# Rinoahu/SwiftOrtho

Measured on AMD Instinct MI355X. Metric: M query-aa/s scanned all-vs-all, higher is better.
Workload: dtype u8/int16/int32 (5-bit packed residues, packed 16-bit score-only DP, int32 traced DP); 1 GPU; BASELINE config 3: 100000 synthetic proteins x 300 aa self-search, seed 11111011111, aa9, -M 120000000, -c 50000 (2 chunks), -e 1e-5, -v 500; query_aa=30007201, rows=1618760

## Files before the change

include/sohit.h:

```cpp
#ifndef SOHIT_H
#define SOHIT_H

#include <stdint.h>

#ifdef __cplusplus
extern "C" {
#endif

#define SOHIT_ABI_VERSION 3

typedef struct so_ctx so_ctx;

typedef struct so_params {
    const char *seeds;
    const char *alphabet;
    int64_t nc;
    int64_t chunk;
    int64_t step;
    int64_t max_hits;
    int64_t thr;
    double expect;
    double max_miss;
    int32_t filter;
    int32_t profile;
// ... 49 lines not shown
    double bgroup_ms;
} so_counters;

so_ctx *so_create(int device, const so_params *params);
void so_destroy(so_ctx *ctx);
const char *so_last_error(const so_ctx *ctx);
int so_abi_version(void);
int so_set_option(so_ctx *ctx, const char *name, const char *value);

int so_load_ref(so_ctx *ctx, const char *fasta_path, int64_t r_lo, int64_t r_hi);
int so_load_ref_mem(so_ctx *ctx, const char *fasta_bytes, int64_t nbytes, int64_t r_lo, int64_t r_hi);
int so_build_index(so_ctx *ctx);
int so_drop_index(so_ctx *ctx);
int so_load_index(so_ctx *ctx, const char *prefix);

int so_load_queries(so_ctx *ctx, const char *fasta_path);
int so_load_queries_mem(so_ctx *ctx, const char *fasta_bytes, int64_t nbytes);
int64_t so_num_queries(const so_ctx *ctx);
int64_t so_num_refs(const so_ctx *ctx);
int64_t so_query_len(const so_ctx *ctx, int64_t qidx);
int64_t so_ref_len(const so_ctx *ctx, int64_t sidx);

int so_search_loaded(so_ctx *ctx, int64_t q_lo, int64_t q_hi, so_hit **hits, int64_t *n_hits);
int so_search(so_ctx *ctx, const char *qry_fasta_path, int64_t q_lo, int64_t q_hi, so_hit **hits, int64_t *n_hits);
void so_free_hits(so_hit *hits);

int so_search_loaded_aln(so_ctx *ctx, int64_t q_lo, int64_t q_hi, so_hit **hits, int64_t *n_hits, char **aln, int64_t *aln_bytes);
void so_free_aln(char *aln);

int so_search_loaded_cigar(so_ctx *ctx, int64_t q_lo, int64_t q_hi, so_hit **hits, int64_t *n_hits, uint32_t **ops, int64_t **op_off);
void so_free_cigar(uint32_t *ops, int64_t *op_off);
int64_t so_format_cigar(const uint32_t *ops, int64_t n_ops, char *buf, int64_t cap);

int so_search_device(so_ctx *ctx, int64_t q_lo, int64_t q_hi, const so_hit **d_hits, int64_t *n_hits);
int so_device_hits_copy(so_ctx *ctx, void *dst_device, int64_t n_hits);
int so_query_work(so_ctx *ctx, int64_t q_lo, int64_t q_hi, uint64_t *work);

int so_write_sc(so_ctx *ctx, const so_hit *hits, int64_t n_hits, const char *path, const char *mode);
int64_t so_format_hit(so_ctx *ctx, const so_hit *hit, char *buf, int64_t cap);
int so_write_sc_cigar(so_ctx *ctx, const so_hit *hits, int64_t n_hits, const uint32_t *ops, const int64_t *op_off, const char *path,
                      const char *mode);

int so_set_profile(so_ctx *ctx, int on);
int64_t so_bucket_count(const so_ctx *ctx);
int64_t so_fmt_rows(const double *v, int64_t n, char *out, int64_t cap);
int so_get_counters(const so_ctx *ctx, so_counters *out);
int so_reset_counters(so_ctx *ctx);
int64_t so_timing_report(const so_ctx *ctx, char *buf, int64_t cap);
int64_t so_chunk_threshold(const so_ctx *ctx, int64_t chunk);
int64_t so_chunk_entries(const so_ctx *ctx, int64_t chunk);
int so_chunk_download(so_ctx *ctx, int64_t chunk, uint32_t *start, uint64_t *entries);
int64_t so_masked_query(so_ctx *ctx, int64_t qidx, char *buf, int64_t cap);
int64_t so_query_candidates(so_ctx *ctx, int64_t qidx, uint32_t *out4, int64_t cap);
int so_align_pairs(so_ctx *ctx, int kernel, int64_t n, const int64_t *task6, const uint32_t *order, int32_t *out);
int so_align_pairs_aln(so_ctx *ctx, int kernel, int64_t n, const int64_t *task6, const uint32_t *order, int32_t *out, char **aln,
                       int64_t *aln_bytes);

int so_align_pairs_cigar(so_ctx *ctx, int kernel, int64_t n, const int64_t *task6, const uint32_t *order, int32_t *out, uint32_t **ops,
                         int64_t **op_off);

typedef struct so_mcl_result {
    int64_t n, nnz;
    int32_t rounds;
    int32_t converged;
    int64_t *indptr;
    int32_t *indices;
    float *data;
} so_mcl_result;
int so_mcl(int device, int64_t n, const int64_t *indptr, const int32_t *indices, const float *data, double inflation, int32_t max_rounds,
           int32_t check_every, double prune, double rtol, double atol, so_mcl_result *out);
void so_mcl_free(so_mcl_result *result);
const char *so_mcl_last_error(void);

typedef struct so_apc_result {
    int64_t n_genes, n_entries;
    int32_t rounds;
    int64_t *labels;
    float *r;
    float *a;
} so_apc_result;
int so_apc(int device, int64_t n_genes, int64_t n_entries, const int32_t *row, const int32_t *col, const float *score, double damp,
           int32_t rounds, so_apc_result *out);
void so_apc_free(so_apc_result *result);
const char *so_apc_last_error(void);

typedef struct so_orth_cand {
    int64_t n_ot, n_ip, n_co, n_rows, n_runs, n_groups;
    int64_t *ot_a, *ot_b; double *ot_s;
    int64_t *ip_a, *ip_b; double *ip_s;
    int64_t *co_key;      double *co_best;
} so_orth_cand;
int so_orth_candidates_cols(int device, int64_t n, const int32_t *q, const int32_t *s, const double *idy, const double *aln,
                            const double *qst, const double *qed, const double *score, const double *qlen, int64_t n_names,
                            const int32_t *tax, int64_t n_taxa, double coverage, double identity, int norm, so_orth_cand *out);
int so_orth_candidates_records(int device, const so_hit *d_hits, int64_t n, const int32_t *qmap, int64_t n_q, const int32_t *smap,
                               int64_t n_s, int64_t n_names, const int32_t *tax, int64_t n_taxa, double coverage, double identity,
                               int norm, so_orth_cand *out);
void so_orth_free(so_orth_cand *result);
const char *so_orth_last_error(void);
typedef struct so_orth_rel {
    int64_t n_ip, n_ot, n_co, n_rows, n_runs, n_groups;
    int64_t *ip_a, *ip_b; double *ip_v;
    int64_t *ot_a, *ot_b; double *ot_v;
    int64_t *co_a, *co_b; double *co_v;
} so_orth_rel;
int so_orth_relations_cols(int device, int64_t n, const int32_t *q, const int32_t *s, const double *idy, const double *aln,
// ... 21 lines not shown
```

swiftortho_amd/_lib.py:

```python
import ctypes as C
import os

HERE = os.path.dirname(os.path.abspath(__file__))
LIBPATH = os.path.join(HERE, "libsohit.so")


class SoParams(C.Structure):
    _fields_ = [("seeds", C.c_char_p), ("alphabet", C.c_char_p), ("nc", C.c_int64), ("chunk", C.c_int64), ("step", C.c_int64),
                ("max_hits", C.c_int64), ("thr", C.c_int64), ("expect", C.c_double), ("max_miss", C.c_double),
                ("filter", C.c_int32), ("profile", C.c_int32)]


class SoOrthRel(C.Structure):
    _fields_ = [(n, C.c_int64) for n in ("n_ip", "n_ot", "n_co", "n_rows", "n_runs", "n_groups")] + \
               [("ip_a", C.POINTER(C.c_int64)), ("ip_b", C.POINTER(C.c_int64)), ("ip_v", C.POINTER(C.c_double)),
                ("ot_a", C.POINTER(C.c_int64)), ("ot_b", C.POINTER(C.c_int64)), ("ot_v", C.POINTER(C.c_double)),
                ("co_a", C.POINTER(C.c_int64)), ("co_b", C.POINTER(C.c_int64)), ("co_v", C.POINTER(C.c_double))]


class SoHit(C.Structure):
    _fields_ = [("qidx", C.c_int64), ("sidx", C.c_int64), ("identity", C.c_double), ("evalue", C.c_double), ("aln", C.c_int32),
                ("mis", C.c_int32), ("gap", C.c_int32), ("qst", C.c_int32), ("qed", C.c_int32), ("sst", C.c_int32),
                ("sed", C.c_int32), ("bit", C.c_int32), ("qlen", C.c_int32), ("slen", C.c_int32), ("matches", C.c_int32),
                ("ungapped", C.c_int32)]


class SoCounters(C.Structure):
    _fields_ = [(n, C.c_int64) for n in ("n_queries", "query_aa", "ref_seqs", "ref_aa", "n_chunks", "seed_windows", "seed_hits",
                                         "groups", "candidates", "alignments", "cells", "rows", "index_entries")] + \
               [("lookup_launches", C.c_int64), ("lookup_ms", C.c_double), ("lookup_bytes", C.c_int64),
                ("bounds_launches", C.c_int64), ("bounds_ms", C.c_double), ("bounds_bytes", C.c_int64),
                ("align_launches", C.c_int64), ("align_ms", C.c_double),
                ("index_ms", C.c_double), ("seed_ms", C.c_double), ("group_ms", C.c_double), ("phase2_ms", C.c_double),
                ("total_ms", C.c_double), ("count_launches", C.c_int64), ("count_ms", C.c_double),
                ("hits_bucketed", C.c_int64), ("align_wide", C.c_int64), ("cells_wide", C.c_int64), ("seed_passes", C.c_int64),
                ("ungap_steps", C.c_int64), ("groups_single", C.c_int64), ("groups_chain", C.c_int64),
                ("bgroup_launches", C.c_int64), ("bgroup_ms", C.c_double)]

    def as_dict(self):
        return {n: getattr(self, n) for n, _ in self._fields_}


EXPORTS = ["so_abi_version", "so_set_option", "so_create", "so_destroy", "so_last_error", "so_load_ref", "so_load_ref_mem", "so_build_index", "so_drop_index", "so_load_index",
           "so_load_queries", "so_load_queries_mem", "so_num_queries", "so_num_refs", "so_query_len", "so_search_loaded",
           "so_search", "so_free_hits", "so_search_loaded_aln", "so_free_aln", "so_write_sc", "so_format_hit", "so_get_counters", "so_reset_counters", "so_timing_report",
           "so_chunk_threshold", "so_chunk_entries", "so_chunk_download", "so_masked_query", "so_query_candidates", "so_align_pairs", "so_align_pairs_aln", "so_set_profile",
           "so_bucket_count", "so_ref_len", "so_search_device", "so_device_hits_copy", "so_query_work", "so_mcl", "so_mcl_free",
           "so_mcl_last_error", "so_tsv_lines", "so_tsv_scan", "so_tsv_codes", "so_format_pairs", "so_py_repr", "so_fmt_rows",
           "so_search_loaded_cigar", "so_free_cigar", "so_format_cigar", "so_write_sc_cigar", "so_align_pairs_cigar",
           "so_apc", "so_apc_free", "so_apc_last_error",
           "so_orth_candidates_cols", "so_orth_candidates_records", "so_orth_free", "so_orth_last_error",
           "so_orth_relations_cols", "so_orth_relations_records", "so_orth_rel_free"]


class SoMclResult(C.Structure):
    _fields_ = [("n", C.c_int64), ("nnz", C.c_int64), ("rounds", C.c_int32), ("converged", C.c_int32), ("indptr", C.POINTER(C.c_int64)),
                ("indices", C.POINTER(C.c_int32)), ("data", C.POINTER(C.c_float))]


class SoApcResult(C.Structure):
    _fields_ = [("n_genes", C.c_int64), ("n_entries", C.c_int64), ("rounds", C.c_int32), ("labels", C.POINTER(C.c_int64)),
                ("r", C.POINTER(C.c_float)), ("a", C.POINTER(C.c_float))]


class SoOrthCand(C.Structure):
    _fields_ = [(n, C.c_int64) for n in ("n_ot", "n_ip", "n_co", "n_rows", "n_runs", "n_groups")] + \
               [("ot_a", C.POINTER(C.c_int64)), ("ot_b", C.POINTER(C.c_int64)), ("ot_s", C.POINTER(C.c_double)),
                ("ip_a", C.POINTER(C.c_int64)), ("ip_b", C.POINTER(C.c_int64)), ("ip_s", C.POINTER(C.c_double)),
                ("co_key", C.POINTER(C.c_int64)), ("co_best", C.POINTER(C.c_double))]


_lib = None


def _preload_torch_hip_runtime():
    import importlib.util
    import sys
    if "torch" in sys.modules or os.environ.get("SOHIT_TORCH_PRELOAD") == "0":
        return
    try:
        spec = importlib.util.find_spec("torch")
    except (ImportError, ValueError):
        spec = None
    if not spec or not spec.submodule_search_locations:
        return
    p = os.path.join(list(spec.submodule_search_locations)[0], "lib", "libamdhip64.so")
    if os.path.isfile(p):
        try:
            C.CDLL(p, mode=C.RTLD_GLOBAL)
        except OSError:
            pass


def load():
    global _lib
    if _lib is not None:
        return _lib
    _preload_torch_hip_runtime()
    if not os.path.isfile(LIBPATH):
# ... 14 lines not shown
    L.so_load_queries.argtypes = [vp, cp]
    L.so_load_queries_mem.argtypes = [vp, cp, i64]
    for f in ("so_num_queries", "so_num_refs"):
        getattr(L, f).restype = i64
        getattr(L, f).argtypes = [vp]
    L.so_query_len.restype = i64
    L.so_query_len.argtypes = [vp, i64]
    L.so_ref_len.restype = i64
    L.so_ref_len.argtypes = [vp, i64]
    L.so_search_loaded.argtypes = [vp, i64, i64, C.POINTER(C.POINTER(SoHit)), C.POINTER(i64)]
    L.so_search.argtypes = [vp, cp, i64, i64, C.POINTER(C.POINTER(SoHit)), C.POINTER(i64)]
    L.so_free_hits.argtypes = [C.POINTER(SoHit)]
    L.so_search_loaded_aln.argtypes = [vp, i64, i64, C.POINTER(C.POINTER(SoHit)), C.POINTER(i64), C.POINTER(C.c_void_p), C.POINTER(i64)]
    L.so_free_aln.argtypes = [vp]
    L.so_search_loaded_cigar.argtypes = [vp, i64, i64, C.POINTER(C.POINTER(SoHit)), C.POINTER(i64), C.POINTER(C.c_void_p), C.POINTER(C.c_void_p)]
    L.so_free_cigar.argtypes = [vp, vp]
    L.so_free_cigar.restype = None
    L.so_format_cigar.restype = i64
    L.so_format_cigar.argtypes = [vp, i64, vp, i64]
    L.so_write_sc_cigar.argtypes = [vp, C.POINTER(SoHit), i64, vp, vp, cp, cp]
    L.so_align_pairs_cigar.argtypes = [vp, C.c_int, i64, vp, vp, vp, C.POINTER(C.c_void_p), C.POINTER(C.c_void_p)]
    L.so_search_device.argtypes = [vp, i64, i64, C.POINTER(vp), C.POINTER(i64)]
    L.so_device_hits_copy.argtypes = [vp, vp, i64]
    L.so_query_work.argtypes = [vp, i64, i64, vp]
    L.so_write_sc.argtypes = [vp, C.POINTER(SoHit), i64, cp, cp]
    L.so_format_hit.restype = i64
    L.so_format_hit.argtypes = [vp, C.POINTER(SoHit), cp, i64]
    L.so_get_counters.argtypes = [vp, C.POINTER(SoCounters)]
    L.so_set_profile.argtypes = [vp, C.c_int]
    L.so_bucket_count.restype = i64
    L.so_bucket_count.argtypes = [vp]
    L.so_reset_counters.argtypes = [vp]
    L.so_timing_report.restype = i64
    L.so_timing_report.argtypes = [vp, cp, i64]
    L.so_tsv_lines.restype = i64
    L.so_tsv_lines.argtypes = [vp, i64, vp, i64]
    L.so_tsv_scan.argtypes = [vp, i64, vp, i64, C.c_int32, vp, vp, vp, vp, vp, vp, vp]
    L.so_tsv_codes.restype = i64
    L.so_tsv_codes.argtypes = [vp, i64, vp, vp, vp, vp, vp, vp, vp, vp, i64]
    L.so_format_pairs.restype = i64
    L.so_format_pairs.argtypes = [cp, C.c_int32, vp, vp, vp, vp, vp, i64, vp, i64]
    L.so_py_repr.restype = i64
    L.so_py_repr.argtypes = [vp, i64, vp, i64]
    L.so_fmt_rows.restype = i64
    L.so_fmt_rows.argtypes = [vp, i64, vp, i64]
    for f in ("so_chunk_threshold", "so_chunk_entries"):
        getattr(L, f).restype = i64
        getattr(L, f).argtypes = [vp, i64]
    L.so_chunk_download.argtypes = [vp, i64, vp, vp]
    L.so_masked_query.restype = i64
    L.so_masked_query.argtypes = [vp, i64, cp, i64]
    L.so_query_candidates.restype = i64
    L.so_query_candidates.argtypes = [vp, i64, vp, i64]
    L.so_align_pairs.argtypes = [vp, C.c_int, i64, vp, vp, vp]
    L.so_align_pairs_aln.argtypes = [vp, C.c_int, i64, vp, vp, vp, C.POINTER(C.c_void_p), C.POINTER(i64)]
    L.so_mcl.argtypes = [C.c_int, i64, vp, vp, vp, C.c_double, C.c_int32, C.c_int32, C.c_double, C.c_double, C.c_double, C.POINTER(SoMclResult)]
    L.so_mcl_free.argtypes = [C.POINTER(SoMclResult)]
    L.so_mcl_last_error.restype = cp
    L.so_apc.argtypes = [C.c_int, i64, i64, vp, vp, vp, C.c_double, C.c_int32, C.POINTER(SoApcResult)]
    L.so_apc_free.argtypes = [C.POINTER(SoApcResult)]
    L.so_apc_last_error.restype = cp
    L.so_orth_candidates_cols.argtypes = [C.c_int, i64, vp, vp, vp, vp, vp, vp, vp, vp, i64, vp, i64, C.c_double, C.c_double, C.c_int, C.POINTER(SoOrthCand)]
    L.so_orth_candidates_records.argtypes = [C.c_int, vp, i64, vp, i64, vp, i64, i64, vp, i64, C.c_double, C.c_double, C.c_int, C.POINTER(SoOrthCand)]
    L.so_orth_free.argtypes = [C.POINTER(SoOrthCand)]
    L.so_orth_last_error.restype = cp
    L.so_orth_relations_cols.argtypes = L.so_orth_candidates_cols.argtypes[:-1] + [C.POINTER(SoOrthRel)]
    L.so_orth_relations_records.argtypes = L.so_orth_candidates_records.argtypes[:-1] + [C.POINTER(SoOrthRel)]
    L.so_orth_rel_free.argtypes = [C.POINTER(SoOrthRel)]
    L.so_set_option.argtypes = [vp, cp, cp]
    if L.so_abi_version() != 3:
        raise ImportError("libsohit.so ABI version mismatch")
    _lib = L
    return L
```

swiftortho_amd/csrc/host.h:

```cpp
#pragma once
#include "common.h"
#include "kernels.h"
#include "seedhash.h"
#include "../../include/sohit.h"

#include <algorithm>
#include <array>
#include <atomic>
#include <chrono>
#include <cmath>
#include <cstring>
#include <functional>
#include <map>
#include <malloc.h>
#include <memory>
#include <mutex>
#include <thread>
#include <unordered_map>
#include <sys/stat.h>

inline double wall() { return std::chrono::duration<double>(std::chrono::steady_clock::now().time_since_epoch()).count(); }

extern double (*volatile p_pow)(double, double);
extern double (*volatile p_log)(double);
// ... 159 lines not shown
    struct BandPlan { i64 lo, hi; int bp; bool multi_ok; int k; u64 nband; };
    std::vector<BandPlan> band_plans;
    i64 r_lo = -1, r_hi = -1;
    std::vector<std::unique_ptr<ChunkIndex>> chunks;
    std::vector<std::unique_ptr<ChunkIndex>> spare_chunks;
    std::vector<std::string> masked;
    i64 masked_lo = 0;
    std::vector<std::vector<u32>> last_cands;
    u64 qry_gen = 0;
    i64 last_q_lo = 0;
    so_counters cnt;
    DevBuf<u32> d_scan_tmp, d_tmp32a, d_tmp32b;
    DevBuf<u64> d_stats;
    DevBuf<u32> d_small;
    DevBuf<u32> ix_bkt, ix_bkt2, ix_flags, ix_ridx, ix_plan, ix_tk;
    DevBuf<u64> ix_ent, ix_tv;
    DevBuf<u8> d_pcls;
    DevBuf<u8> d_sort_tmp;
    hipEvent_t ev0 = nullptr, ev1 = nullptr;
    hipStream_t st_rows = nullptr;
    hipEvent_t ev_rows = nullptr, ev_rows_done = nullptr;
    hipEvent_t ev_part[EMIT_PARTS_MAX] = {nullptr};
    hipStream_t st_side = nullptr;
    hipEvent_t ev_side_go = nullptr, ev_korder = nullptr;
    hipStream_t st_ug = nullptr;
    hipEvent_t ev_ug_go = nullptr, ev_ug_done = nullptr;
    hipEvent_t ev_bnd_go = nullptr, ev_bnd_done = nullptr;
    bool rows_in_flight = false;
    bool count_tab_now = false;
    size_t max_hits_per_pass = (size_t)1 << 30;
    u32 max_batch = 131072;
    DevBuf<u8> d_segtab, d_symmap, d_upmap, d_segmask;
    bool seg_on_device = false;
    bool q_present[256];
    void* pinned = nullptr;
    size_t pinned_cap = 0;
    bool want_aln = false;
    bool want_cigar = false;
    void* pinned_aln = nullptr;
    size_t pinned_aln_cap = 0;
    hipEvent_t ev_aln = nullptr;
    struct EmitJob {
        std::thread th;
        bool active = false;
        size_t base = 0, n = 0;
        bool aln = false;
        bool cig = false;
        std::atomic<i64> dropped{0};
        std::exception_ptr err;
    } emit;
    unsigned long long* h_qhits = nullptr;
    size_t h_qhits_cap = 0;
    unsigned long long* h_small = nullptr;
    std::map<std::string, double> tm;
    std::map<std::string, double> lt;
    std::shared_ptr<void> batch;
    std::thread warm;
    bool dev_out = false;
    DevBuf<u8> d_hits;
    size_t d_hits_n = 0;
    DevBuf<double> d_p2tab;
};

static inline u64 cand_limit() { return tune().cand_limit > 0 ? (u64)tune().cand_limit : 0xFFFFFFF0ull; }


struct SegTables {
    double lg12[64];
    double lgn[13][32];
    double log2v;
    SegTables() {
        log2v = p_log(2);
        for (int k = 1; k < 64; ++k) lg12[k] = p_log((double)k / 12.);
        lg12[0] = 0;
        for (int n = 1; n <= 12; ++n)
            for (int j = 1; j < 32; ++j) lgn[n][j] = p_log((double)j / ((double)n * 1.));
    }
};


template <class F>
void parallel_for(i64 n, F f) {
    unsigned nt = std::max(1u, std::min(16u, std::thread::hardware_concurrency()));
    if (n < 200000 || nt == 1) {
        for (i64 i = 0; i < n; ++i) f(i);
        return;
    }
    std::atomic<i64> next(0);
    std::vector<std::thread> th;
    for (unsigned t = 0; t < nt; ++t)
        th.emplace_back([&] {
            for (;;) {
                i64 b = next.fetch_add(4096);
                if (b >= n) break;
                for (i64 i = b; i < std::min(n, b + 4096); ++i) f(i);
            }
        });
    for (auto& t : th) t.join();
}


inline AlnSide aln_side(const SeqSet& s) { return AlnSide{s.d_res.p, s.d_scls.p, s.d_scls4.p, s.d_pcls.p, s.d_pcls4.p, s.d_off.p, s.d_bound.p}; }
struct AlnChain {
    DevBuf<u32> units, rofs, aofs, code, words, cofs, comp, runs, oofs, ops;
    size_t slot_words = 0;
};
// ... 262 lines not shown
        if (n + extra <= cap) return;
        if (!p) p = g_hit_cache.take(cap);
        if (n + extra <= cap) return;
        size_t nc = std::max<size_t>(n + extra, cap + cap / 2 + 1024);
        so_hit* np_ = (so_hit*)realloc(p, nc * sizeof(so_hit));
        if (!np_) throw SoError("out of host memory for the result rows");
        p = np_;
        cap = nc;
    }
    so_hit* release() {
        so_hit* r = p ? p : (so_hit*)malloc(sizeof(so_hit));
        p = nullptr;
        n = cap = 0;
        return r;
    }
    ~HitBuf() { g_hit_cache.give(p); }
};

struct HostRow {
    int v[12];
};

std::vector<std::string> split(const std::string& s, char sep);
void build_score_maps(u8 smap[256], signed char b62c[SCLS_N * SCLS_N]);
void nr_table(const std::string& gaa, int tbl[256]);
void byte_presence(const u8* bytes, size_t n, bool present[256]);
void build_hash_classes(const bool present[256], const std::vector<std::array<int, 256>>& codes, u8 hmap[256], HashLut& lut);
void set_tune(const Tune* t);
void set_params(so_ctx* c, const so_params* p);
void upload_constants(so_ctx* c);
void layout_set(so_ctx* c, SeqSet& s, const bool present[256], size_t nres, u32 nseq);
void upload_set(so_ctx* c, SeqSet& s, const u8* residues, const std::vector<u32>& off, u32 nseq, const bool* present_in = nullptr);
const SegTables& seg_tables();
void seg_mask(const u8* S, int n, u8* out);
void load_ref_common(so_ctx* c, i64 r_lo, i64 r_hi);
void load_queries_common(so_ctx* c, bool parsed = false);
void file_stamp(const char* path, long long& size, long long& mtime_ns);
bool read_file(const char* path, std::string& out);
i64 chunk_threshold(so_ctx* c, const u32* d_counts , u64 s1, u64 s2, u64 nn);
void warm_sort_modules(int device);
void build_index(so_ctx* c);
void load_index(so_ctx* c, const char* prefix);
void band_plan(so_ctx* c, ChunkIndex& ch, int bp, bool multi_ok, int* k_out, u64* nband_out);
ChunkIndex::BandEnc* band_encoding(so_ctx* c, ChunkIndex& ch, int ba, int bp, bool multi_ok);
void order_chunk(so_ctx* c, ChunkIndex& ch);
const ChunkIndex::RangeTab* range_table(so_ctx* c, ChunkIndex& ch, const ChunkIndex::BandEnc& e, int wb, u32 R);
void prepare_batch(so_ctx* c, Batch& b, i64 q_lo, i64 q_hi);
void order_queries(so_ctx* c, Batch& b);
void order_open_queries(so_ctx* c, Batch& b, const unsigned long long* qh);
void* small_host(so_ctx* c);
u32 d2h_u32(so_ctx* c, const u32* p);
void stash_u32(so_ctx* c, const u32* p, int slot);
void d2h_pair(so_ctx* c, const u32* second, u32& a, u32& b);
void ensure_sort_tmp(so_ctx* c, size_t bytes);
const unsigned long long* chunk_qhits(so_ctx* c, Batch& b, int ci);
void chunk_qhits_deferred(so_ctx* c, Batch& b, int ci);
bool class_takes_sorted_path(so_ctx* c, ChunkIndex& ch, u32 maxq, unsigned long long hits, unsigned long long nq);
void seed_stage(so_ctx* c, Batch& b, int ci);
void seed_pass(so_ctx* c, Batch& b, int ci, u32 qa, u32 qb, double t0, StageClock& sc);
void emit_join(so_ctx* c, HitBuf& out);
void phase2(so_ctx* c, Batch& b, HitBuf& out);
void align_pairs(so_ctx* c, int kernel, i64 n, const int64_t* task6, const uint32_t* order, int32_t* out, AlnBytes* aln = nullptr, CigarBuf* cig = nullptr);
void aln_decode(const u32* w, int AL, const u8* qp, const u8* sp, char* sq, char* ss);
void search_loaded(so_ctx* c, i64 q_lo, i64 q_hi, HitBuf& out);
void query_work(so_ctx* c, i64 q_lo, i64 q_hi, u64* out);
void format_hit_into(so_ctx* c, const so_hit& h, std::vector<char>& out);
std::string format_hit(so_ctx* c, const so_hit& h);
extern std::string g_create_err;


template <class F>
int guarded(so_ctx* c, F f) {
    try {
        if (!c) return 1;
        set_tune(&c->tune);
        g_poison = (int)c->tune.poison;
        HIP_CHECK(hipSetDevice(c->device));
        f();
        c->err.clear();
        return 0;
    } catch (const std::exception& e) {
        if (c) c->err = e.what();
        return 1;
    }
}
```

swiftortho_amd/csrc/host_abi.hip:

```cpp
#include "host.h"

std::string g_create_err;


int fmt_f6(double x, char* out) {
    if (!(std::fabs(x) < 1e15)) return snprintf(out, 400, "%f", x);
    char* o = out;
    if (std::signbit(x)) *o++ = '-', x = -x;
    unsigned __int128 q = 0;
    if (x != 0) {
        int ex;
        const double fr = frexp(x, &ex);
        const u64 m = (u64)ldexp(fr, 53);
        const int e = ex - 53;
        const unsigned __int128 P = (unsigned __int128)m * 1000000u;
        if (e >= 0) {
            q = P << e;
        } else if (-e < 100) {
            const int sh = -e;
            q = P >> sh;
            const unsigned __int128 rem = P & (((unsigned __int128)1 << sh) - 1), half = (unsigned __int128)1 << (sh - 1);
            if (rem > half || (rem == half && (q & 1))) ++q;
        }
    }
// ... 101 lines not shown
        if (!params) throw SoError("so_create: params is NULL");
        int n = 0;
        hipError_t e = hipGetDeviceCount(&n);
        if (e != hipSuccess || n <= 0) throw SoError("so_create: no HIP device available (libsohit has no CPU fallback)");
        if (device < 0 || device >= n) throw SoError("so_create: device index out of range");
        HIP_CHECK(hipSetDevice(device));
        c = new so_ctx();
        c->device = device;
        c->tune.read();
        set_tune(&c->tune);
        g_poison = (int)c->tune.poison;
        {
            int ncu = 0;
            HIP_CHECK(hipDeviceGetAttribute(&ncu, hipDeviceAttributeMultiprocessorCount, device));
            c->ncu = (u32)std::max(1, ncu);
        }
        memset(&c->cnt, 0, sizeof c->cnt);
        set_params(c, params);
        HIP_CHECK(hipStreamCreate(&c->st));
        HIP_CHECK(hipEventCreate(&c->ev0));
        HIP_CHECK(hipEventCreate(&c->ev1));
        HIP_CHECK(hipStreamCreateWithFlags(&c->st_rows, hipStreamNonBlocking));
        HIP_CHECK(hipEventCreateWithFlags(&c->ev_rows, hipEventDisableTiming));
        HIP_CHECK(hipEventCreateWithFlags(&c->ev_rows_done, hipEventDisableTiming));
        HIP_CHECK(hipEventCreateWithFlags(&c->ev_aln, hipEventDisableTiming));
        for (auto& e : c->ev_part) HIP_CHECK(hipEventCreateWithFlags(&e, hipEventDisableTiming));
        HIP_CHECK(hipStreamCreateWithFlags(&c->st_side, hipStreamNonBlocking));
        HIP_CHECK(hipEventCreateWithFlags(&c->ev_side_go, hipEventDisableTiming));
        HIP_CHECK(hipEventCreateWithFlags(&c->ev_korder, hipEventDisableTiming));
        HIP_CHECK(hipStreamCreateWithFlags(&c->st_ug, hipStreamNonBlocking));
        HIP_CHECK(hipEventCreateWithFlags(&c->ev_ug_go, hipEventDisableTiming));
        HIP_CHECK(hipEventCreateWithFlags(&c->ev_ug_done, hipEventDisableTiming));
        HIP_CHECK(hipEventCreateWithFlags(&c->ev_bnd_go, hipEventDisableTiming));
        HIP_CHECK(hipEventCreateWithFlags(&c->ev_bnd_done, hipEventDisableTiming));
        upload_constants(c);
        c->warm = std::thread(warm_sort_modules, device);
        g_create_err.clear();
        return c;
    } catch (const std::exception& e) {
        g_create_err = e.what();
        delete c;
        return nullptr;
    }
}

void so_destroy(so_ctx* c) {
    if (!c) return;
    if (c->warm.joinable()) c->warm.join();
    (void)hipSetDevice(c->device);
    if (c->st) (void)hipStreamSynchronize(c->st);
    if (c->pinned) (void)hipHostFree(c->pinned);
    if (c->pinned_aln) (void)hipHostFree(c->pinned_aln);
    if (c->h_small) (void)hipHostFree(c->h_small);
    if (c->h_qhits) (void)hipHostFree(c->h_qhits);
    if (c->ev0) (void)hipEventDestroy(c->ev0);
    if (c->ev1) (void)hipEventDestroy(c->ev1);
    if (c->ev_rows) (void)hipEventDestroy(c->ev_rows);
    if (c->ev_rows_done) (void)hipEventDestroy(c->ev_rows_done);
    if (c->ev_aln) (void)hipEventDestroy(c->ev_aln);
    for (auto& e : c->ev_part)
        if (e) (void)hipEventDestroy(e);
    if (c->st_rows) (void)hipStreamDestroy(c->st_rows);
    if (c->ev_side_go) (void)hipEventDestroy(c->ev_side_go);
    if (c->ev_korder) (void)hipEventDestroy(c->ev_korder);
    if (c->st_side) (void)hipStreamDestroy(c->st_side);
    if (c->ev_ug_go) (void)hipEventDestroy(c->ev_ug_go);
    if (c->ev_ug_done) (void)hipEventDestroy(c->ev_ug_done);
    if (c->ev_bnd_go) (void)hipEventDestroy(c->ev_bnd_go);
    if (c->ev_bnd_done) (void)hipEventDestroy(c->ev_bnd_done);
    if (c->st_ug) (void)hipStreamDestroy(c->st_ug);
    if (c->st) (void)hipStreamDestroy(c->st);
    if (&c->tune == &tune()) set_tune(nullptr);
    delete c;
    g_hit_cache.clear();
    g_cig_ops_cache.clear(), g_cig_off_cache.clear();
}

const char* so_last_error(const so_ctx* c) { return c ? c->err.c_str() : g_create_err.c_str(); }

int so_load_ref(so_ctx* c, const char* path, int64_t r_lo, int64_t r_hi) {
    return guarded(c, [&] {
        if (!read_file(path, c->ref.data)) throw SoError(std::string("cannot read reference FASTA ") + path);
        load_ref_common(c, r_lo, r_hi);
        c->ref_path = path;
        file_stamp(path, c->ref_fsize, c->ref_mtime_ns);
    });
}

int so_load_ref_mem(so_ctx* c, const char* bytes, int64_t n, int64_t r_lo, int64_t r_hi) {
    return guarded(c, [&] {
        c->ref.data.assign(bytes, (size_t)n);
        load_ref_common(c, r_lo, r_hi);
        c->ref_path.clear();
    });
}

int so_build_index(so_ctx* c) {
    return guarded(c, [&] { build_index(c); });
}

int so_load_index(so_ctx* c, const char* prefix) {
    return guarded(c, [&] { load_index(c, prefix); });
}

int so_drop_index(so_ctx* c) {
    return guarded(c, [&] {
// ... 326 lines not shown
    memset(&c->cnt, 0, sizeof c->cnt);
    c->cnt.ref_seqs = keep.ref_seqs, c->cnt.ref_aa = keep.ref_aa, c->cnt.n_chunks = keep.n_chunks;
    c->cnt.index_entries = keep.index_entries;
    return 0;
}

int64_t so_chunk_threshold(const so_ctx* c, int64_t k) { return (c && k >= 0 && k < (int64_t)c->chunks.size()) ? c->chunks[k]->threshold : -1; }
int64_t so_chunk_entries(const so_ctx* c, int64_t k) { return (c && k >= 0 && k < (int64_t)c->chunks.size()) ? (int64_t)c->chunks[k]->E : -1; }

int so_chunk_download(so_ctx* c, int64_t k, uint32_t* start, uint64_t* entries) {
    return guarded(c, [&] {
        if (k < 0 || k >= (int64_t)c->chunks.size()) throw SoError("so_chunk_download: no such chunk");
        ChunkIndex& ch = *c->chunks[k];
        order_chunk(c, ch);
        if (start) {
            std::vector<u32> ub(ch.U), ubeg((size_t)ch.U + 1);
            if (ch.U) {
                HIP_CHECK(hipMemcpy(ub.data(), ch.ub.p, (size_t)ch.U * sizeof(u32), hipMemcpyDeviceToHost));
                HIP_CHECK(hipMemcpy(ubeg.data(), ch.ubeg.p, ((size_t)ch.U + 1) * sizeof(u32), hipMemcpyDeviceToHost));
            }
            size_t k = 0;
            for (size_t bk = 0; bk <= (size_t)c->nc; ++bk) {
                while (k < ch.U && ub[k] < bk) ++k;
                start[bk] = k < ch.U ? ubeg[k] : ch.E;
            }
        }
        if (entries && ch.E) {
            HIP_CHECK(hipStreamSynchronize(c->st));
            HIP_CHECK(hipMemcpy(entries, ch.entries.p, (size_t)ch.E * sizeof(u64), hipMemcpyDeviceToHost));
        }
    });
}

int64_t so_masked_query(so_ctx* c, int64_t q, char* buf, int64_t cap) {
    if (!c) return -1;
    i64 k = q - c->masked_lo;
    if (k < 0 || k >= (i64)c->masked.size()) return -1;
    const std::string& s = c->masked[(size_t)k];
    if (buf && cap > 0) memcpy(buf, s.data(), std::min<size_t>(s.size(), (size_t)cap));
    return (int64_t)s.size();
}

int64_t so_query_candidates(so_ctx* c, int64_t q, uint32_t* out4, int64_t cap) {
    if (!c) return -1;
    i64 k = q - c->last_q_lo;
    if (k < 0 || k >= (i64)c->last_cands.size()) return -1;
    const auto& v = c->last_cands[(size_t)k];
    const int64_t n = (int64_t)v.size() / 4;
    if (out4)
        for (int64_t i = 0; i < std::min(n, cap) * 4; ++i) out4[i] = v[(size_t)i];
    return n;
}

int so_align_pairs(so_ctx* c, int kernel, int64_t n, const int64_t* task6, const uint32_t* order, int32_t* out) {
    return guarded(c, [&] { align_pairs(c, kernel, n, task6, order, out); });
}

int so_align_pairs_aln(so_ctx* c, int kernel, int64_t n, const int64_t* task6, const uint32_t* order, int32_t* out, char** aln, int64_t* aln_bytes) {
    return guarded(c, [&] {
        if (!aln || !aln_bytes) throw SoError("so_align_pairs_aln: output pointers are NULL");
        *aln = nullptr, *aln_bytes = 0;
        if (kernel != 3 && kernel != 4) throw SoError("so_align_pairs_aln: only the traced kernels (3, 4) give alignments");
        AlnBytes a;
        align_pairs(c, kernel, n, task6, order, out, &a);
        *aln_bytes = (int64_t)a.n;
        *aln = a.release();
    });
}

int so_align_pairs_cigar(so_ctx* c, int kernel, int64_t n, const int64_t* task6, const uint32_t* order, int32_t* out, uint32_t** ops, int64_t** op_off) {
    return guarded(c, [&] {
        if (!ops || !op_off) throw SoError("so_align_pairs_cigar: output pointers are NULL");
        *ops = nullptr, *op_off = nullptr;
        if (kernel != 3 && kernel != 4) throw SoError("so_align_pairs_cigar: only the traced kernels (3, 4) give alignments");
        CigarBuf g;
        align_pairs(c, kernel, n, task6, order, out, nullptr, &g);
        g.release(ops, op_off);
    });
}

}
```

swiftortho_amd/csrc/host_index.hip:

```cpp
#include "host.h"


i64 chunk_threshold(so_ctx* c, const u32* d_counts , u64 s1, u64 s2, u64 nn) {
    const double N = (double)(nn + 1);
    const double mu = (double)s1 / N;
    long double lm = (long double)mu;
    long double ss = (long double)s2 - 2.0L * lm * (long double)s1 + (long double)nn * lm * lm;
    if (ss < 0) ss = 0;
    long double T = lm + 2.0L * sqrtl(ss / (long double)N);
    long double fl = floorl(T);
    long double margin = ((long double)nn * 8e-16L + 1e-11L) * (T + 1.0L);
    const bool forced = tune().exact_threshold;
    if (!forced && T - fl > margin && (fl + 1.0L) - T > margin) return (i64)fl;
    std::vector<u32> counts((size_t)nn);
    if (nn) HIP_CHECK(hipMemcpyAsync(counts.data(), d_counts, (size_t)nn * sizeof(u32), hipMemcpyDeviceToHost, c->st));
    HIP_CHECK(hipStreamSynchronize(c->st));
    i64 Nn = 1;
    double m = 0.;
    for (u32 v : counts)
        if (v > 0) m += (double)v, Nn += 1;
    m /= (double)Nn;
    double sd = 0.;
    for (u32 v : counts)
        if (v > 0) sd += p_pow((double)v - m, 2);
// ... 48 lines not shown
    };
    for (i64 s = Start; s < End; s += c->chunk) {
        std::unique_ptr<ChunkIndex> ch;
        if (!c->spare_chunks.empty()) {
            ch = std::move(c->spare_chunks.front());
            c->spare_chunks.erase(c->spare_chunks.begin());
            ch->d_sh_subj = ch->d_sh_diag = -1;
            for (auto& e : ch->encs) e->stale = true;
            ch->ordered = false;
            for (auto& t : ch->rtabs) t->k = -1;
        } else {
            ch = std::make_unique<ChunkIndex>();
        }
        i64 e = std::min(s + c->chunk, End);
        ch->seq_lo = std::min<i64>(std::max<i64>(0, s), N);
        ch->seq_hi = std::min<i64>(e, N);
        if (ch->seq_hi < ch->seq_lo) ch->seq_hi = ch->seq_lo;
        ch->p_lo = c->ref.off[ch->seq_lo] + (u32)ch->seq_lo;
        ch->p_hi = c->ref.off[ch->seq_hi] + (u32)ch->seq_hi;
        ch->maxslen = 0;
        for (i64 j = ch->seq_lo; j < ch->seq_hi; ++j) ch->maxslen = std::max(ch->maxslen, c->ref.len(j));
        {
            ch->use_dir = (u64)NC <= (tune().dir_max >= 0 ? (u64)tune().dir_max : (1ull << 28));
        }
        const u32 npos = ch->p_hi - ch->p_lo;
        const int AS = c->cfg.A * c->cfg.S;
        const u64 nslots64 = (u64)npos * (u64)AS;
        if (nslots64 >= (1ull << 31)) throw SoError("chunk holds 2^31 seed-window slots or more; lower -c");
        const u32 nslots = (u32)nslots64;
        u32 E = 0;
        ch->U = 0;
        u64 s2 = 0;
        if (nslots) {
            c->ix_bkt.ensure((size_t)nslots + 4), c->ix_ent.ensure((size_t)nslots + 4);
            c->ix_plan.ensure(ixsort_plan_elems((u32)NC) + 8);
            c->d_scan_tmp.ensure(scan_u32_temp_elems(std::max<size_t>(ixsort_plan_elems((u32)NC), (size_t)nslots + 1)) + 8);
            dlap("alloc pairs / plan");
            launch_index_windows_sparse(c->ref.d_words.p, c->ref.d_pseq.p, c->ref.d_off.p, ch->p_lo, ch->p_hi, c->ref.Ppad, (u32)ch->seq_lo, c->cfg, c->ref.lut,
                                        (u32)c->step, c->ix_bkt.p, c->ix_ent.p, c->st);
            E = d2h_u32(c, ixsort_count(c->ix_bkt.p, nslots, (u32)NC, c->ix_plan.p, c->d_scan_tmp.p, c->st));
            dlap("windows + level-1 count");
        }
        if ((u64)E >= (1ull << 29)) throw SoError("chunk index exceeds 2^29 entries (the lookup kernel addresses 8-byte slots with 32-bit byte offsets); lower -c");
        ch->E = E;
        ch->entries.ensure((size_t)E + 4);
        if (E) {
            c->ix_bkt2.ensure((size_t)E + 4), c->ix_tk.ensure((size_t)E + 4), c->ix_tv.ensure((size_t)E + 4);
            dlap("alloc entries / grouping scratch");
            ixsort_finish(c->ix_bkt.p, c->ix_ent.p, nslots, (u32)NC, c->ix_plan.p, c->ix_tk.p, c->ix_tv.p, c->ix_bkt2.p, ch->entries.p, c->st);
            dlap("pair grouping");
            c->ix_flags.ensure((size_t)E + 4), c->ix_ridx.ensure((size_t)E + 4);
            c->d_scan_tmp.ensure(scan_u32_temp_elems((size_t)E + 1) + 8);
            launch_run_heads(c->ix_bkt2.p, E, c->ix_flags.p, c->st);
            const u32 U = d2h_u32(c, scan_u32(c->ix_flags.p, c->ix_ridx.p, E, false, c->d_scan_tmp.p, c->st));
            ch->U = U;
            ch->ub.ensure((size_t)U + 4), ch->ubeg.ensure((size_t)U + 4), ch->ucnt.ensure((size_t)U + 4);
            launch_run_list(c->ix_bkt2.p, c->ix_flags.p, c->ix_ridx.p, E, U, ch->ub.p, ch->ubeg.p, ch->ucnt.p, c->st);
            dlap("run heads / list");
            launch_index_stats(ch->ucnt.p, U, c->d_stats.p, c->st);
            u64* stats = (u64*)small_host(c);
            u32* last_lo_h = (u32*)(stats + 4);
            HIP_CHECK(hipMemcpyAsync(stats, c->d_stats.p, 4 * sizeof(u64), hipMemcpyDeviceToHost, c->st));
            HIP_CHECK(hipMemcpyAsync(last_lo_h, ch->ubeg.p + (U - 1), sizeof(u32), hipMemcpyDeviceToHost, c->st));
            HIP_CHECK(hipStreamSynchronize(c->st));
            s2 = stats[1];
            const u32 last_lo = *last_lo_h;
            dlap("stats");
            if (ch->use_dir) {
                const size_t nd = (size_t)NC / 32 + 2;
                ch->dir.ensure(nd);
                HIP_CHECK(hipMemsetAsync(ch->dir.p, 0, nd * sizeof(u64), c->st));
                launch_dir_build(ch->ub.p, U, ch->dir.p, c->st);
            } else {
                u32 cap = 1024;
                int lg = 10;
                while (cap < 2 * U) cap <<= 1, ++lg;
                ch->hkey.ensure(cap), ch->hval.ensure(cap);
                ch->hshift = 32 - lg, ch->hmask = cap - 1;
                HIP_CHECK(hipMemsetAsync(ch->hkey.p, 0xFF, (size_t)cap * sizeof(u32), c->st));
                launch_htab_insert(ch->ub.p, ch->ubeg.p, U, ch->hkey.p, ch->hval.p, ch->hshift, ch->hmask, c->st);
            }
            launch_index_fixlast(ch->entries.p, last_lo, E, c->st);
        } else if (ch->use_dir) {
            const size_t nd = (size_t)NC / 32 + 2;
            ch->dir.ensure(nd);
            ch->ubeg.ensure(4);
            HIP_CHECK(hipMemsetAsync(ch->dir.p, 0, nd * sizeof(u64), c->st));
        } else {
            ch->hkey.ensure(1024), ch->hval.ensure(1024);
            ch->hshift = 22, ch->hmask = 1023;
            HIP_CHECK(hipMemsetAsync(ch->hkey.p, 0xFF, 1024 * sizeof(u32), c->st));
        }
        dlap("directory + fixlast");
        ch->threshold = chunk_threshold(c, ch->ucnt.p, (u64)E, s2, (u64)ch->U);
        ch->s2 = s2;
        HIP_CHECK(hipStreamSynchronize(c->st));
        c->cnt.index_entries += ch->E;
        c->chunks.push_back(std::move(ch));
    }
    c->spare_chunks.clear();
    c->cnt.n_chunks = (i64)c->chunks.size();
    c->index_built = true;
    c->cnt.index_ms += (wall() - t0) * 1e3;
}


bool host_window_bucket(const so_ctx* c, const u8* seq, u32 len, u32 pos, int a, int s, u32* bucket) {
// ... 314 lines not shown
```

swiftortho_amd/csrc/host_phase2.hip:

```cpp
#include "host.h"


void aln_decode(const u32* w, int AL, const u8* qp, const u8* sp, char* sq, char* ss) {
    for (int f = 0; f < AL; ++f) {
        const int cc = AL - 1 - f;
        const u32 code = (w[cc >> 4] >> ((cc & 15) << 1)) & 3u;
        sq[f] = code != 2 ? (char)*qp++ : '-';
        ss[f] = code != 3 ? (char)*sp++ : '-';
    }
}

void emit_join(so_ctx* c, HitBuf& out) {
    if (!c->emit.active) return;
    c->emit.th.join();
    c->emit.active = false;
    if (c->emit.err) {
        std::exception_ptr e = c->emit.err;
        c->emit.err = nullptr;
        std::rethrow_exception(e);
    }
    if (c->emit.dropped.load()) {
        const double expect = c->expect;
        if (c->emit.cig) {
            CigarBuf& g = out.cig;
            size_t w = c->emit.base;
            int64_t rp = g.off[c->emit.base], ap = rp;
            for (size_t k = c->emit.base; k < c->emit.base + c->emit.n; ++k) {
                const int64_t re = g.off[k + 1], nr = re - rp;
                if (out.p[k].evalue <= expect) {
                    if (nr && ap != rp) memmove(g.ops + ap, g.ops + rp, (size_t)nr * sizeof(uint32_t));
                    ap += nr;
                    g.off[++w] = ap;
                }
                rp = re;
            }
            g.n = (size_t)ap;
        }
        size_t wpos = c->emit.base;
        size_t bytes = 0;
        if (c->emit.aln)
            for (size_t k = c->emit.base; k < c->emit.base + c->emit.n; ++k) bytes += 2 * (size_t)std::max(0, out.p[k].aln);
        size_t rpos = out.aln.n - std::min(bytes, out.aln.n), apos = rpos;
        for (size_t k = c->emit.base; k < c->emit.base + c->emit.n; ++k) {
            const size_t nb = c->emit.aln ? 2 * (size_t)std::max(0, out.p[k].aln) : 0;
            if (out.p[k].evalue <= expect) {
                if (nb && apos != rpos) memmove(out.aln.p + apos, out.aln.p + rpos, nb);
                apos += nb;
                out.p[wpos++] = out.p[k];
            }
            rpos += nb;
        }
        out.n = wpos;
        if (c->emit.aln) out.aln.n = apos;
    }
}

enum { P2TAB_N = 1200 };
static const double* pow2_table() {
    static const std::vector<double> t = [] {
        std::vector<double> v(P2TAB_N);
        for (int k = 0; k < P2TAB_N; ++k) v[k] = p_pow(2, (double)(-k));
        return v;
    }();
    return t.data();
}

static void aln_slots(so_ctx* c, AlnChain& a, const AlnTask* tasks, const u32* list, u32 n, u32 ntasks, const AlnSeqs& s) {
    a.units.ensure((size_t)n + 4), a.rofs.ensure((size_t)n + 4), a.aofs.ensure((size_t)ntasks + 4);
    c->d_scan_tmp.ensure(scan_u32_temp_elems((size_t)n + 1) + 8);
    if ((u64)n * 129u >= (1ull << 30)) throw SoError("alignments: more than 8 M reported rows in one batch; search a smaller query range per call");
    launch_aln_units(tasks, list, n, s, a.units.p, c->st);
    const size_t units = d2h_u32(c, scan_u32(a.units.p, a.rofs.p, (size_t)n + 1, false, c->d_scan_tmp.p, c->st));
    a.slot_words = units * aln_unit_words();
    a.code.ensure(a.slot_words + 64);
    launch_aln_scatter(list, n, a.rofs.p, a.aofs.p, c->st);
}
static size_t aln_compact(so_ctx* c, AlnChain& a, const u32* list, u32 n, const AlnRes* res) {
    a.words.ensure((size_t)n + 4), a.cofs.ensure((size_t)n + 4);
    launch_aln_words(list, n, res, a.words.p, c->st);
    const size_t words = d2h_u32(c, scan_u32(a.words.p, a.cofs.p, (size_t)n + 1, false, c->d_scan_tmp.p, c->st));
    a.comp.ensure(words + 64);
    launch_aln_compact(list, n, a.aofs.p, a.code.p, a.cofs.p, a.comp.p, c->st);
    return words;
}
static size_t cigar_code(so_ctx* c, AlnChain& a, const u32* list, u32 n, const AlnRes* res) {
    if (a.slot_words * 16ull >= (1ull << 32)) throw SoError("CIGARs: the reported rows of one batch hold 2^32 columns or more; search a smaller query range per call");
    a.runs.ensure((size_t)n + 4), a.oofs.ensure((size_t)n + 4);
    launch_cigar_count(list, n, a.aofs.p, a.code.p, res, a.runs.p, c->st);
    const size_t n_ops = d2h_u32(c, scan_u32(a.runs.p, a.oofs.p, (size_t)n + 1, false, c->d_scan_tmp.p, c->st));
    a.ops.ensure(n_ops + 64);
    launch_cigar_emit(list, n, a.aofs.p, a.code.p, res, a.oofs.p, a.ops.p, c->st);
    return n_ops;
}
template <class F>
static std::vector<size_t> aln_word_offsets(size_t n, F aln_at, size_t words, const char* who) {
    std::vector<size_t> w(n + 1, 0);
    for (size_t i = 0; i < n; ++i) w[i + 1] = w[i] + (size_t)(std::max(0, (int)aln_at(i)) + 15) / 16;
    if (w[n] != words) throw SoError(std::string(who) + ": column words do not add up");
    return w;
}

struct P2 {
    P2(so_ctx* c, const Batch& b) : sc(c), nq(b.nq) {}
    const double t0 = wall();
    StageClock sc;
    u32 nq, Ntot = 0, NT = 0, nspec = 0, NO = 0;
    AlnSeqs seqs{};
    bool align_sort = false, pk_on = false, pk_mixed = false, lane_on = false, traced_pk = false, aln_on = false, cig_on = false;
    u32 stride = 0, slab = 0, TU = 0;
    size_t var_budget_words = 0, aln_words = 0, cig_ops = 0;
    int parts = 1; u32 qstep = 0;
    std::array<u32, EMIT_PARTS_MAX + 1> part_row{};
    std::vector<u32> h_ooff;
};

static bool gather_candidates(so_ctx* c, Batch& b, P2& p) {
    const int nchunks = (int)c->chunks.size();
    const u32 nq = p.nq;
    const u32 Ntot = p.Ntot = b.chunk_base.empty() ? 0u : b.chunk_base.back();
    b.qtot.ensure((size_t)nq + 4), b.qcoff.ensure((size_t)nq + 4), b.prior.ensure((size_t)nq + 4), b.cqoff.ensure((size_t)nq + 4);
    HIP_CHECK(hipMemsetAsync(b.qtot.p, 0, ((size_t)nq + 4) * sizeof(u32), c->st));
    for (int ci = 0; ci < nchunks; ++ci) launch_add_u32(b.qtot.p, b.ccnt.p + (size_t)ci * nq, nq, c->st);
    c->d_scan_tmp.ensure(scan_u32_temp_elems((size_t)nq + 1) + 8);
    scan_u32(b.qtot.p, b.qcoff.p, (size_t)nq + 1, false, c->d_scan_tmp.p, c->st);
    b.fin_rec.ensure(4 * (size_t)Ntot + 16);
    HIP_CHECK(hipMemsetAsync(b.prior.p, 0, ((size_t)nq + 4) * sizeof(u32), c->st));
    for (int ci = 0; ci < nchunks; ++ci) {
        const u32 lo = ci == 0 ? 0u : b.chunk_base[ci - 1], hi = b.chunk_base[ci];
        const u32* cc = b.ccnt.p + (size_t)ci * nq;
        if (hi > lo) {
            scan_u32(cc, b.cqoff.p, nq, false, c->d_scan_tmp.p, c->st);
            launch_gather_cands(b.cand_q.p + lo, b.cand_rec.p + 4 * (size_t)lo, hi - lo, b.cqoff.p, b.prior.p, b.qcoff.p, b.fin_rec.p,
                                c->st);
        }
        launch_add_u32(b.prior.p, cc, nq, c->st);
    }
    p.sc.lap("phase2.gather");
    if (tune().keep_cands) {
        std::vector<u32> qcoff((size_t)nq + 1), rec(4 * (size_t)Ntot + 4);
        HIP_CHECK(hipMemcpyAsync(qcoff.data(), b.qcoff.p, ((size_t)nq + 1) * sizeof(u32), hipMemcpyDeviceToHost, c->st));
        if (Ntot) HIP_CHECK(hipMemcpyAsync(rec.data(), b.fin_rec.p, 4 * (size_t)Ntot * sizeof(u32), hipMemcpyDeviceToHost, c->st));
        HIP_CHECK(hipStreamSynchronize(c->st));
        for (u32 q = 0; q < nq; ++q) {
            auto& dst = c->last_cands[(size_t)(b.q_lo - c->last_q_lo) + b.qid[q]];
            dst.assign(rec.begin() + 4 * (size_t)qcoff[q], rec.begin() + 4 * (size_t)qcoff[q + 1]);
        }
    }
    return Ntot != 0;
}

static void make_tasks(so_ctx* c, Batch& b, P2& p) {
    const u32 nq = p.nq, Ntot = p.Ntot;
    const u32 vmax = (u32)std::max<i64>(100, std::max<i64>(c->v + 100, (i64)((double)c->v * 1.1)));
    b.perm.ensure((size_t)Ntot + 4), b.ntask.ensure((size_t)nq + 4), b.ntile.ensure((size_t)nq + 4);
    b.toff.ensure((size_t)nq + 4), b.roffc.ensure((size_t)nq + 4);
    HIP_CHECK(hipMemsetAsync(b.ntask.p, 0, ((size_t)nq + 4) * sizeof(u32), c->st));
    HIP_CHECK(hipMemsetAsync(b.ntile.p, 0, ((size_t)nq + 4) * sizeof(u32), c->st));
    if (c->h_qhits_cap < nq) {
        if (c->h_qhits) (void)hipHostFree(c->h_qhits);
        c->h_qhits_cap = (size_t)nq + 1024;
        HIP_CHECK(hipHostMalloc((void**)&c->h_qhits, c->h_qhits_cap * sizeof(unsigned long long), hipHostMallocDefault));
    }
    const u32* qt = reinterpret_cast<const u32*>(c->h_qhits);
    HIP_CHECK(hipMemcpyAsync(c->h_qhits, b.qtot.p, (size_t)nq * sizeof(u32), hipMemcpyDeviceToHost, c->st));
    HIP_CHECK(hipStreamSynchronize(c->st));
    u32 mx = 0;
    for (u32 i = 0; i < nq; ++i) mx = std::max(mx, qt[i]);
    u64* gx = nullptr;
    u32 *gL = nullptr, *gR = nullptr;
    if ((int)mx > csort_lds_max()) {
        b.gx.ensure((size_t)Ntot + 4), b.gL.ensure((size_t)Ntot + 4), b.gR.ensure((size_t)Ntot + 4);
        gx = b.gx.p, gL = b.gL.p, gR = b.gR.p;
    }
    const bool cs_aside = gx != nullptr;
    if (cs_aside) {
        HIP_CHECK(hipEventRecord(c->ev_ug_go, c->st));
        HIP_CHECK(hipStreamWaitEvent(c->st_side, c->ev_ug_go, 0));
    }
    launch_csort(b.fin_rec.p, b.qcoff.p, nq, vmax, b.dev.d_off.p, c->ref.d_off.p, b.perm.p, b.ntask.p, b.ntile.p, gx, gL, gR, c->st,
                 cs_aside ? c->st_side : c->st);
    if (cs_aside) {
        HIP_CHECK(hipEventRecord(c->ev_ug_done, c->st_side));
        HIP_CHECK(hipStreamWaitEvent(c->st, c->ev_ug_done, 0));
    }
    const u32* dNRk = scan_u32(b.ntask.p, b.roffc.p, (size_t)nq + 1, false, c->d_scan_tmp.p, c->st);
    stash_u32(c, dNRk, SM_STASH0);
    const u32* dNT = scan_u32(b.ntile.p, b.toff.p, (size_t)nq + 1, false, c->d_scan_tmp.p, c->st);
    u32 NRK;
    d2h_pair(c, dNT, NRK, p.NT);
    const u32 NT = p.NT;
    p.sc.lap("phase2.csort");
    b.tasks.ensure((size_t)NT + 4), b.ares.ensure((size_t)NT + 4), b.bits.ensure((size_t)NT + 4), b.sel.ensure((size_t)NT + 4);
    b.rk_slot.ensure((size_t)NRK + 4);
    b.qcells.ensure((size_t)nq + 2);
    HIP_CHECK(hipMemsetAsync(b.qcells.p, 0, ((size_t)nq + 2) * sizeof(unsigned long long), c->st));
    launch_mktasks(b.fin_rec.p, b.qcoff.p, b.perm.p, b.ntask.p, b.roffc.p, b.toff.p, nq, b.dev.d_off.p, c->ref.d_off.p, b.tasks.p,
                   b.rk_slot.p, c->st);
    p.align_sort = tune().align_sort;
    const u32 maxwin_q = std::min<u32>(b.maxqlen, LONG_SEQ), maxwin_s = std::min<u32>(c->ref.maxlen, LONG_SEQ);
    p.pk_on = tune().align_pk && align_pk_supported(c->st);
    p.pk_mixed = p.pk_on && (int)std::min(maxwin_q, maxwin_s) > align_pk_max_len();
    p.seqs = AlnSeqs{aln_side(b.dev), aln_side(c->ref), c->d_b62c.p};
    p.lane_on = p.pk_on && tune().align_lane && b.maxqlen < LONG_SEQ && c->ref.maxlen < LONG_SEQ;
    p.traced_pk = p.pk_on;
    p.stride = align_trace_stride((int)std::min<u32>(std::max(maxwin_q, maxwin_s), std::min(maxwin_q, maxwin_s) + 16) + 1);
    const long long trace_var_max = tune().trace_var_max;
    const size_t budget_words = trace_var_max >= 0 ? (size_t)trace_var_max : (size_t)1 << 30;
    p.slab = (u32)std::max<size_t>(16, std::min<size_t>(std::max<u32>(NT, 1), budget_words / std::max<u32>(p.stride, 1)));
    p.var_budget_words = trace_var_max >= 0 ? (size_t)trace_var_max : (size_t)1 << 31;
    p.TU = align_trace_unit();
    b.st_state.ensure(5 * (size_t)nq + 8), b.rcnt.ensure((size_t)nq + 4), b.tcnt.ensure((size_t)nq + 4), b.roff.ensure((size_t)nq + 4);
    b.order_tmp.ensure((size_t)nq + 4);
    b.ridx.ensure((size_t)NT + 4);
    HIP_CHECK(hipMemsetAsync(b.st_state.p, 0, (5 * (size_t)nq + 8) * sizeof(u32), c->st));
    p.sc.lap("phase2.mktasks");
}

static void order_by_rows(so_ctx* c, Batch& b, const AlnSeqs& s, const u32* in, u32 n, u32* out, u32* n_wide, unsigned long long* cells) {
    if (!n) return;
    b.tmp64.ensure((size_t)n + 2), b.c_ft2.ensure((size_t)n + 2);
    ensure_sort_tmp(c, sort_pairs_u64_u32_temp_bytes(n, 64));
    launch_task_rows(b.tasks.p, in, n, s, n_wide, cells, b.tmp64.p, c->st);
    sort_pairs_u64_u32(c->d_sort_tmp.p, c->d_sort_tmp.cap, b.tmp64.p, b.c_ft2.p, in, out, n, n_wide ? 14 : 13, c->st);
}

static const u32* round_list(so_ctx* c, Batch& b, const P2& p, const u32* list, u32 n, u32* n_wide) {
    const bool split = n_wide && p.pk_mixed;
    if (n_wide) *n_wide = p.pk_on ? 0u : n;
    if (!split && (!p.align_sort || n < 4096)) return list;
    b.ridx2.ensure((size_t)n + 2);
    c->d_small.ensure(SM_WORDS);
    if (split) HIP_CHECK(hipMemsetAsync(c->d_small.p + SM_WIDE_ROUND, 0, sizeof(u32), c->st));
    order_by_rows(c, b, p.seqs, list, n, b.ridx2.p, split ? c->d_small.p + SM_WIDE_ROUND : nullptr, b.ucount.p + 2);
    if (split) *n_wide = d2h_u32(c, c->d_small.p + SM_WIDE_ROUND);
    return b.ridx2.p;
}

static size_t trace_offsets(so_ctx* c, Batch& b, const P2& p, const u32* list, u32 n) {
    if ((u64)n * ((u64)(p.stride + p.TU - 1) / p.TU + 1) >= (1ull << 32)) return ~(size_t)0;
    b.tr_units.ensure((size_t)n + 4), b.tr_ofs.ensure((size_t)n + 4);
    c->d_scan_tmp.ensure(scan_u32_temp_elems((size_t)n + 1) + 8);
    launch_trace_units(b.tasks.p, list, n, p.seqs, b.tr_units.p, c->st);
    return (size_t)d2h_u32(c, scan_u32(b.tr_units.p, b.tr_ofs.p, (size_t)n + 1, false, c->d_scan_tmp.p, c->st)) * p.TU;
}

static void align_rounds(so_ctx* c, Batch& b, P2& p) {
    const u32 nq = p.nq, NT = p.NT;
    const AlnSeqs& s = p.seqs;
    u32 aligned_total = 0;
    const bool spec_on = tune().spec >= 0 ? tune().spec != 0 : NT >= (1u << 21);
    const double spec_slack = tune().spec_slack;
    u32 spec_cap = NT;
    if (tune().spec_cap >= 0) spec_cap = (u32)tune().spec_cap;
    if (spec_on) {
        b.tpos.ensure((size_t)NT + 4);
        HIP_CHECK(hipMemsetAsync(b.tpos.p, 0xFF, ((size_t)NT + 4) * sizeof(u32), c->st));
    }
    bool first_round = true;
    for (u32 minr = 8;; minr = minr < 256 ? minr * 2 : minr) {
        u32 NR = 0, RR = 0, NS = 0;
        bool spec_round = spec_on && first_round;
        first_round = false;
        if (spec_round) {
            b.spcnt.ensure((size_t)nq + 4), b.spoff.ensure((size_t)nq + 4), b.sidx.ensure((size_t)NT + 4);
            c->d_small.ensure(SM_WORDS);
            HIP_CHECK(hipMemsetAsync(c->d_small.p + SM_ANY_RANK, 0, sizeof(u32), c->st));
            launch_round_counts_spec(b.ntask.p, b.ntile.p, b.roffc.p, b.rk_slot.p, b.qcoff.p, b.st_state.p, nq, c->max_miss, minr, b.tasks.p, b.toff.p,
                                     b.dev.d_off.p, c->ref.d_off.p, c->d_bittab.p, so_ctx::BITTAB_N, c->ref.N, c->expect * spec_slack, b.rcnt.p, b.tcnt.p, b.spcnt.p,
                                     c->d_small.p + SM_ANY_RANK, c->st);
            stash_u32(c, scan_u32(b.tcnt.p, b.roff.p, (size_t)nq + 1, false, c->d_scan_tmp.p, c->st), SM_STASH0);
            stash_u32(c, scan_u32(b.spcnt.p, b.spoff.p, (size_t)nq + 1, false, c->d_scan_tmp.p, c->st), SM_STASH1);
            u32* v = (u32*)small_host(c);
            HIP_CHECK(hipMemcpyAsync(v, c->d_small.p, (SM_ANY_RANK + 1) * sizeof(u32), hipMemcpyDeviceToHost, c->st));
            HIP_CHECK(hipStreamSynchronize(c->st));
            NR = v[SM_STASH0], NS = v[SM_STASH1], RR = v[SM_ANY_RANK];
            if (NS > spec_cap) spec_round = false;
        }
        if (!spec_round) {
            NS = 0;
            launch_round_counts(b.ntask.p, b.ntile.p, b.roffc.p, b.rk_slot.p, b.qcoff.p, b.st_state.p, nq, c->max_miss, minr, b.rcnt.p,
                                b.tcnt.p, c->st);
            const u32* dNR = scan_u32(b.tcnt.p, b.roff.p, (size_t)nq + 1, false, c->d_scan_tmp.p, c->st);
            stash_u32(c, dNR, SM_STASH0);
            const u32* dRR = scan_u32(b.rcnt.p, b.order_tmp.p, (size_t)nq + 1, false, c->d_scan_tmp.p, c->st);
            d2h_pair(c, dRR, NR, RR);
        }
        if (RR == 0) break;
        if (spec_round) {
            launch_round_idx_spec(b.tcnt.p, b.spcnt.p, b.roff.p, b.spoff.p, b.toff.p, b.ntask.p, b.ntile.p, b.roffc.p, b.rk_slot.p, b.st_state.p, nq,
                                  b.ridx.p, b.sidx.p, c->st);
            if (NS) {
                u32 nw_s = 0;
                const u32* slist = round_list(c, b, p, b.sidx.p, NS, p.traced_pk ? &nw_s : nullptr);
                if (!p.traced_pk) nw_s = NS;
                const size_t tw = trace_offsets(c, b, p, slist, NS);
                ProfTimer pt(c, &c->cnt.align_ms, &c->cnt.align_launches);
                if (tw <= p.var_budget_words) {
                    b.spec_trace.ensure(tw + 64);
                    launch_align_traced(b.tasks.p, slist, NS, s, b.spec_trace.p, p.TU, b.tr_ofs.p, b.ares.p, b.tpos.p, 0u, c->st, nw_s);
                    p.nspec = NS;
                } else {
                    if (tune().debug) fprintf(stderr, "[sohit] kept traces do not fit: %u tasks scored only\n", NS);
                    launch_align(b.tasks.p, slist, NS, s, b.ares.p, c->st);
                }
                pt.stop();
            }
        } else if (NR) {
            launch_round_idx(b.tcnt.p, b.roff.p, b.toff.p, b.ntask.p, b.ntile.p, b.roffc.p, b.rk_slot.p, b.st_state.p, nq, b.ridx.p, c->st);
        }
        if (NR) {
            u32 n_wide = 0;
            const u32* rlist = round_list(c, b, p, b.ridx.p, NR, &n_wide);
            ProfTimer pt(c, &c->cnt.align_ms, &c->cnt.align_launches);
            const bool wide_aside = n_wide && NR > n_wide;
            hipStream_t wst = wide_aside ? c->st_side : c->st;
            if (wide_aside) {
                HIP_CHECK(hipEventRecord(c->ev_ug_go, c->st));
                HIP_CHECK(hipStreamWaitEvent(c->st_side, c->ev_ug_go, 0));
            }
            if (n_wide) launch_align(b.tasks.p, rlist, n_wide, s, b.ares.p, wst);
            if (wide_aside) HIP_CHECK(hipEventRecord(c->ev_ug_done, c->st_side));
            if (NR > n_wide) {
                if (p.lane_on && (long long)(NR - n_wide) >= tune().align_lane_min) {
                    c->d_small.ensure(SM_WORDS);
                    launch_align_lane(b.tasks.p, rlist + n_wide, NR - n_wide, s, b.ares.p, c->d_small.p + SM_LANE_CTR, c->ncu, c->st);
                } else {
                    launch_align_pk(b.tasks.p, rlist + n_wide, NR - n_wide, s, b.ares.p, c->st);
                }
            }
            if (wide_aside) HIP_CHECK(hipStreamWaitEvent(c->st, c->ev_ug_done, 0));
            pt.stop();
            c->cnt.align_wide += n_wide;
        }
        launch_stop_round_w(b.tasks.p, b.ares.p, b.qcoff.p, b.ntask.p, b.ntile.p, b.roffc.p, b.rk_slot.p, b.toff.p, b.rcnt.p, nq,
                            b.dev.d_off.p, c->ref.d_off.p, c->d_bittab.p, so_ctx::BITTAB_N, c->ref.N, c->expect, c->max_miss, c->v, b.sel.p,
                            b.st_state.p, b.bits.p, b.qcells.p, c->st);
        aligned_total += NR + NS;
    }
    launch_sum_u64(b.qcells.p, nq, b.ucount.p + 1, c->st);
    p.sc.lap("phase2.align_rounds");
    c->cnt.alignments += aligned_total;
}

static void select_rows(so_ctx* c, Batch& b, P2& p) {
    const u32 nq = p.nq;
    b.nout.ensure((size_t)nq + 4), b.ooff.ensure((size_t)nq + 4);
    HIP_CHECK(hipMemsetAsync(b.nout.p, 0xFF, (size_t)nq * sizeof(u32), c->st));
    HIP_CHECK(hipMemsetAsync(b.nout.p + nq, 0, 4 * sizeof(u32), c->st));
    launch_final_select(b.toff.p, nq, c->v, b.sel.p, b.st_state.p, b.bits.p, b.nout.p, c->st);
    const u32* dNO = scan_u32(b.nout.p, b.ooff.p, (size_t)nq + 1, false, c->d_scan_tmp.p, c->st);
    const int emit_parts = std::min<int>(EMIT_PARTS_MAX, std::max(1, (p.nspec && (b.permuted || p.pk_mixed)) ? 2 : (int)tune().emit_parts));
    const u32 emit_min_rows = (u32)std::max(1ll, tune().emit_min_rows);
    const u32 qstep = p.qstep = (nq + emit_parts - 1) / emit_parts;
    c->d_small.ensure(SM_WORDS);
    launch_stride_gather(b.ooff.p, qstep, (nq + qstep - 1) / qstep, c->d_small.p + SM_PART_ROW, c->st);
    stash_u32(c, dNO, SM_STASH0);
    u32* v = (u32*)small_host(c);
    HIP_CHECK(hipMemcpyAsync(v, c->d_small.p, (SM_PART_ROW + EMIT_PARTS_MAX) * sizeof(u32), hipMemcpyDeviceToHost, c->st));
    if (b.permuted && !c->dev_out) {
        p.h_ooff.resize((size_t)nq + 1);
        HIP_CHECK(hipMemcpyAsync(p.h_ooff.data(), b.ooff.p, ((size_t)nq + 1) * sizeof(u32), hipMemcpyDeviceToHost, c->st));
    }
    HIP_CHECK(hipStreamSynchronize(c->st));
    const u32 NO = p.NO = v[SM_STASH0];
    for (int q = 0; q <= emit_parts; ++q) p.part_row[q] = (u64)q * qstep < nq ? v[SM_PART_ROW + q] : NO;
    p.parts = (c->dev_out || NO < emit_min_rows) ? 1 : emit_parts;
    if (p.parts == 1) p.part_row[1] = NO;
    p.aln_on = c->want_aln && !c->dev_out;
    p.cig_on = c->want_cigar && !c->dev_out;
    p.sc.lap("phase2.stop");
}

static void split_kept_traces(so_ctx* c, Batch& b, const P2& p, u32* pb ) {
    const u32 NO = p.NO;
    const int parts = p.parts;
    const u32* slist = b.sel_idx.p;
    b.flags.ensure((size_t)NO + 4), b.gidx.ensure((size_t)NO + 4), b.sel_b.ensure((size_t)NO + 4), b.sel_a.ensure((size_t)NO + 4);
    c->d_scan_tmp.ensure(scan_u32_temp_elems((size_t)NO + 1) + 8);
    launch_trace_flags(slist, NO, b.tpos.p, b.flags.p, c->st);
    const u32* dNB = scan_u32(b.flags.p, b.gidx.p, NO, false, c->d_scan_tmp.p, c->st);
    launch_trace_split(slist, NO, b.flags.p, b.gidx.p, b.sel_b.p, b.sel_a.p, c->st);
    u32* v = (u32*)small_host(c);
    HIP_CHECK(hipMemcpyAsync(v + parts, dNB, sizeof(u32), hipMemcpyDeviceToHost, c->st));
    for (int q = 1; q < parts; ++q)
        if (p.part_row[q] < NO) HIP_CHECK(hipMemcpyAsync(v + q, b.gidx.p + p.part_row[q], sizeof(u32), hipMemcpyDeviceToHost, c->st));
    HIP_CHECK(hipStreamSynchronize(c->st));
    pb[parts] = v[parts];
    for (int q = 1; q < parts; ++q) pb[q] = p.part_row[q] < NO ? v[q] : pb[parts];
    if (tune().debug) fprintf(stderr, "[sohit] kept traces %u, reported rows %u, of them without a trace %u\n", p.nspec, NO, pb[parts]);
}

static void order_trace_lists(so_ctx* c, Batch& b, const P2& p, const u32* tlist, u32 tn, const u32* alist, const u32* pb, u32* nwide) {
    c->d_small.ensure(SM_WORDS);
    const bool split = p.traced_pk && p.pk_mixed;
    if (split) HIP_CHECK(hipMemsetAsync(c->d_small.p + SM_WIDE_PART, 0, EMIT_PARTS_MAX * sizeof(u32), c->st));
    b.tl_sorted.ensure((size_t)tn + 4);
    if (p.nspec) b.al_sorted.ensure((size_t)(p.NO - tn) + 4);
    for (int q = 0; q < p.parts; ++q) {
        const u32 a0 = p.part_row[q] - pb[q], a1 = p.part_row[q + 1] - pb[q + 1];
        order_by_rows(c, b, p.seqs, tlist + pb[q], pb[q + 1] - pb[q], b.tl_sorted.p + pb[q], split ? c->d_small.p + SM_WIDE_PART + q : nullptr, nullptr);
        if (p.nspec) order_by_rows(c, b, p.seqs, alist + a0, a1 - a0, b.al_sorted.p + a0, nullptr, nullptr);
    }
    if (split) {
        u32* v = (u32*)small_host(c);
        HIP_CHECK(hipMemcpyAsync(v, c->d_small.p + SM_WIDE_PART, EMIT_PARTS_MAX * sizeof(u32), hipMemcpyDeviceToHost, c->st));
        HIP_CHECK(hipStreamSynchronize(c->st));
        for (int q = 0; q < p.parts; ++q) nwide[q] = v[q];
    }
}

static void trace_pass(so_ctx* c, Batch& b, P2& p, HitBuf& out) {
    const u32 nq = p.nq, NO = p.NO, nspec = p.nspec;
    const int parts = p.parts;
    b.sel_idx.ensure((size_t)NO + 4);
    launch_selected_idx(b.toff.p, b.sel.p, b.nout.p, b.ooff.p, nq, b.sel_idx.p, c->st);
    u32 maxpart = 0;
    for (int q = 0; q < parts; ++q) maxpart = std::max(maxpart, p.part_row[q + 1] - p.part_row[q]);
    b.outrec.ensure(12 * (size_t)NO + 16);
    if (c->rows_in_flight) {
        HIP_CHECK(hipStreamWaitEvent(c->st, c->ev_rows_done, 0));
        c->rows_in_flight = false;
    }
    if (!c->dev_out) {
        emit_join(c, out);
        if (c->pinned_cap < (size_t)NO * sizeof(HostRow)) {
            if (c->pinned) (void)hipHostFree(c->pinned);
            c->pinned_cap = (size_t)NO * sizeof(HostRow) * 5 / 4 + 4096;
            HIP_CHECK(hipHostMalloc(&c->pinned, c->pinned_cap, hipHostMallocDefault));
        }
    }
    const u32* slist = b.sel_idx.p;
    const bool emit_cols = p.aln_on || p.cig_on;
    if (emit_cols) aln_slots(c, b.aln, b.tasks.p, slist, NO, p.NT, p.seqs);
// ... 46 lines not shown
            HIP_CHECK(hipMemcpyAsync((char*)c->pinned + (size_t)r0 * sizeof(HostRow), b.outrec.p + 12 * (size_t)r0, (size_t)(r1 - r0) * sizeof(HostRow),
                                     hipMemcpyDeviceToHost, c->st_rows));
            HIP_CHECK(hipEventRecord(c->ev_part[q], c->st_rows));
        }
    }
    if (p.aln_on) {
        const size_t aln_words = p.aln_words = aln_compact(c, b.aln, slist, NO, b.ares.p);
        const size_t qbytes = b.h_off[nq], need = aln_words * 4 + qbytes + 64;
        if (c->pinned_aln_cap < need) {
            if (c->pinned_aln) (void)hipHostFree(c->pinned_aln);
            c->pinned_aln = nullptr, c->pinned_aln_cap = 0;
            HIP_CHECK(hipHostMalloc(&c->pinned_aln, need * 5 / 4 + 4096, hipHostMallocDefault));
            c->pinned_aln_cap = need * 5 / 4 + 4096;
        }
        if (aln_words) HIP_CHECK(hipMemcpyAsync(c->pinned_aln, b.aln.comp.p, aln_words * 4, hipMemcpyDeviceToHost, c->st));
        if (qbytes) HIP_CHECK(hipMemcpyAsync((char*)c->pinned_aln + aln_words * 4, b.dev.d_res.p, qbytes, hipMemcpyDeviceToHost, c->st));
        HIP_CHECK(hipEventRecord(c->ev_aln, c->st));
    }
    if (p.cig_on) {
        const size_t n_ops = p.cig_ops = cigar_code(c, b.aln, slist, NO, b.ares.p);
        const size_t need = ((size_t)NO + 1 + n_ops) * sizeof(u32) + 64;
        if (c->pinned_aln_cap < need) {
            if (c->pinned_aln) (void)hipHostFree(c->pinned_aln);
            c->pinned_aln = nullptr, c->pinned_aln_cap = 0;
            HIP_CHECK(hipHostMalloc(&c->pinned_aln, need * 5 / 4 + 4096, hipHostMallocDefault));
            c->pinned_aln_cap = need * 5 / 4 + 4096;
        }
        HIP_CHECK(hipMemcpyAsync(c->pinned_aln, b.aln.oofs.p, ((size_t)NO + 1) * sizeof(u32), hipMemcpyDeviceToHost, c->st));
        if (n_ops) HIP_CHECK(hipMemcpyAsync((u32*)c->pinned_aln + NO + 1, b.aln.ops.p, n_ops * sizeof(u32), hipMemcpyDeviceToHost, c->st));
        HIP_CHECK(hipEventRecord(c->ev_aln, c->st));
    }
    p.sc.lap("phase2.trace_pass");
    {
        static bool fired = false;
        if (!fired && nq > 1 && tune().test_oom_phase2) {
            fired = true;
            throw DevOom(0);
        }
    }
}

static void emit_device(so_ctx* c, Batch& b, P2& p) {
    const u32 nq = p.nq, NO = p.NO;
    if (!c->d_p2tab.p) {
        c->d_p2tab.ensure(P2TAB_N);
        HIP_CHECK(hipMemcpy(c->d_p2tab.p, pow2_table(), P2TAB_N * sizeof(double), hipMemcpyHostToDevice));
    }
    c->d_hits.ensure((c->d_hits_n + NO) * sizeof(so_hit) + 256, true, c->st);
    const u32 *d_qid = nullptr, *d_ostart = nullptr;
    if (b.permuted) {
        b.d_ocnt.ensure((size_t)nq + 4), b.d_ostart.ensure((size_t)nq + 4);
        launch_scatter_u32(b.nout.p, b.d_qid.p, nq, b.d_ocnt.p, c->st);
        HIP_CHECK(hipMemsetAsync(b.d_ocnt.p + nq, 0, sizeof(u32), c->st));
        scan_u32(b.d_ocnt.p, b.d_ostart.p, (size_t)nq + 1, false, c->d_scan_tmp.p, c->st);
        d_qid = b.d_qid.p, d_ostart = b.d_ostart.p;
    }
    launch_make_hits(b.outrec.p, NO, b.q_lo, d_qid, b.ooff.p, d_ostart, c->qry.d_off.p, c->ref.d_off.p, c->ref.N, c->d_p2tab.p, P2TAB_N,
                     c->d_hits.p + c->d_hits_n * sizeof(so_hit), c->st);
    c->d_hits_n += NO;
    p.sc.lap("phase2.emit_device");
}

static void emit_host(so_ctx* c, Batch& b, P2& p, HitBuf& out) {
    const u32 nq = p.nq, NO = p.NO;
    const HostRow* rows = (const HostRow*)c->pinned;
    HIP_CHECK(hipEventRecord(c->ev_rows_done, c->st_rows));
    c->rows_in_flight = true;
    if (c->profile) HIP_CHECK(hipEventSynchronize(c->ev_rows_done));
    p.sc.lap("phase2.emit_d2h");
    const size_t base = out.n;
    out.grow(NO);
    so_hit* dst = out.p + base;
    out.n = base + NO;
    std::shared_ptr<std::vector<std::pair<u32, i64>>> place;
    if (b.permuted) {
        const std::vector<u32>& ooff = p.h_ooff;
        std::vector<u32> ocnt((size_t)nq + 1, 0);
        for (u32 s = 0; s < nq; ++s) ocnt[b.qid[s]] = ooff[s + 1] - ooff[s];
        u32 run = 0;
        for (u32 o = 0; o < nq; ++o) {
            const u32 n = ocnt[o];
            ocnt[o] = run;
            run += n;
        }
        place = std::make_shared<std::vector<std::pair<u32, i64>>>(nq);
        for (u32 s = 0; s < nq; ++s) (*place)[s] = {b.qid[s], (i64)ocnt[b.qid[s]] - (i64)ooff[s]};
    }
    c->emit.base = base, c->emit.n = NO, c->emit.aln = p.aln_on, c->emit.cig = p.cig_on;
    if (p.cig_on) out.cig.rows(base + NO);
    c->emit.dropped.store(0);
    c->emit.active = true;
    std::shared_ptr<std::vector<u32>> aln_qoff;
    if (p.aln_on) aln_qoff = std::make_shared<std::vector<u32>>(b.h_off.begin(), b.h_off.begin() + nq + 1);
    c->emit.th = std::thread([c, rows, dst, NO, D = c->ref.N, expect = c->expect, q_lo = b.q_lo, p2p = pow2_table(), place, part_row = p.part_row, parts = p.parts, aln_qoff,
                              abuf = &out.aln, aln_words = p.aln_words, cbuf = p.cig_on ? &out.cig : nullptr, cig_ops = p.cig_ops, base] {
        try {
            HIP_CHECK(hipSetDevice(c->device));
            auto convert = [&](i64 i) {
                const int* v = rows[i].v;
                so_hit h;
                i64 di = i;
                if (place) {
                    const auto& pl = (*place)[(size_t)v[0]];
                    h.qidx = q_lo + pl.first;
                    di = i + pl.second;
                } else {
                    h.qidx = q_lo + v[0];
// ... 131 lines not shown
        if (kernel == 2 && (qe != lq || se != ls)) refuse("k_align_lane takes no tile: both windows must end where their sequences end");
        if (kernel == 2 && (lq >= LONG_SEQ || ls >= LONG_SEQ)) refuse("k_align_lane takes no sequence of 4096 residues or more");
        tk[(size_t)t] = AlnTask{(u32)v[0], (u32)v[1], (u32)v[2], (u32)v[3], 0u, 0u, (u32)qe, (u32)se};
    }
    std::vector<u32> list((size_t)n);
    std::vector<char> listed((size_t)n, 0);
    for (i64 p = 0; p < n; ++p) {
        const u32 s = order ? order[p] : (u32)p;
        if ((i64)s >= n) throw SoError("so_align_pairs: order[" + std::to_string(p) + "] out of range");
        if (traced && listed[s]) throw SoError("so_align_pairs: a traced launch list holds every task once");
        listed[s] = 1, list[(size_t)p] = s;
    }
    if (packed && !(tune().align_pk && align_pk_supported(c->st))) throw SoError("so_align_pairs: the packed aligners are switched off or not supported here");
    SeqSet qs;
    upload_set(c, qs, Q.res.data(), Q.off, (u32)Q.N);
    const AlnSeqs seqs{aln_side(qs), aln_side(R), c->d_b62c.p};
    DevBuf<AlnTask> d_tasks;
    DevBuf<u32> d_list, d_cnt;
    DevBuf<u64> d_keys;
    DevBuf<AlnRes> d_res;
    d_tasks.ensure((size_t)n + 4), d_list.ensure((size_t)n + 4), d_cnt.ensure(4), d_keys.ensure((size_t)n + 4), d_res.ensure((size_t)n + 4);
    HIP_CHECK(hipMemcpyAsync(d_tasks.p, tk.data(), (size_t)n * sizeof(AlnTask), hipMemcpyHostToDevice, c->st));
    HIP_CHECK(hipMemcpyAsync(d_list.p, list.data(), (size_t)n * sizeof(u32), hipMemcpyHostToDevice, c->st));
    HIP_CHECK(hipMemsetAsync(d_cnt.p, 0, 4 * sizeof(u32), c->st));
    launch_task_rows(d_tasks.p, d_list.p, (u32)n, seqs, d_cnt.p, nullptr, d_keys.p, c->st);
    std::vector<u64> keys((size_t)n);
    HIP_CHECK(hipMemcpyAsync(keys.data(), d_keys.p, (size_t)n * sizeof(u64), hipMemcpyDeviceToHost, c->st));
    HIP_CHECK(hipStreamSynchronize(c->st));
    std::vector<char> wide((size_t)n, 0);
    for (i64 p = 0; p < n; ++p) wide[list[(size_t)p]] = (keys[(size_t)p] & 8192u) ? 0 : 1;
    if (packed)
        for (i64 t = 0; t < n; ++t)
            if (listed[(size_t)t] && wide[(size_t)t])
                throw SoError("so_align_pairs: task " + std::to_string(t) + ": its scores need 32-bit cells, the packed aligners do not take it");
    DevBuf<u32> d_units, d_tofs, d_trace;
    AlnChain chain;
    std::vector<u32> h_acomp, h_oofs, h_ops;
    size_t aln_words = 0;
    switch (kernel) {
    case 0:
        launch_align(d_tasks.p, d_list.p, (u32)n, seqs, d_res.p, c->st);
        break;
    case 1:
        launch_align_pk(d_tasks.p, d_list.p, (u32)n, seqs, d_res.p, c->st);
        break;
    case 2:
        launch_align_lane(d_tasks.p, d_list.p, (u32)n, seqs, d_res.p, d_cnt.p + 1, c->ncu, c->st);
        break;
    default: {
        const u32 TU = align_trace_unit();
        d_units.ensure((size_t)n + 4), d_tofs.ensure((size_t)n + 4);
        c->d_scan_tmp.ensure(scan_u32_temp_elems((size_t)n + 1) + 8);
        launch_trace_units(d_tasks.p, d_list.p, (u32)n, seqs, d_units.p, c->st);
        const size_t tw = (size_t)d2h_u32(c, scan_u32(d_units.p, d_tofs.p, (size_t)n + 1, false, c->d_scan_tmp.p, c->st)) * TU;
        d_trace.ensure(tw + 64);
        if (aln || cig) aln_slots(c, chain, d_tasks.p, d_list.p, (u32)n, (u32)n, seqs);
        launch_align_walk(d_tasks.p, d_list.p, (u32)n, seqs, d_trace.p, TU, d_tofs.p, d_res.p, c->st, kernel == 3 ? (u32)n : 0u, aln || cig ? chain.code.p : nullptr,
                          aln || cig ? chain.aofs.p : nullptr);
        if (cig) {
            const size_t n_ops = cigar_code(c, chain, d_list.p, (u32)n, d_res.p);
            h_oofs.resize((size_t)n + 1), h_ops.resize(n_ops + 1);
            HIP_CHECK(hipMemcpyAsync(h_oofs.data(), chain.oofs.p, ((size_t)n + 1) * sizeof(u32), hipMemcpyDeviceToHost, c->st));
            if (n_ops) HIP_CHECK(hipMemcpyAsync(h_ops.data(), chain.ops.p, n_ops * sizeof(u32), hipMemcpyDeviceToHost, c->st));
        }
        if (aln) {
            aln_words = aln_compact(c, chain, d_list.p, (u32)n, d_res.p);
            h_acomp.resize(aln_words + 1);
            if (aln_words) HIP_CHECK(hipMemcpyAsync(h_acomp.data(), chain.comp.p, aln_words * sizeof(u32), hipMemcpyDeviceToHost, c->st));
        }
        break;
    }
    }
    std::vector<AlnRes> res((size_t)n);
    HIP_CHECK(hipMemcpyAsync(res.data(), d_res.p, (size_t)n * sizeof(AlnRes), hipMemcpyDeviceToHost, c->st));
    HIP_CHECK(hipStreamSynchronize(c->st));
    if (aln) {
        const std::vector<size_t> woff = aln_word_offsets((size_t)n, [&](size_t p) { return res[list[p]].aln; }, aln_words, "so_align_pairs_aln");
        std::vector<size_t> boff((size_t)n + 1, 0);
        for (i64 t = 0; t < n; ++t) boff[(size_t)t + 1] = boff[(size_t)t] + 2 * (size_t)std::max(0, res[(size_t)t].aln);
        const size_t a0 = aln->n;
        aln->grow(boff[(size_t)n]);
        for (i64 p = 0; p < n; ++p) {
            const u32 t = list[(size_t)p];
            const AlnRes& r = res[t];
            if (r.aln <= 0) continue;
            const u32* w = h_acomp.data() + woff[(size_t)p];
            int nq_adv = 0, ns_adv = 0;
            for (int cc = 0; cc < r.aln; ++cc) {
                const u32 code = (w[cc >> 4] >> ((cc & 15) << 1)) & 3u;
                nq_adv += code != 2, ns_adv += code != 3;
            }
            if (r.qst < 0 || r.sst < 0 || nq_adv != r.qed - r.qst || ns_adv != r.sed - r.sst || r.qed > (int)Q.len(tk[t].q) || r.sed > (int)R.len(tk[t].subj))
                throw SoError("so_align_pairs_aln: task " + std::to_string(t) + ": the columns do not cover its coordinates");
            char* sq = aln->p + a0 + boff[t];
            aln_decode(w, r.aln, Q.res.data() + Q.off[tk[t].q] + r.qst, R.res.data() + R.off[tk[t].subj] + r.sst, sq, sq + r.aln);
        }
        aln->n = a0 + boff[(size_t)n];
    }
    if (cig) {
        for (i64 p = 0; p < n; ++p) cig->off[list[(size_t)p] + 1] = (int64_t)h_oofs[(size_t)p + 1] - (int64_t)h_oofs[(size_t)p];
        for (i64 t = 0; t < n; ++t) cig->off[t + 1] += cig->off[t];
        cig->grow((size_t)cig->off[n]);
        for (i64 p = 0; p < n; ++p) {
            const u32 t = list[(size_t)p];
            const AlnRes& r = res[t];
            const u32* w = h_ops.data() + h_oofs[(size_t)p];
            const i64 nr = cig->off[t + 1] - cig->off[t];
// ... 20 lines not shown
```

swiftortho_amd/csrc/host_seed.hip:

```cpp
#include "host.h"

static void defer_long_class(so_ctx* c, Batch& b, u32 q_long) {
    b.korder_async = q_long < b.nq && b.cls_sorted && b.qcls[q_long] != b.qcls[0];
    if (!b.korder_async) return;
    b.q_defer = q_long;
    while (b.q_defer > 0 && b.qcls[b.q_defer - 1] == b.qcls[q_long]) --b.q_defer;
    HIP_CHECK(hipEventRecord(c->ev_side_go, c->st));
    HIP_CHECK(hipStreamWaitEvent(c->st_side, c->ev_side_go, 0));
}

void order_queries(so_ctx* c, Batch& b) {
    const u32 q_long = b.ksc_long;
    const size_t nres = b.h_off[b.nq];
    if (q_long < b.nq) b.gx.ensure(nres + 4), b.gL.ensure(nres + 4), b.gR.ensure(nres + 4);
    defer_long_class(c, b, q_long);
    launch_ksc_order(b.dev.d_scls.p, b.dev.d_off.p, b.nq, q_long, c->cfg.mink, c->d_b62c.p, b.gx.p, b.gL.p, b.gR.p, b.korder.p, c->st,
                     b.korder_async ? c->st_side : c->st);
    if (b.korder_async) HIP_CHECK(hipEventRecord(c->ev_korder, c->st_side));
    b.korder_ready = true;
}

void order_open_queries(so_ctx* c, Batch& b, const unsigned long long* qh) {
    u32 q_long = b.nq;
    for (u32 q = b.ksc_long; q < b.nq && q_long == b.nq; ++q)
// ... 82 lines not shown
                HIP_CHECK(hipStreamWaitEvent(c->st_side, c->ev_side_go, 0));
            }
            launch_seg(c->qry.d_res.p, c->qry.d_off.p, (u32)q_lo, d_qid, b.nq, b.dev.d_off.p, c->d_symmap.p, c->d_upmap.p, c->d_segtab.p,
                       c->d_segmask.p, b.dev.d_res.p, b.maxqlen, q_mid, q_long, c->st, seg_aside ? c->st_side : c->st);
            if (seg_aside) {
                HIP_CHECK(hipEventRecord(c->ev_ug_done, c->st_side));
                HIP_CHECK(hipStreamWaitEvent(c->st, c->ev_ug_done, 0));
            }
        } else if (b.permuted) {
            launch_gather_seqs(c->qry.d_res.p, c->qry.d_off.p, (u32)q_lo, d_qid, b.nq, b.dev.d_off.p, b.dev.d_res.p, c->st);
        } else {
            launch_copy_range(c->qry.d_res.p + Q.off[q_lo], b.dev.d_res.p, nres_b, c->st);
        }
        layout_set(c, b.dev, c->q_present, nres_b, b.nq);
        b.h_res.clear();
    } else {
        b.h_res.resize(nres_b + 16);
        const u8* src = Q.res.data();
        parallel_for((i64)b.nq, [&](i64 i) { seg_mask(src + Q.off[q_lo + b.qid[i]], (int)Q.len(q_lo + b.qid[i]), b.h_res.data() + b.h_off[i]); });
        upload_set(c, b.dev, b.h_res.data(), b.h_off, b.nq);
    }
    const int AS = c->cfg.A * c->cfg.S;
    const u32 Ppad = b.dev.Ppad;
    const size_t T = (size_t)AS * Ppad;
    b.qbucket.ensure(T);
    launch_qhash(b.dev.d_words.p, Ppad, c->cfg, b.dev.lut, b.qbucket.p, c->st);
    const size_t nres = b.h_off[b.nq];
    b.korder.ensure(nres + 1);
    {
        u32 q_long = b.nq;
        for (u32 blk = 0; blk < (u32)b.blkmax.size() && q_long == b.nq; ++blk) {
            if ((i64)b.blkmax[blk] - c->cfg.mink + 1 <= (i64)ksc_lds_max()) continue;
            for (u32 i = blk << 8; i < std::min<u32>(b.nq, (blk + 1) << 8); ++i)
                if ((i64)(b.h_off[i + 1] - b.h_off[i]) - c->cfg.mink + 1 > (i64)ksc_lds_max()) {
                    q_long = i;
                    break;
                }
        }
        b.ksc_long = q_long;
        b.korder_ready = false, b.kord_have_clear = false, b.n_open = 0;
        if (!tune().ksc_lazy) order_queries(c, b);
    }
    b.sbeg.ensure(T), b.scnt.ensure(T), b.hoff.ensure(T + 4), b.cidx.ensure(T + 4);
    b.pcnt.ensure(Ppad), b.mark.ensure(Ppad);
    b.counters.ensure(8);
    b.ucount.ensure(4);
    HIP_CHECK(hipMemsetAsync(b.ucount.p, 0, 4 * sizeof(unsigned long long), c->st));
    c->d_scan_tmp.ensure(std::max(scan_u32_temp_elems(std::max<size_t>(T, (size_t)c->nc + 1)), effscan_temp_elems(T)) + 8);
    c->cnt.seed_windows += (i64)AS * (i64)nres;
}


void* small_host(so_ctx* c) {
    if (!c->h_small) HIP_CHECK(hipHostMalloc((void**)&c->h_small, 1024, hipHostMallocDefault));
    return c->h_small;
}

u32 d2h_u32(so_ctx* c, const u32* p) {
    u32* v = (u32*)small_host(c);
    HIP_CHECK(hipMemcpyAsync(v, p, sizeof(u32), hipMemcpyDeviceToHost, c->st));
    HIP_CHECK(hipStreamSynchronize(c->st));
    return *v;
}

void stash_u32(so_ctx* c, const u32* p, int slot) {
    c->d_small.ensure(SM_WORDS);
    HIP_CHECK(hipMemcpyAsync(c->d_small.p + slot, p, sizeof(u32), hipMemcpyDeviceToDevice, c->st));
}
void d2h_pair(so_ctx* c, const u32* second, u32& a, u32& b) {
    stash_u32(c, second, SM_STASH1);
    u32* v = (u32*)small_host(c);
    HIP_CHECK(hipMemcpyAsync(v, c->d_small.p + SM_STASH0, 2 * sizeof(u32), hipMemcpyDeviceToHost, c->st));
    HIP_CHECK(hipStreamSynchronize(c->st));
    a = v[0], b = v[1];
}

void ensure_sort_tmp(so_ctx* c, size_t bytes) { c->d_sort_tmp.ensure(bytes + 256); }

const unsigned long long* chunk_qhits(so_ctx* c, Batch& b, int ci) {
    ChunkIndex& ch = *c->chunks[ci];
    const int AS = c->cfg.A * c->cfg.S;
    const u32 Ppad = b.dev.Ppad, NC = (u32)c->nc;
    if (b.bnd_ci == ci) {
        HIP_CHECK(hipStreamWaitEvent(c->st, c->ev_bnd_done, 0));
        std::swap(b.sbeg.p, b.sbeg2.p), std::swap(b.sbeg.cap, b.sbeg2.cap);
        std::swap(b.scnt.p, b.scnt2.p), std::swap(b.scnt.cap, b.scnt2.cap);
        std::swap(b.pcnt.p, b.pcnt2.p), std::swap(b.pcnt.cap, b.pcnt2.cap);
    } else {
        if (b.bnd_ci >= 0) HIP_CHECK(hipStreamWaitEvent(c->st, c->ev_bnd_done, 0));
        ProfTimer pt(c, &c->cnt.bounds_ms, &c->cnt.bounds_launches);
        launch_bounds(b.qbucket.p, Ppad, AS, ch.hkey.p, ch.hval.p, ch.hshift, ch.hmask, ch.use_dir ? ch.dir.p : nullptr, ch.ubeg.p, NC, ch.E, b.sbeg.p,
                      b.scnt.p, b.pcnt.p, c->st);
        pt.stop();
        if (c->profile) c->cnt.bounds_bytes += (i64)8 * AS * (i64)b.h_off[b.nq];
    }
    b.bnd_ci = -1;
    if (tune().bounds_ahead && !c->profile) {
        int nx = ci + 1;
        while (nx < (int)c->chunks.size() && (c->chunks[nx]->seq_hi == c->chunks[nx]->seq_lo || c->chunks[nx]->E == 0)) ++nx;
        if (nx < (int)c->chunks.size()) {
            ChunkIndex& cn = *c->chunks[nx];
            const size_t T = (size_t)AS * Ppad;
            b.sbeg2.ensure(T), b.scnt2.ensure(T), b.pcnt2.ensure(Ppad);
            HIP_CHECK(hipEventRecord(c->ev_bnd_go, c->st));
            HIP_CHECK(hipStreamWaitEvent(c->st_side, c->ev_bnd_go, 0));
            launch_bounds(b.qbucket.p, Ppad, AS, cn.hkey.p, cn.hval.p, cn.hshift, cn.hmask, cn.use_dir ? cn.dir.p : nullptr, cn.ubeg.p, NC, cn.E, b.sbeg2.p, b.scnt2.p,
                          b.pcnt2.p, c->st_side);
            HIP_CHECK(hipEventRecord(c->ev_bnd_done, c->st_side));
// ... 93 lines not shown
                unsigned long long h = 0;
                for (u32 q = b.cls_start[k]; q < b.cls_start[k + 1]; ++q) h += qh[q];
                hits[k] = h;
            }
        } else {
            for (u32 q = 0; q < known; ++q) {
                const int k = b.qcls[q];
                hits[k] += qh[q], cnt[k]++, maxq[k] = std::max(maxq[k], b.h_off[q + 1] - b.h_off[q]);
            }
        }
        whole_classes = b.cls_sorted && known == b.nq;
        for (int k = 0; k < QCLASSES; ++k) cls_hits[k] = hits[k];
        {
            unsigned long long tot = 0;
            for (int k = 0; k < QCLASSES; ++k) tot += hits[k];
            c->count_tab_now = tune().count_tab >= 2 || (tune().count_tab == 1 && (ch.ordered || tot >= 2 * budget));
            if (tune().debug) fprintf(stderr, "[sohit] chunk %d: %llu seed hits in this batch, budget %llu per pass, count_tab %lld -> %d\n", ci, tot, budget, (long long)tune().count_tab, (int)c->count_tab_now);
        }
        const int held = b.korder_async ? (int)b.qcls[b.q_defer] : -1;
        bool sp[QCLASSES];
        for (int k = 0; k < QCLASSES; ++k) sp[k] = merge_on && k != held && cnt[k] && class_takes_sorted_path(c, ch, maxq[k], hits[k], cnt[k]);
        grp[0] = 0;
        for (int k = 1; k < QCLASSES; ++k) {
            int j = k - 1;
            while (j > 0 && !cnt[j] && j != held) --j;
            grp[k] = grp[k - 1] + ((sp[k] && sp[j] && grp[j] == grp[k - 1]) || (!cnt[k] && k != held) ? 0 : 1);
        }
    }
    u32 qa = 0;
    while (qa < b.nq) {
        if (b.korder_async && qa >= b.q_defer) chunk_qhits_deferred(c, b, ci);
        unsigned long long acc = 0;
        u32 qb = qa;
        while (whole_classes && qb < b.nq && qb == b.cls_start[b.qcls[qb]] && acc + cls_hits[b.qcls[qb]] <= budget && grp[b.qcls[qb]] == grp[b.qcls[qa]])
            acc += cls_hits[b.qcls[qb]], qb = b.cls_start[b.qcls[qb] + 1];
        while (qb < b.nq && (qb == qa || (acc + qh[qb] <= budget && grp[b.qcls[qb]] == grp[b.qcls[qa]]))) acc += qh[qb++];
        if (acc >= 0xFFFFFFF0ull) throw SoError("a single query visits >= 2^32 index entries in one chunk: lower -c");
        if (acc) seed_pass(c, b, ci, qa, qb, wall(), sc), ++c->cnt.seed_passes;
        if (tune().debug) fprintf(stderr, "[sohit] chunk %d pass queries [%u, %u) classes %d..%d hits %llu\n", ci, qa, qb, (int)b.qcls[qa], (int)b.qcls[qb - 1], acc);
        qa = qb;
    }
}

void seed_pass(so_ctx* c, Batch& b, int ci, u32 qa, u32 qb, double t0, StageClock& sc) {
    ChunkIndex& ch = *c->chunks[ci];
    const u32 p_lo = b.h_off[qa] + qa, p_hi = b.h_off[qb] + qb;
    const int AS = c->cfg.A * c->cfg.S;
    const u32 nseq_chunk = (u32)(ch.seq_hi - ch.seq_lo);
    u32* qcnt = b.ccnt.p + (size_t)ci * b.nq;
    const size_t t_lo = (size_t)AS * p_lo, Tp = (size_t)AS * (p_hi - p_lo);
    u32 H, K;
    if (AS == 1) {
        c->d_scan_tmp.ensure(effscan_temp_elems(Tp) + 8);
        const u32* dHK = effscan(b.mark.p + p_lo, b.scnt.p + t_lo, Tp, b.hoff.p + t_lo, b.cidx.p + t_lo, c->d_scan_tmp.p, c->st);
        u32* v = (u32*)small_host(c);
        HIP_CHECK(hipMemcpyAsync(v, dHK, 2 * sizeof(u32), hipMemcpyDeviceToHost, c->st));
        HIP_CHECK(hipStreamSynchronize(c->st));
        H = v[0], K = v[1];
    } else {
        b.eff.ensure((size_t)AS * b.dev.Ppad + 4), b.nz.ensure((size_t)AS * b.dev.Ppad + 4);
        launch_effcnt(b.mark.p, b.scnt.p, AS, p_lo, p_hi, b.eff.p, b.nz.p, c->st);
        const u32* dH = scan_u32(b.eff.p + t_lo, b.hoff.p + t_lo, Tp, false, c->d_scan_tmp.p, c->st);
        stash_u32(c, dH, SM_STASH0);
        const u32* dK = scan_u32(b.nz.p + t_lo, b.cidx.p + t_lo, Tp, false, c->d_scan_tmp.p, c->st);
        d2h_pair(c, dK, H, K);
    }
    sc.lap("seed.bounds_cap_scan");
    c->cnt.seed_hits += H;
    if (H == 0 || K == 0) {
        c->cnt.seed_ms += (wall() - t0) * 1e3;
        return;
    }
    u32 pmaxq = 0;
    for (u32 q = qa; q < qb;) {
        if ((q & 255u) == 0 && q + 256u <= qb) pmaxq = std::max(pmaxq, b.blkmax[q >> 8]), q += 256u;
        else pmaxq = std::max(pmaxq, b.h_off[q + 1] - b.h_off[q]), ++q;
    }
    KeyLayout kl;
    kl.bq = ceil_log2((u64)b.nq + 1);
    kl.bp = ceil_log2(std::max<u32>(pmaxq, 2));
    kl.ba = AS > 1 ? ceil_log2((u64)AS) : 0;
    const bool force_wide = tune().lk_wide;
    const bool bands_ok = tune().bands;
    if (tune().bucket && c->count_tab_now && AS == 1 && !force_wide && !ch.ordered &&
        (u64)H * 1024ull >= (u64)std::max(1ll, tune().bucket_min) * (u64)(qb - qa) * (u64)std::max<u32>(nseq_chunk, 1))
        order_chunk(c, ch);
    ChunkIndex::BandEnc* enc = force_wide ? nullptr : band_encoding(c, ch, kl.ba, kl.bp, AS == 1 && bands_ok);
    const bool compact = enc != nullptr;
    const u32 nunit = compact ? enc->nband : nseq_chunk;
    if (compact) {
        kl.bs = ceil_log2(std::max<u32>(enc->nband, 2));
        kl.bd = enc->k;
        kl.diag_off = enc->C;
    } else {
        kl.bs = ceil_log2(nseq_chunk);
        kl.bd = ceil_log2((u64)pmaxq + ch.maxslen + 1);
        kl.diag_off = ch.maxslen;
    }
    kl.finish();
    KeyLayout klr = kl;
    const void* btab = nullptr;
    if (compact && enc->multi) {
        klr.bs = ceil_log2(nseq_chunk);
        klr.bd = ceil_log2((u64)pmaxq + ch.maxslen + 1);
        klr.diag_off = ch.maxslen;
        klr.finish();
        btab = enc->btab.p;
    }
    const u32 gallop_min = 1024;
    const int bsp = ceil_log2((u64)ch.maxslen + 1);
    const int ft_bits_entry = (klr.bs + 1) + klr.ba + bsp;
    const bool ft_walk = AS > 1;
    if (kl.total > 64) throw SoError("sort key needs " + std::to_string(kl.total) + " bits (> 64): lower SOHIT_BATCH or -c");
    if (klr.sh_subj + klr.bs > 64) throw SoError("pass-record key exceeds 64 bits: sequences too long for this build");
    if (kl.ba + kl.bp + ft_bits_entry > 64) throw SoError("first-touch key exceeds 64 bits: sequences too long for this build");
    b.cs_hoff.ensure((size_t)K + 2), b.cs_beg.ensure((size_t)K + 2), b.cs_kbase.ensure((size_t)K + 2);
    launch_compact_seeds(b.mark.p, b.scnt.p, b.hoff.p, b.cidx.p, b.sbeg.p, b.dev.d_pseq.p, b.dev.d_off.p, p_lo, p_hi, AS, kl, b.cs_hoff.p, b.cs_beg.p,
                         b.cs_kbase.p, c->st);
    const u32* dk32 = compact ? enc->dk32.p : nullptr;
    if (!compact && (ch.d_sh_subj != kl.sh_subj || ch.d_sh_diag != kl.sh_diag)) {
        ch.dkeys.ensure((size_t)ch.E + 2);
        launch_encode_delta(ch.entries.p, ch.E, kl.sh_subj, kl.sh_diag, ch.maxslen, ch.dkeys.p, c->st);
        ch.d_sh_subj = kl.sh_subj, ch.d_sh_diag = kl.sh_diag;
    }
    const u32 shard_cap = ungap_shard_cap(H);
    const size_t pcap = (size_t)shard_cap * UG_SHARDS + 2 + ungap1_list_slack(c->ncu);
    b.p_qs.ensure(pcap), b.p_sd.ensure(pcap), b.p_ft.ensure(pcap);
    b.shard.ensure(2 * UG_SHARDS + 8);
    b.stepshard.ensure(UG_SHARDS + 4);
    b.bflag.ensure(8);
    double t1 = wall();
    bool bbest = false;
    BktLayout bL;
    u32 bnb = 0;
    memset(&bL, 0, sizeof bL);
    unsigned long long* const ugstat = c->tune.count_steps ? b.stepshard.p + UG_SHARDS : nullptr;
    auto reset_pass_lists = [&] {
        HIP_CHECK(hipMemsetAsync(b.shard.p, 0, (2 * UG_SHARDS + 8) * sizeof(u32), c->st));
        HIP_CHECK(hipMemsetAsync(b.stepshard.p, 0, (UG_SHARDS + 4) * sizeof(unsigned long long), c->st));
        HIP_CHECK(hipMemsetAsync(b.bflag.p, 0, 8 * sizeof(u32), c->st));
    };

    auto group_bucketed = [&]() -> bool {
        const bool enabled = tune().bucket;
        if (!enabled || AS != 1 || !compact || UG_SHARDS != 1) return false;
        const u32 nqp = qb - qa;
        const int wb_hi = std::min(std::min(31 - kl.bd - kl.bp, kl.bs), bkt_max_wb());
        int wb_lo = 0;
        while (((u64)nunit + (1ull << wb_lo) - 1) >> wb_lo > BKT_RMAX) ++wb_lo;
        if (wb_hi < wb_lo || kl.bp > 16) return false;
        const u32 target = (u32)std::max(1ll, tune().bucket_avg);
        int wb = wb_hi;
        const u32 sparse = (u32)std::max(0ll, tune().bucket_min);
        if ((u64)H / ((u64)nqp * (((u64)nunit + (1ull << wb) - 1) >> wb)) < sparse) return false;
        while (wb > wb_lo && (u64)H / ((u64)nqp * (((u64)nunit + (1ull << wb) - 1) >> wb)) > target) --wb;
        BktLayout L;
        L.wb = wb, L.bd = kl.bd, L.bp = kl.bp, L.sh_q = kl.sh_q, L.sh_qpos = kl.sh_qpos, L.nqp = nqp, L.qa = qa;
        L.R = (u32)(((u64)nunit + (1ull << wb) - 1) >> wb);
        L.maxslen = ch.maxslen;
        if ((u64)L.R * nqp >= 0xFFFFFFF0ull) return false;
        const u32 nb = L.R * nqp;
        b.qseg.ensure((size_t)b.nq + 4);
        launch_query_segments(b.hoff.p, b.dev.d_off.p, qa, qb, AS, H, b.qseg.p, c->st);
        const u32* qseg = b.qseg.p + qa;
        b.bt0.ensure((size_t)nqp + 4);
        launch_bkt_ntiles(qseg, nqp, b.bt0.p, c->st);
        c->d_scan_tmp.ensure(scan_u32_temp_elems((size_t)nqp + 1) + 8);
        const u32 NT = d2h_u32(c, scan_u32(b.bt0.p, b.bt0.p, (size_t)nqp + 1, false, c->d_scan_tmp.p, c->st));
        if ((u64)L.R * NT >= 0xFFFFFFF0ull) return false;
        b.btd.ensure(4 * (size_t)NT + 8);
        launch_bkt_tiledesc(qseg, b.bt0.p, nqp, NT, b.cs_hoff.p, K, b.btd.p, c->st);
        const size_t nm = (size_t)L.R * NT;
        b.bmat.ensure(nm + 4);
        {
            const ChunkIndex::RangeTab* rt = (c->count_tab_now && ch.ordered) ? range_table(c, ch, *enc, wb, L.R) : nullptr;
            const bool tab = rt && rt->ok;
            ProfTimer pt(c, &c->cnt.count_ms, &c->cnt.count_launches);
            if (tab) launch_bkt_count_tab(b.btd.p, qseg, b.bt0.p, nqp, NT, b.cs_hoff.p, b.cs_beg.p, ch.row_of_slot.p, rt->tab.p, L.R, b.bmat.p, c->st);
            else launch_bkt_pass(false, b.btd.p, qseg, NT, b.cs_hoff.p, b.cs_beg.p, b.cs_kbase.p, dk32, c->ref.d_off.p + ch.seq_lo, L, b.bmat.p, nullptr, c->st);
            pt.stop();
            if (tab && c->profile) c->tm["seed.bucket_count_tab_launches"] += 1;
            if (tab && tune().count_tab == 2) {
                b.bpart.ensure(nm + 4);
                launch_bkt_pass(false, b.btd.p, qseg, NT, b.cs_hoff.p, b.cs_beg.p, b.cs_kbase.p, dk32, c->ref.d_off.p + ch.seq_lo, L, b.bpart.p, nullptr, c->st);
                c->d_small.ensure(SM_WORDS);
                HIP_CHECK(hipMemsetAsync(c->d_small.p + SM_FLAG, 0, sizeof(u32), c->st));
                launch_u32_differ(b.bmat.p, b.bpart.p, nm, c->d_small.p + SM_FLAG, c->st);
                const u32 nd = d2h_u32(c, c->d_small.p + SM_FLAG);
                if (nd) throw SoError("range-table counts differ from the counting pass in " + std::to_string(nd) + " cells");
            }
        }
        const size_t npart = (size_t)L.R * bkt_scan_blocks(NT);
        b.bpart.ensure(npart + 4);
        c->d_scan_tmp.ensure(scan_u32_temp_elems(npart + 1) + 8);
        launch_bkt_colsum(b.bmat.p, NT, L.R, b.bpart.p, c->st);
        const u32* dHv = scan_u32(b.bpart.p, b.bpart.p, npart, false, c->d_scan_tmp.p, c->st);
        stash_u32(c, dHv, SM_SEED_TOTAL);
        launch_bkt_colscan(b.bmat.p, NT, L.R, b.bpart.p, c->st);
        const u32 Hv = d2h_u32(c, c->d_small.p + SM_SEED_TOTAL);
        sc.lap("seed.bucket_count");
        b.hits32.ensure((size_t)H + 2);
        {
            ProfTimer pt(c, &c->cnt.lookup_ms, &c->cnt.lookup_launches);
            launch_bkt_pass(true, b.btd.p, qseg, NT, b.cs_hoff.p, b.cs_beg.p, b.cs_kbase.p, dk32, c->ref.d_off.p + ch.seq_lo, L, b.bmat.p,
                            b.hits32.p, c->st);
            pt.stop();
            if (c->profile) c->cnt.lookup_bytes += (i64)8 * (i64)H;
        }
        t1 = wall();
        sc.lap("seed.bucket_scatter");
        const bool w32 = tune().ug_w32;
        if (w32) b.hits32s.ensure((size_t)H + 8);
        else b.keys2.ensure((size_t)H + 2);
        b.bext.ensure((size_t)nb + 4);
        launch_bkt_extents(b.bmat.p, b.bt0.p, NT, L.R, nqp, nb, c->d_small.p + SM_SEED_TOTAL, b.bext.p, c->st);
        {
            ProfTimer pt(c, &c->cnt.bgroup_ms, &c->cnt.bgroup_launches);
            launch_bkt_group(b.hits32.p, b.bext.p, nb, L, kl, w32 ? nullptr : b.keys2.p, w32 ? b.hits32s.p : nullptr, b.bflag.p, c->st);
            pt.stop();
        }
        const u32 refused = d2h_u32(c, b.bflag.p);
        sc.lap("group.bucket_group");
        if (refused) {
            if (tune().debug) fprintf(stderr, "[sohit] bucketed pass refused (flag %u): sorted path\n", refused);
            return false;
        }
        if (tune().debug) fprintf(stderr, "[sohit] bucketed pass: wb %d ranges %u buckets %u tiles %u hits %u of %u\n", wb, L.R, nb, NT, Hv, H);
        bbest = tune().bucket_best && !ft_walk && (kl.ba + kl.bp + ft_bits_entry <= 44) &&
                (u64)std::min<u32>(pmaxq, ch.maxslen) * 11ull < (1ull << 20);
        const bool ug1 = w32 && c->tune.ug1 && pmaxq <= ungap1_qcap() && bbest;
        const bool ug2 = ug1 && c->tune.ug1_chain;
        if (ug1 && !c->ref.ug_valid) {
            const size_t nres = c->ref.res.size();
            c->ref.d_ug_store.ensure(nres + 2 * (size_t)U1_UG_PAD);
            launch_make_ug(c->ref.d_scls.p, c->ref.d_off.p, (u32)c->ref.N, nres, 8u, c->ref.d_ug_store.p + U1_UG_PAD, c->st);
            c->ref.ug_valid = true;
        }
        if (ug2) {
            if (!b.dev.ug_valid) {
                const size_t nres = b.h_off[b.nq];
                b.dev.d_ug_store.ensure(nres + 2 * (size_t)U1_UG_PAD);
                launch_make_ug(b.dev.d_scls.p, b.dev.d_off.p, b.nq, nres, 1u, b.dev.d_ug_store.p + U1_UG_PAD, c->st);
                b.dev.ug_valid = true;
            }
            b.mlist.ensure(ungap1_mlist_cap(Hv, c->ncu));
        }
        if (ug1)
            launch_ungap1(c->ncu, pmaxq, b.hits32s.p, b.bext.p, nb, L, kl, klr, btab, U1_WAIT, b.dev.d_scls.p, b.dev.d_off.p,
                          c->ref.d_ug_store.p + U1_UG_PAD, c->ref.d_off.p + ch.seq_lo, c->d_b62c.p, b.bflag.p + 1, b.shard.p, b.p_qs.p, b.p_sd.p, b.p_ft.p, b.stepshard.p,
                          ug2 ? b.mlist.p : nullptr, b.bflag.p + 3, ugstat, c->st);
        if (ug2)
            launch_ungap2(c->ncu, b.mlist.p, b.bflag.p + 3, b.hits32s.p, b.bext.p, L, kl, klr, btab, U1_WAIT, b.dev.d_ug_store.p + U1_UG_PAD, b.dev.d_off.p,
// ... 47 lines not shown
    sc.lap("seed.compact_lookup");
    const int seg_mode = (int)tune().segsort;
    if (seg_mode && nseg >= 256) {
        ensure_sort_tmp(c, sort_keys_u64_seg_temp_bytes(H, nseg, kl.sh_diag, kl.sh_q));
        if (uq) sort_keys_u64_seg2(c->d_sort_tmp.p, c->d_sort_tmp.cap, b.keys.p, b.keys2.p, H, nseg, b.qseg.p + qa, b.flags.p, kl.sh_diag, kl.sh_q, c->st);
        else sort_keys_u64_seg(c->d_sort_tmp.p, c->d_sort_tmp.cap, b.keys.p, b.keys2.p, H, nseg, b.qseg.p + qa, kl.sh_diag, kl.sh_q, c->st);
    } else {
    ensure_sort_tmp(c, sort_keys_u64_temp_bytes(H, kl.total));
    sort_keys_u64(c->d_sort_tmp.p, c->d_sort_tmp.cap, b.keys.p, b.keys2.p, H, kl.sh_diag, kl.total, c->st);
    }
    sc.lap("group.sort_keys");
    launch_ungap(b.keys2.p, H, kl, klr, btab, pmaxq >= gallop_min, ft_walk, b.dev.d_scls.p, b.dev.d_off.p, c->ref.d_scls4.p, c->ref.d_off.p + ch.seq_lo,
                 c->d_b62c.p, b.shard.p, shard_cap, b.p_qs.p, b.p_sd.p, b.p_ft.p, b.stepshard.p, c->st, nullptr, nullptr, 0, nullptr, false, ugstat);
    };

    reset_pass_lists();
    if (!group_bucketed()) {
        bbest = false;
        group_sorted();
    }
    u64* c_ftp = nullptr;
    u32 *c_qp = nullptr, *c_recp = nullptr;
    u32 NS = 0, maxseg = 0xFFFFFFFFu;
    int cand_idx_bits = 0, cand_ftw = 0;
    for (;;) {
        u32* shard_off = b.shard.p + UG_SHARDS;
        launch_shard_scan(b.shard.p, shard_off, c->st);
        u32 NP;
        {
            static_assert((UG_SHARDS + 4) * sizeof(unsigned long long) + sizeof(u32) <= 1024, "h_small too small");
            unsigned long long* gc = (unsigned long long*)small_host(c);
            u32* np = (u32*)(gc + UG_SHARDS + 4);
            HIP_CHECK(hipMemcpyAsync(gc, b.stepshard.p, (UG_SHARDS + 4) * sizeof(unsigned long long), hipMemcpyDeviceToHost, c->st));
            HIP_CHECK(hipMemcpyAsync(np, shard_off + UG_SHARDS, sizeof(u32), hipMemcpyDeviceToHost, c->st));
            HIP_CHECK(hipStreamSynchronize(c->st));
            for (int k = 0; k < UG_SHARDS; ++k) c->cnt.groups += (i64)gc[k];
            c->cnt.ungap_steps += (i64)gc[UG_SHARDS], c->cnt.groups_single += (i64)gc[UG_SHARDS + 1], c->cnt.groups_chain += (i64)gc[UG_SHARDS + 2];
            NP = *np;
        }
        sc.lap("group.ungap");
        const u64 *q_qs = b.p_qs.p, *q_sd = b.p_sd.p, *q_ft = b.p_ft.p;
        if (NP && UG_SHARDS > 1) {
            b.q_qs.ensure((size_t)NP + 2), b.q_sd.ensure((size_t)NP + 2), b.q_ft.ensure((size_t)NP + 2);
            launch_compact_shards(b.shard.p, shard_off, shard_cap, b.p_qs.p, b.p_sd.p, b.p_ft.p, b.q_qs.p, b.q_sd.p, b.q_ft.p, c->st);
            q_qs = b.q_qs.p, q_sd = b.q_sd.p, q_ft = b.q_ft.p;
        }
        if (bbest && NP) {
            static_assert(UG_SHARDS == 1, "the bucketed best-diagonal path reads one contiguous pass list");
            b.bcnt.ensure((size_t)bnb + 2), b.bccnt.ensure((size_t)bnb + 2), b.pidx.ensure((size_t)NP + 2);
            b.q_qs.ensure((size_t)NP + 2), b.q_sd.ensure((size_t)NP + 2), b.q_ft.ensure((size_t)NP + 2);
            c->d_scan_tmp.ensure(scan_u32_temp_elems((size_t)bnb + 2) + 8);
            HIP_CHECK(hipMemsetAsync(b.bcnt.p, 0, ((size_t)bnb + 2) * sizeof(u32), c->st));
            launch_rec_count(b.p_qs.p, NP, klr.bs, bL, b.bcnt.p, b.pidx.p, c->st);
            scan_u32(b.bcnt.p, b.bcnt.p, (size_t)bnb + 1, false, c->d_scan_tmp.p, c->st);
            launch_rec_scatter(b.p_qs.p, b.p_sd.p, b.p_ft.p, b.pidx.p, NP, klr, bL, ft_bits_entry, bsp, c->ref.d_off.p + ch.seq_lo, b.bcnt.p, b.q_qs.p,
                               b.q_sd.p, b.q_ft.p, c->st);
            HIP_CHECK(hipMemsetAsync(b.bccnt.p + bnb, 0, 2 * sizeof(u32), c->st));
            launch_bkt_best(false, b.q_qs.p, b.q_sd.p, b.q_ft.p, b.bcnt.p, bnb, bL, klr.bs, (u32)ch.seq_lo, b.bccnt.p, nullptr, nullptr, nullptr, bsp, 0,
                            c->st);
            NS = d2h_u32(c, scan_u32(b.bccnt.p, b.bccnt.p, (size_t)bnb + 1, false, c->d_scan_tmp.p, c->st));
            if (tune().debug)
                fprintf(stderr, "[sohit] seed pass: queries %u..%u hits %u seeds %u pass records %u candidates %u (bucketed best)\n", qa, qb, H, K, NP, NS);
            b.c_ft.ensure((size_t)NS + 2), b.c_q.ensure((size_t)NS + 2), b.c_rec.ensure(4 * (size_t)NS + 8);
            c_ftp = b.c_ft.p, c_qp = b.c_q.p, c_recp = b.c_rec.p;
            {
                const int ftw = kl.ba + kl.bp + ft_bits_entry - bsp + 1;
                if (bL.nqp >= 256 && ftw < 63 && 63 - ftw >= klr.bs + 1) cand_idx_bits = 63 - ftw, cand_ftw = ftw;
            }
            launch_bkt_best(true, b.q_qs.p, b.q_sd.p, b.q_ft.p, b.bcnt.p, bnb, bL, klr.bs, (u32)ch.seq_lo, b.bccnt.p, c_ftp, c_qp, c_recp, bsp,
                            cand_idx_bits, c->st);
            break;
        }
        if (NP) launch_first_touch(ft_walk, b.keys2.p, H, klr, ft_bits_entry, bsp, c->ref.d_off.p + ch.seq_lo, const_cast<u64*>(q_ft), NP, c->st);
        if (NP == 0) break;
        if (pmaxq < 4096 && (kl.ba + kl.bp + ft_bits_entry) - bsp + 1 <= cand_order_lds_key_bits() && qb > qa) {
            const u32 nqp = qb - qa;
            BktLayout Lq{};
            Lq.wb = 31, Lq.nqp = nqp, Lq.qa = qa, Lq.R = 1;
            b.bcnt.ensure((size_t)nqp + 2), b.bccnt.ensure((size_t)nqp + 2), b.pidx.ensure((size_t)NP + 2), b.pidx2.ensure((size_t)NP + 2);
            b.order.ensure((size_t)NP + 2), b.order2.ensure((size_t)NP + 2), b.p_qs2.ensure((size_t)NP + 2), b.tmp64.ensure((size_t)NP + 2);
            b.c_rec.ensure(4 * (size_t)NP + 8), b.bflag.ensure(4);
            c->d_scan_tmp.ensure(scan_u32_temp_elems((size_t)nqp + 2) + 8);
            HIP_CHECK(hipMemsetAsync(b.bcnt.p, 0, ((size_t)nqp + 2) * sizeof(u32), c->st));
            launch_rec_count(q_qs, NP, klr.bs, Lq, b.bcnt.p, b.pidx.p, c->st);
            scan_u32(b.bcnt.p, b.bcnt.p, (size_t)nqp + 1, false, c->d_scan_tmp.p, c->st);
            launch_qrec_scatter(q_qs, q_sd, q_ft, b.pidx.p, NP, klr.bs, qa, b.bcnt.p, b.pidx2.p , b.order.p , b.p_qs2.p ,
                                b.tmp64.p , c->st);
            HIP_CHECK(hipMemsetAsync(b.bflag.p, 0, sizeof(u32), c->st));
            launch_q_best(b.bcnt.p, qa, nqp, b.order.p, b.p_qs2.p, b.tmp64.p, (u32)ch.seq_lo, bsp, b.c_rec.p, b.order2.p, qcnt, b.bflag.p, c->st);
            HIP_CHECK(hipMemcpyAsync(b.bccnt.p, qcnt + qa, (size_t)nqp * sizeof(u32), hipMemcpyDeviceToDevice, c->st));
            HIP_CHECK(hipMemsetAsync(b.bccnt.p + nqp, 0, 2 * sizeof(u32), c->st));
            const u32* dT = scan_u32(b.bccnt.p, b.bccnt.p, (size_t)nqp + 1, false, c->d_scan_tmp.p, c->st);
            stash_u32(c, dT, SM_STASH0);
            u32 flag = 0;
            d2h_pair(c, b.bflag.p, NS, flag);
            if (!flag) {
                if (tune().debug) fprintf(stderr, "[sohit] seed pass: queries %u..%u hits %u seeds %u pass records %u candidates %u (per query)\n", qa, qb, H, K, NP, NS);
                if (NS) {
                    const u32 base = b.chunk_base.back();
                    if ((u64)base + NS >= cand_limit()) throw CandOverflow();
                    b.cand_q.ensure((size_t)base + NS + 4, true, c->st);
                    b.cand_rec.ensure(4 * ((size_t)base + NS) + 16, true, c->st);
                    launch_q_emit(b.bcnt.p, qa, nqp, NP, b.pidx2.p, qcnt, b.bccnt.p, b.order2.p, b.c_rec.p, b.cand_q.p + base, b.cand_rec.p + 4 * (size_t)base, c->st);
                    b.chunk_base.back() = base + NS;
                    c->cnt.candidates += NS;
                }
                sc.lap("group.best_order");
                c->cnt.seed_ms += (t1 - t0) * 1e3;
                c->cnt.group_ms += (wall() - t1) * 1e3;
                return;
            }
            NS = 0;
        }
        b.pidx.ensure((size_t)NP + 2), b.pidx2.ensure((size_t)NP + 2), b.p_qs2.ensure((size_t)NP + 2);
        launch_iota(b.pidx.p, NP, c->st);
        ensure_sort_tmp(c, sort_pairs_u64_u32_temp_bytes(NP, 64));
        sort_pairs_u64_u32(c->d_sort_tmp.p, c->d_sort_tmp.cap, q_qs, b.p_qs2.p, b.pidx.p, b.pidx2.p, NP, klr.bs + kl.bq, c->st);
        b.flags.ensure((size_t)NP + 4), b.gidx.ensure((size_t)NP + 4);
        c->d_small.ensure(SM_WORDS);
        launch_seg_flags(b.p_qs2.p, NP, b.flags.p, c->d_small.p + SM_STASH0, c->st);
        const u32* dS = scan_u32(b.flags.p, b.gidx.p, NP, false, c->d_scan_tmp.p, c->st);
        b.qseg.ensure((size_t)b.nq + 4);
        launch_qseg(b.p_qs2.p, NP, b.gidx.p, dS, klr.bs, qa, qb, b.qseg.p, c->d_small.p + SM_STASH0, c->st);
        d2h_pair(c, dS, maxseg, NS);
        b.shead.ensure((size_t)NS + 2);
        if (tune().debug) fprintf(stderr, "[sohit] seed pass: queries %u..%u hits %u seeds %u pass records %u candidates %u\n", qa, qb, H, K, NP, NS);
        launch_group_list(b.flags.p, b.gidx.p, NP, b.shead.p, c->st);
        b.c_ft.ensure((size_t)NS + 2), b.c_q.ensure((size_t)NS + 2), b.c_rec.ensure(4 * (size_t)NS + 8);
        c_ftp = b.c_ft.p, c_qp = b.c_q.p, c_recp = b.c_rec.p;
        launch_best(b.p_qs2.p, b.pidx2.p, b.shead.p, NS, NP, q_sd, q_ft, (u32)ch.seq_lo, klr.bs, c_ftp, c_qp, c_recp, c->st);
        break;
    }
    if (NS == 0) {
        c->cnt.seed_ms += (t1 - t0) * 1e3;
        c->cnt.group_ms += (wall() - t1) * 1e3;
        return;
    }
    const int ftbits = kl.ba + kl.bp + ft_bits_entry;
    if (!bbest && maxseg <= (u32)cand_order_lds_max() && ftbits - bsp + 1 <= cand_order_lds_key_bits()) {
        const u32 base = b.chunk_base.back();
        if ((u64)base + NS >= cand_limit()) throw CandOverflow();
        b.cand_q.ensure((size_t)base + NS + 4, true, c->st);
        b.cand_rec.ensure(4 * ((size_t)base + NS) + 16, true, c->st);
        launch_cand_order_lds(c_ftp, c_recp, b.qseg.p, qa, qb, maxseg, bsp, b.cand_q.p + base, b.cand_rec.p + 4 * (size_t)base, qcnt, c->st);
        b.chunk_base.back() = base + NS;
        c->cnt.candidates += NS;
        sc.lap("group.best_order");
        c->cnt.seed_ms += (t1 - t0) * 1e3;
        c->cnt.group_ms += (wall() - t1) * 1e3;
        return;
    }
    if (cand_idx_bits) {
        const u32 base = b.chunk_base.back();
        if ((u64)base + NS >= cand_limit()) throw CandOverflow();
        b.qseg.ensure((size_t)b.nq + 4), b.tmp64.ensure((size_t)NS + 2);
        launch_stride_gather(b.bccnt.p, bL.R, bL.nqp + 1, b.qseg.p, c->st);
        b.cand_q.ensure((size_t)base + NS + 4, true, c->st);
        b.cand_rec.ensure(4 * ((size_t)base + NS) + 16, true, c->st);
        HIP_CHECK(hipMemsetAsync(b.bflag.p, 0, sizeof(u32), c->st));
        launch_cand_order_seg(c_ftp, b.qseg.p, bL.nqp, bL.qa, cand_idx_bits, cand_idx_bits + cand_ftw, c_recp, b.cand_q.p + base, b.cand_rec.p + 4 * (size_t)base,
                              qcnt, b.bflag.p, c->st);
        if (d2h_u32(c, b.bflag.p) != 0) {
            ensure_sort_tmp(c, sort_cand_keys_seg_temp_bytes(NS, bL.nqp, cand_idx_bits, cand_idx_bits + cand_ftw));
            sort_cand_keys_seg(c->d_sort_tmp.p, c->d_sort_tmp.cap, c_ftp, b.tmp64.p, NS, bL.nqp, b.qseg.p, cand_idx_bits, cand_idx_bits + cand_ftw, c->st);
            launch_emit_cands_seg(b.tmp64.p, b.qseg.p, bL.nqp, bL.qa, cand_idx_bits, c_recp, b.cand_q.p + base, b.cand_rec.p + 4 * (size_t)base, qcnt, c->st);
        }
        b.chunk_base.back() = base + NS;
        c->cnt.candidates += NS;
        sc.lap("group.best_order");
        c->cnt.seed_ms += (t1 - t0) * 1e3;
        c->cnt.group_ms += (wall() - t1) * 1e3;
        return;
    }
    b.order.ensure((size_t)NS + 2), b.order2.ensure((size_t)NS + 2), b.tmp64.ensure((size_t)NS + 2), b.c_ft2.ensure((size_t)NS + 2);
    launch_iota(b.order.p, NS, c->st);
    int qshift = 0;
    if (ftbits + kl.bq <= 64) {
// ... 25 lines not shown
```

swiftortho_amd/csrc/k_util.hip:

```cpp
#include "common.h"
#include "kernels.h"

#define SCAN_THREADS 256
#define SCAN_ITERS 8
#define SCAN_TILE (SCAN_THREADS * 4 * SCAN_ITERS)

__device__ __forceinline__ uint4 ld4(const u32* p) {
    uint4 v;
    __builtin_memcpy(&v, p, 16);
    return v;
}
__device__ __forceinline__ void st4(u32* p, const uint4& v) { __builtin_memcpy(p, &v, 16); }

__device__ __forceinline__ u32 wave_incl_scan_u32(u32 v, int lane) {
#pragma unroll
    for (int o = 1; o < 64; o <<= 1) {
        u32 t = __shfl_up(v, o);
        if (lane >= o) v += t;
    }
    return v;
}

__device__ __forceinline__ u32 block_excl_scan_u32(u32 v, u32* lds4, u32* total) {
    const int lane = threadIdx.x & 63, w = threadIdx.x >> 6;
    u32 inc = wave_incl_scan_u32(v, lane);
    if (lane == 63) lds4[w] = inc;
    __syncthreads();
    u32 base = 0, tot = 0;
#pragma unroll
    for (int k = 0; k < SCAN_THREADS / 64; ++k) {
        u32 s = lds4[k];
        if (k < w) base += s;
        tot += s;
    }
    __syncthreads();
    *total = tot;
    return base + inc - v;
}

__global__ __launch_bounds__(SCAN_THREADS) void k_scan_reduce(const u32* __restrict__ in, size_t n, u32* __restrict__ blocksums) {
    __shared__ u32 lds4[4];
    size_t base = (size_t)blockIdx.x * SCAN_TILE;
    u32 s = 0;
#pragma unroll
    for (int it = 0; it < SCAN_ITERS; ++it) {
        size_t i = base + (size_t)it * SCAN_THREADS * 4 + (size_t)threadIdx.x * 4;
        if (i + 3 < n) {
            uint4 v = ld4(in + i);
            s += v.x + v.y + v.z + v.w;
        } else {
            for (int k = 0; k < 4; ++k)
                if (i + k < n) s += in[i + k];
        }
    }
    u32 tot;
    block_excl_scan_u32(s, lds4, &tot);
    if (threadIdx.x == 0) blocksums[blockIdx.x] = tot;
}

__global__ __launch_bounds__(SCAN_THREADS) void k_scan_blocksums(u32* __restrict__ blocksums, size_t nb) {
    __shared__ u32 lds4[4];
    u32 carry = 0;
    for (size_t b0 = 0; b0 < nb; b0 += SCAN_THREADS) {
        size_t i = b0 + threadIdx.x;
        u32 v = i < nb ? blocksums[i] : 0;
        u32 tot;
        u32 ex = block_excl_scan_u32(v, lds4, &tot);
        if (i < nb) blocksums[i] = carry + ex;
        carry += tot;
    }
    if (threadIdx.x == 0) blocksums[nb] = carry;
}

__global__ __launch_bounds__(SCAN_THREADS) void k_scan_apply(const u32* __restrict__ in, u32* __restrict__ out, size_t n,
                                                             const u32* __restrict__ blocksums, int inclusive) {
    __shared__ u32 lds4[4];
    size_t base = (size_t)blockIdx.x * SCAN_TILE;
    u32 carry = blocksums[blockIdx.x];
#pragma unroll 1
    for (int it = 0; it < SCAN_ITERS; ++it) {
        size_t i = base + (size_t)it * SCAN_THREADS * 4 + (size_t)threadIdx.x * 4;
        u32 a = 0, b = 0, c = 0, d = 0;
        if (i + 3 < n) {
            uint4 v = ld4(in + i);
            a = v.x, b = v.y, c = v.z, d = v.w;
        } else {
            if (i < n) a = in[i];
            if (i + 1 < n) b = in[i + 1];
            if (i + 2 < n) c = in[i + 2];
            if (i + 3 < n) d = in[i + 3];
        }
        u32 s = a + b + c + d, tot;
        u32 ex = carry + block_excl_scan_u32(s, lds4, &tot);
        u32 o0, o1, o2, o3;
        if (inclusive) o0 = ex + a, o1 = o0 + b, o2 = o1 + c, o3 = o2 + d;
        else o0 = ex, o1 = ex + a, o2 = o1 + b, o3 = o2 + c;
        if (i + 3 < n) {
            st4(out + i, make_uint4(o0, o1, o2, o3));
        } else {
            if (i < n) out[i] = o0;
            if (i + 1 < n) out[i + 1] = o1;
            if (i + 2 < n) out[i + 2] = o2;
            if (i + 3 < n) out[i + 3] = o3;
        }
        carry += tot;
    }
}

__device__ __forceinline__ u64 wave_incl_scan_u64(u64 v, int lane) {
#pragma unroll
    for (int o = 1; o < 64; o <<= 1) {
        const u64 t = __shfl_up((unsigned long long)v, o);
        if (lane >= o) v += t;
    }
    return v;
}
__device__ __forceinline__ u64 block_excl_scan_u64(u64 v, u64* lds4, u64* total) {
    const int lane = threadIdx.x & 63, w = threadIdx.x >> 6;
    const u64 inc = wave_incl_scan_u64(v, lane);
    if (lane == 63) lds4[w] = inc;
    __syncthreads();
    u64 base = 0, tot = 0;
#pragma unroll
    for (int k = 0; k < SCAN_THREADS / 64; ++k) {
        const u64 s = lds4[k];
        if (k < w) base += s;
        tot += s;
    }
    __syncthreads();
    *total = tot;
    return base + inc - v;
}
__device__ __forceinline__ uint4 eff4(const u8* __restrict__ mark, const u32* __restrict__ scnt, size_t i, size_t n) {
    uint4 c = make_uint4(0, 0, 0, 0);
    if (i + 3 < n) {
        u32 m;
        __builtin_memcpy(&m, mark + i, 4);
        const uint4 v = ld4(scnt + i);
        c.x = (m & 0xFFu) ? v.x : 0u, c.y = (m & 0xFF00u) ? v.y : 0u, c.z = (m & 0xFF0000u) ? v.z : 0u, c.w = (m & 0xFF000000u) ? v.w : 0u;
    } else {
        if (i < n) c.x = mark[i] ? scnt[i] : 0u;
        if (i + 1 < n) c.y = mark[i + 1] ? scnt[i + 1] : 0u;
        if (i + 2 < n) c.z = mark[i + 2] ? scnt[i + 2] : 0u;
    }
    return c;
}
__device__ __forceinline__ u64 pair4(const uint4& c) {
    return ((u64)((c.x != 0) + (c.y != 0) + (c.z != 0) + (c.w != 0)) << 32) + (u64)c.x + c.y + c.z + c.w;
}

__global__ __launch_bounds__(SCAN_THREADS) void k_effscan_reduce(const u8* __restrict__ mark, const u32* __restrict__ scnt, size_t n,
                                                                 u64* __restrict__ blocksums) {
    __shared__ u64 lds4[4];
    const size_t base = (size_t)blockIdx.x * SCAN_TILE;
    u64 s = 0;
#pragma unroll
    for (int it = 0; it < SCAN_ITERS; ++it) s += pair4(eff4(mark, scnt, base + (size_t)it * SCAN_THREADS * 4 + (size_t)threadIdx.x * 4, n));
    u64 tot;
    block_excl_scan_u64(s, lds4, &tot);
    if (threadIdx.x == 0) blocksums[blockIdx.x] = tot;
}

__global__ __launch_bounds__(SCAN_THREADS) void k_scan_blocksums64(u64* __restrict__ blocksums, size_t nb) {
    __shared__ u64 lds4[4];
    u64 carry = 0;
    for (size_t b0 = 0; b0 < nb; b0 += SCAN_THREADS) {
        const size_t i = b0 + threadIdx.x;
        const u64 v = i < nb ? blocksums[i] : 0;
        u64 tot;
        const u64 ex = block_excl_scan_u64(v, lds4, &tot);
        if (i < nb) blocksums[i] = carry + ex;
        carry += tot;
    }
    if (threadIdx.x == 0) blocksums[nb] = carry;
}

__global__ __launch_bounds__(SCAN_THREADS) void k_effscan_apply(const u8* __restrict__ mark, const u32* __restrict__ scnt, size_t n,
                                                                const u64* __restrict__ blocksums, u32* __restrict__ hoff, u32* __restrict__ cidx) {
    __shared__ u64 lds4[4];
    const size_t base = (size_t)blockIdx.x * SCAN_TILE;
    u64 carry = blocksums[blockIdx.x];
#pragma unroll 1
    for (int it = 0; it < SCAN_ITERS; ++it) {
        const size_t i = base + (size_t)it * SCAN_THREADS * 4 + (size_t)threadIdx.x * 4;
        const uint4 c = eff4(mark, scnt, i, n);
        u64 tot;
        const u64 ex = carry + block_excl_scan_u64(pair4(c), lds4, &tot);
        const u32 h0 = (u32)ex, h1 = h0 + c.x, h2 = h1 + c.y, h3 = h2 + c.z;
        const u32 k0 = (u32)(ex >> 32), k1 = k0 + (c.x != 0), k2 = k1 + (c.y != 0), k3 = k2 + (c.z != 0);
        if (i + 3 < n) {
            st4(hoff + i, make_uint4(h0, h1, h2, h3));
            st4(cidx + i, make_uint4(k0, k1, k2, k3));
        } else {
            if (i < n) hoff[i] = h0, cidx[i] = k0;
            if (i + 1 < n) hoff[i + 1] = h1, cidx[i + 1] = k1;
            if (i + 2 < n) hoff[i + 2] = h2, cidx[i + 2] = k2;
        }
        carry += tot;
    }
}

size_t effscan_temp_elems(size_t n) { return 2 * ((n + SCAN_TILE - 1) / SCAN_TILE + 2) + 2; }

const u32* effscan(const u8* mark, const u32* scnt, size_t n, u32* hoff, u32* cidx, u32* temp, hipStream_t st) {
    const size_t nb = (n + SCAN_TILE - 1) / SCAN_TILE;
    u64* t64 = reinterpret_cast<u64*>(temp);
    if (nb == 0) {
        HIP_CHECK(hipMemsetAsync(t64, 0, sizeof(u64), st));
        return temp;
    }
    hipLaunchKernelGGL(k_effscan_reduce, dim3((unsigned)nb), dim3(SCAN_THREADS), 0, st, mark, scnt, n, t64);
    hipLaunchKernelGGL(k_scan_blocksums64, dim3(1), dim3(SCAN_THREADS), 0, st, t64, nb);
    hipLaunchKernelGGL(k_effscan_apply, dim3((unsigned)nb), dim3(SCAN_THREADS), 0, st, mark, scnt, n, t64, hoff, cidx);
    return reinterpret_cast<const u32*>(t64 + nb);
}

#define SS_THREADS 1024
#define SS_ITEMS 16
__global__ __launch_bounds__(SS_THREADS) void k_scan_small(const u32* __restrict__ in, u32* __restrict__ out, size_t n, u32* __restrict__ total,
                                                           int inclusive) {
    __shared__ u32 s_w[SS_THREADS / 64];
    const int lane = threadIdx.x & 63, w = threadIdx.x >> 6;
    u32 carry = 0;
    for (size_t i0 = 0; i0 < n; i0 += (size_t)SS_THREADS * SS_ITEMS) {
        const size_t i = i0 + (size_t)threadIdx.x * SS_ITEMS;
        u32 v[SS_ITEMS];
        if (i + SS_ITEMS <= n) {
#pragma unroll
            for (int k = 0; k < SS_ITEMS; k += 4) {
                const uint4 x = ld4(in + i + k);
                v[k] = x.x, v[k + 1] = x.y, v[k + 2] = x.z, v[k + 3] = x.w;
            }
        } else {
#pragma unroll
            for (int k = 0; k < SS_ITEMS; ++k) v[k] = i + k < n ? in[i + k] : 0u;
        }
        u32 s = 0;
#pragma unroll
        for (int k = 0; k < SS_ITEMS; ++k) s += v[k];
        const u32 inc = wave_incl_scan_u32(s, lane);
        if (lane == 63) s_w[w] = inc;
        __syncthreads();
        u32 base = 0, tot = 0;
#pragma unroll
        for (int k = 0; k < SS_THREADS / 64; ++k) {
            const u32 x = s_w[k];
            base += k < w ? x : 0u;
            tot += x;
        }
        __syncthreads();
        u32 run = carry + base + inc - s;
#pragma unroll
        for (int k = 0; k < SS_ITEMS; ++k) {
            const u32 x = v[k];
            v[k] = inclusive ? run + x : run;
            run += x;
        }
        if (i + SS_ITEMS <= n) {
#pragma unroll
            for (int k = 0; k < SS_ITEMS; k += 4) st4(out + i + k, make_uint4(v[k], v[k + 1], v[k + 2], v[k + 3]));
        } else {
#pragma unroll
            for (int k = 0; k < SS_ITEMS; ++k)
                if (i + k < n) out[i + k] = v[k];
        }
        carry += tot;
    }
    if (threadIdx.x == 0) *total = carry;
}
#define SCAN_SMALL_TILES 4

size_t scan_u32_temp_elems(size_t n) { return (n + SCAN_TILE - 1) / SCAN_TILE + 2; }

const u32* scan_u32(const u32* in, u32* out, size_t n, bool inclusive, u32* temp, hipStream_t st) {
    size_t nb = (n + SCAN_TILE - 1) / SCAN_TILE;
    if (nb == 0) {
        HIP_CHECK(hipMemsetAsync(temp, 0, sizeof(u32), st));
        return temp;
    }
    if (nb <= SCAN_SMALL_TILES) {
        hipLaunchKernelGGL(k_scan_small, dim3(1), dim3(SS_THREADS), 0, st, in, out, n, temp + nb, inclusive ? 1 : 0);
        return temp + nb;
    }
    hipLaunchKernelGGL(k_scan_reduce, dim3((unsigned)nb), dim3(SCAN_THREADS), 0, st, in, n, temp);
    hipLaunchKernelGGL(k_scan_blocksums, dim3(1), dim3(SCAN_THREADS), 0, st, temp, nb);
    hipLaunchKernelGGL(k_scan_apply, dim3((unsigned)nb), dim3(SCAN_THREADS), 0, st, in, out, n, temp, inclusive ? 1 : 0);
    return temp + nb;
}

__global__ void k_fill_u32(u32* p, size_t n, u32 v) {
    size_t i = (size_t)blockIdx.x * blockDim.x + threadIdx.x;
    if (i < n) p[i] = v;
}

void fill_u32(u32* p, size_t n, u32 v, hipStream_t st) {
    if (!n) return;
    hipLaunchKernelGGL(k_fill_u32, dim3((unsigned)((n + 255) / 256)), dim3(256), 0, st, p, n, v);
}

__global__ __launch_bounds__(256) void k_query_segments(const u32* __restrict__ hoff, const u32* __restrict__ qoff, u32 qa, u32 qb, int AS,
                                                        u32 H, u32* __restrict__ seg ) {
    const u32 q = qa + blockIdx.x * 256u + threadIdx.x;
    if (q > qb) return;
    const size_t t = ((size_t)qoff[q] + q) * (size_t)AS;
    seg[q] = q < qb ? hoff[t] : H;
}

void launch_query_segments(const u32* hoff, const u32* qoff, u32 qa, u32 qb, int AS, u32 H, u32* seg, hipStream_t st) {
    hipLaunchKernelGGL(k_query_segments, dim3((qb - qa + 1 + 255) / 256), dim3(256), 0, st, hoff, qoff, qa, qb, AS, H, seg);
}
```

swiftortho_amd/csrc/kernels.h:

```cpp
#pragma once
#include "common.h"

struct HashLut;

size_t scan_u32_temp_elems(size_t n);
size_t effscan_temp_elems(size_t n);
const u32* effscan(const u8* mark, const u32* scnt, size_t n, u32* hoff, u32* cidx, u32* temp, hipStream_t st);
const u32* scan_u32(const u32* in, u32* out, size_t n, bool inclusive, u32* temp, hipStream_t st);
void fill_u32(u32* p, size_t n, u32 v, hipStream_t st);

size_t sort_keys_u64_temp_bytes(size_t n, int bits);
void sort_keys_u64(void* temp, size_t temp_bytes, const u64* in, u64* out, size_t n, int begin_bit, int end_bit, hipStream_t st);
void launch_query_segments(const u32* hoff, const u32* qoff, u32 qa, u32 qb, int AS, u32 H, u32* seg, hipStream_t st);
size_t sort_keys_u64_seg_temp_bytes(size_t n, u32 nseg, int begin_bit, int end_bit);
void sort_keys_u64_seg(void* temp, size_t temp_bytes, const u64* in, u64* out, size_t n, u32 nseg, const u32* seg, int begin_bit,
                       int end_bit, hipStream_t st);
void sort_keys_u64_seg2(void* temp, size_t temp_bytes, const u64* in, u64* out, size_t n, u32 nseg, const u32* seg_begin, const u32* seg_end, int begin_bit,
                        int end_bit, hipStream_t st);
void launch_stride_gather(const u32* src, u32 stride, u32 n, u32* dst, hipStream_t st);
size_t sort_pairs_u64_u32_temp_bytes(size_t n, int bits);
void sort_pairs_u64_u32(void* temp, size_t temp_bytes, const u64* kin, u64* kout, const u32* vin, u32* vout, size_t n, int bits,
                        hipStream_t st);
size_t sort_pairs_u64_u64_temp_bytes(size_t n, int bits);
void sort_pairs_u64_u64(void* temp, size_t temp_bytes, const u64* kin, u64* kout, const u64* vin, u64* vout, size_t n, int bits,
                        hipStream_t st);

size_t ixsort_plan_elems(u32 NC);
void ixsort_pairs(u32* kin, u64* vin, u32 E, u32 NC, u32* plan, u32* scan_tmp, u32* tk, u64* tv, u32* kout, u64* vout, hipStream_t st);
const u32* ixsort_count(const u32* kin, u32 n, u32 NC, u32* plan, u32* scan_tmp, hipStream_t st);
void ixsort_finish(u32* kin, u64* vin, u32 n, u32 NC, const u32* plan, u32* tk, u64* tv, u32* kout, u64* vout, hipStream_t st);
void launch_index_windows_sparse(const u32* words, const u32* pseq, const u32* off, u32 p_lo, u32 p_hi, u32 Ppad, u32 seq_lo, const SeedCfg& cfg, const HashLut& lut, u32 step,
                                 u32* bkt, u64* ent, hipStream_t st);

void launch_layout(const u8* res, const u32* off, u32 nseq, u32 P, u32 Ppad, const u8* hmap, u32* pseq, u8* pcls, u32* words,
                   hipStream_t st);
#define PCLS_PAD 48
struct AlnSide { const u8 *res, *scls, *scls4, *pcls, *pcls4; const u32 *off, *bound; };
struct AlnSeqs { AlnSide q, r; const signed char* b62 ; };
void launch_pad_cls(const u8* scls, const u32* off, u32 nseq, u8* out , u8* out4,
                    hipStream_t st);
#define SCLS_PAD_FRONT 16
#define SCLS_PAD_BACK 64
void launch_scls(const u8* res, size_t n, const u8* smap, u8* scls, u8* scls4 , hipStream_t st);
void launch_seq_bound(const u8* scls, const u32* off, u32 nseq, const signed char* b62c_host, u32* bound, hipStream_t st);
void launch_seg(const u8* raw, const u32* src_off, u32 q_lo, const u32* qid, u32 nq, const u32* dst_off, const u8* symmap, const u8* upmap,
                const void* tab, u8* mk, u8* out, u32 max_len, u32 q_mid, u32 q_long, hipStream_t st, hipStream_t st_long);
void launch_gather_seqs(const u8* raw, const u32* src_off, u32 q_lo, const u32* qid, u32 nq, const u32* dst_off, u8* out, hipStream_t st);
void launch_copy_range(const u8* src, u8* dst, size_t n, hipStream_t st);

#define HTAB_EMPTY 0xFFFFFFFFu
void launch_run_heads(const u32* bkt, u32 E, u32* flags, hipStream_t st);
void launch_run_list(const u32* bkt, const u32* flags, const u32* ridx, u32 E, u32 U, u32* ub, u32* ubeg, u32* cnt, hipStream_t st);
void launch_dir_build(const u32* ub, u32 U, u64* dir , hipStream_t st);
void launch_htab_insert(const u32* ub, const u32* ubeg, u32 U, u32* hkey, u64* hval, int hshift, u32 hmask, hipStream_t st);
#define INDEX_STATS_BLOCKS 2048
void launch_index_stats(const u32* counts, u32 NC, u64* stats_buf , hipStream_t st);
void launch_encode_band32(const u64* entries, u32 E, int ba, const u32* gbase , const u32* roff , u32* dk32, hipStream_t st);
void launch_encode_delta(const u64* entries, u32 E, int sh_subj, int sh_diag, u32 maxslen, u64* dkeys, hipStream_t st);
void launch_index_fixlast(u64* entries, u32 lo, u32 E, hipStream_t st);

void launch_qhash(const u32* words, u32 Ppad, const SeedCfg& cfg, const HashLut& lut, u32* qbucket, hipStream_t st);
// ... 172 lines not shown
```

swiftortho_amd/csrc/tune.h:

```cpp
#pragma once
#include <cstdlib>

#define SOHIT_TUNE_TABLE(X)                                                                                                                                     \
                                                                                                                              \
    X(B, ug1, "SOHIT_UG1", 1, "bucketed passes: singleton groups to k_ungap1 (0: everything to k_ungap)")                                                     \
    X(B, ug1_chain, "SOHIT_UG1_CHAIN", 1, "... and the groups of two and more hits to k_ungap2 (0: to k_ungap, which then skips the singletons)")              \
    X(B, count_steps, "SOHIT_UG_COUNT", 0, "counting instances of the extension kernels: so_counters.ungap_steps, groups_single, groups_chain")                \
    X(B, ungapq, "SOHIT_UNGAPQ", 1, "sparse passes of queries up to 512 residues: hits alone on their diagonal by k_ungapq, a wave per query (0: every hit through the sorted keys)")     \
    X(B, ug_w32, "SOHIT_UG_W32", 1, "bucketed passes hand k_ungap the buckets' 32-bit words (0: 64-bit keys; no k_ungap1 then)")                               \
                                                                                                             \
    X(B, bucket, "SOHIT_BUCKET", 1, "bucketed diagonal binning (0: every pass on the sorted path)")                                                            \
    X(I, bucket_min, "SOHIT_BUCKET_MIN", 192, "hits per bucket below which a pass takes the sorted path (0: bucketed whenever possible)")                      \
    X(I, bucket_avg, "SOHIT_BUCKET_AVG", 2560, "average bucket size the band-range width is chosen for")                                                       \
    X(I, count_tab, "SOHIT_COUNT_TAB", 1, "bucketed passes: hits per (tile, range) from the range boundaries of the ordered index buckets when a batch brings a chunk two passes and more (0: always the counting pass over the entries; 2: always both, compared -- tests; 3: always)") \
    X(B, bucket_best, "SOHIT_BUCKET_BEST", 1, "best diagonal per subject by the per-bucket reduction (0: sort of the pass records)")                           \
    X(B, bands, "SOHIT_BANDS", 1, "diagonal bands follow the subjects' lengths (0: one band per subject)")                                                     \
    X(B, lk_wide, "SOHIT_LK_WIDE", 0, "8-byte index addends whatever the field widths")                                                                        \
    X(B, qclass, "SOHIT_QCLASS", 1, "queries of a batch in length-class order (0: file order)")                                                                \
    X(B, pass_merge, "SOHIT_PASS_MERGE", 1, "neighbouring length classes that take the sorted path anyway share one pass")                                     \
    X(B, ksc_lazy, "SOHIT_KSC_LAZY", 1, "k-mer orders computed for the queries that reach their frequency cap, when they do (a query below it keeps every window whatever the order; 0: for every query, with the batch)") \
    X(B, bounds_ahead, "SOHIT_BOUNDS_AHEAD", 1, "the next chunk's bucket bounds (k_bounds) on the side stream beside this chunk's seed stage (0: in front of its own)")     \
    X(I, segsort, "SOHIT_SEGSORT", 1, "sorted path: segmented sort of the keys inside each query (0: device-wide sort)")                                        \
    X(I, write_threads, "SOHIT_WRITE_THREADS", 48, "so_write_sc: formatter threads (at most the host's cores)")                                                                          \
                                                                                                                                 \
    X(I, cand_limit, "SOHIT_CAND_LIMIT", 0, "tests: candidate-store size at which a batch is split (0: 2^32 - 16)")                                            \
                                                                                                                                         \
    X(B, align_pk, "SOHIT_ALIGN_PK", 1, "packed 16-bit score-only aligner where the scores fit")                                                               \
    X(B, align_lane, "SOHIT_ALIGN_LANE", 1, "score-only rounds: one lane per alignment pair (k_align_lane) when no sequence reaches 4096 residues (0: k_align_pk)")            \
    X(I, align_lane_min, "SOHIT_ALIGN_LANE_MIN", 1 << 18, "... for rounds of at least this many packed tasks (below: k_align_pk; tests: 0)")                 \
    X(B, align_sort, "SOHIT_ALIGN_SORT", 1, "launch lists ordered by band rows")                                                                               \
    X(I, trace_wave_rows, "SOHIT_TRACE_WAVE_ROWS", 1024, "traceback: bands of this many rows and more are walked by a wave of their own (0: never)")         \
    X(I, trace_wave_max, "SOHIT_TRACE_WAVE_MAX", 32768, "... among the first this many positions of a launch list")                                            \
    X(I, spec, "SOHIT_SPEC", -1, "speculative traces in the first round: 0 off, 1 on, -1 from 2^21 tasks on")                                                  \
    X(D, spec_slack, "SOHIT_SPEC_SLACK", 1e6, "... the guess tests the ungapped score against expect x this (tests: 1e30 = every first-round task traced, 1e-30 = none)")          \
    X(I, spec_cap, "SOHIT_SPEC_CAP", -1, "tests: most speculative traces kept (-1: all)")                                                                      \
    X(I, trace_var_max, "SOHIT_TRACE_VAR_MAX", -1, "tests: trace words a launch list's own-size traces may take, and the fixed-stride slabs' budget (-1: 2^31 / 2^30)") \
    X(I, emit_parts, "SOHIT_EMIT_PARTS", 4, "... and otherwise")                                                                                               \
    X(I, emit_min_rows, "SOHIT_EMIT_MIN_ROWS", 1 << 18, "rows below which the emission is one part")                                                           \
    X(P, test_oom_phase2, "SOHIT_TEST_OOM_PHASE2", 0, "tests: phase 2 of the first batch fails once with an out-of-memory error")                              \
                                                                                                                                 \
    X(I, batch, "SOHIT_BATCH", 0, "queries per device batch (0: 131072, lowered when the candidate estimate asks)")                                            \
    X(I, max_hits, "SOHIT_MAX_HITS", 0, "seed hits per pass (0: 2^30)")                                                                                        \
    X(I, poison, "SOHIT_POISON", -1, "tests: byte every fresh device allocation is filled with (-1: none)")                                                    \
    X(B, hit_cache, "SOHIT_HIT_CACHE", 1, "one released result array is kept for the next search")                                                             \
    X(P, keep_cands, "SOHIT_KEEP_CANDS", 0, "tests: keep every query's candidate list (so_query_candidates)")                                                  \
    X(P, keep_masked, "SOHIT_KEEP_MASKED", 0, "tests: keep the masked queries (so_masked_query)")                                                              \
    X(I, mcl_scratch, "SOHIT_MCL_SCRATCH", -1, "tests: u32 words of expansion / convergence scratch per range of rows (-1: 2^28)")                             \
                                                                                      \
    X(T, orth_tier, "SOHIT_ORTH_TIER", 0, "tests: every run of query rows through one tier of k_orth_run wherever that tier can take it (0 = auto: by run length)") \
                                                                                                                                           \
    X(P, exact_threshold, "SOHIT_EXACT_THRESHOLD", 0, "threshold always by the sequential fp64 replay")                                                        \
    X(I, dir_max, "SOHIT_DIR_MAX", -1, "largest -M served by the bitmap + rank directory (-1: 2^31)")                                                          \
                                                                                                                                          \
    X(P, debug, "SOHIT_DEBUG", 0, "per-pass lines on stderr")                                                                                                  \
    X(P, debug_index, "SOHIT_DEBUG_INDEX", 0, "wall laps of the index build on stderr")

#define ORTH_WAVE_ROWS 64
#define ORTH_LDS_ROWS 1024
#define ORTH_LDS_TAXA 512
enum { ORTH_TIER_AUTO = 0, ORTH_TIER_WAVE = 1, ORTH_TIER_LDS = 2, ORTH_TIER_SCRATCH = 3 };
static inline int orth_tier_of(const char* v) {
    switch (v[0]) {
        case 'w': case '1': return ORTH_TIER_WAVE;
        case 'l': case '2': return ORTH_TIER_LDS;
        case 's': case '3': return ORTH_TIER_SCRATCH;
        default: return ORTH_TIER_AUTO;
    }
}

struct Tune {
#define X_B(f, d) bool f = (d) != 0;
#define X_I(f, d) long long f = (d);
#define X_D(f, d) double f = (d);
#define X_P(f, d) bool f = false;
#define X_T(f, d) int f = (d);
#define X(kind, field, env, dflt, text) X_##kind(field, dflt)
    SOHIT_TUNE_TABLE(X)
#undef X
#undef X_B
#undef X_I
#undef X_D
#undef X_P
#undef X_T
    void read() {
#define X_B(f, e) if (const char* v = getenv(e)) f = atoi(v) != 0;
#define X_I(f, e) if (const char* v = getenv(e)) f = strtoll(v, nullptr, 0);
#define X_D(f, e) if (const char* v = getenv(e)) f = atof(v);
#define X_P(f, e) f = getenv(e) != nullptr;
#define X_T(f, e) if (const char* v = getenv(e)) f = orth_tier_of(v);
#define X(kind, field, env, dflt, text) X_##kind(field, env)
        SOHIT_TUNE_TABLE(X)
#undef X
// ... 11 lines not shown
```

Baseline: 671.9 M query-aa/s.

## Chain device scans by decoupled look-back and write host-read totals to pinned words

Replaces the three-launch reduce / block-sums / apply prefix scan with a single-launch chained scan that uses decoupled look-back across tiles, with the three-launch path kept as a fallback. Scan totals and counts that the host waits on are written by the computing kernel directly into pinned host words, instead of being stashed in a device word and copied back with a memcpy plus stream sync. The aim is to cut kernel launches and device-to-host round-trips on the many small scans in phase 2 and index build. In exchange it adds persistent ticket and status buffers, epoch management, spin limits with an error fallback, and a test entry point.

```diff
diff --git a/include/sohit.h b/include/sohit.h
--- a/include/sohit.h
+++ b/include/sohit.h
@@ -125,6 +125,7 @@
 int so_chunk_download(so_ctx *ctx, int64_t chunk, uint32_t *start, uint64_t *entries);
 int64_t so_masked_query(so_ctx *ctx, int64_t qidx, char *buf, int64_t cap);
 int64_t so_query_candidates(so_ctx *ctx, int64_t qidx, uint32_t *out4, int64_t cap);
+int so_scan_test(so_ctx *ctx, int kind, int inclusive, int64_t n, int offset, const void *in, void *out, uint32_t *total);
 int so_align_pairs(so_ctx *ctx, int kernel, int64_t n, const int64_t *task6, const uint32_t *order, int32_t *out);
 int so_align_pairs_aln(so_ctx *ctx, int kernel, int64_t n, const int64_t *task6, const uint32_t *order, int32_t *out, char **aln,
                        int64_t *aln_bytes);
diff --git a/swiftortho_amd/_lib.py b/swiftortho_amd/_lib.py
--- a/swiftortho_amd/_lib.py
+++ b/swiftortho_amd/_lib.py
@@ -44,7 +44,7 @@
 EXPORTS = ["so_abi_version", "so_set_option", "so_create", "so_destroy", "so_last_error", "so_load_ref", "so_load_ref_mem", "so_build_index", "so_drop_index", "so_load_index",
            "so_load_queries", "so_load_queries_mem", "so_num_queries", "so_num_refs", "so_query_len", "so_search_loaded",
            "so_search", "so_free_hits", "so_search_loaded_aln", "so_free_aln", "so_write_sc", "so_format_hit", "so_get_counters", "so_reset_counters", "so_timing_report",
-           "so_chunk_threshold", "so_chunk_entries", "so_chunk_download", "so_masked_query", "so_query_candidates", "so_align_pairs", "so_align_pairs_aln", "so_set_profile",
+           "so_chunk_threshold", "so_chunk_entries", "so_chunk_download", "so_masked_query", "so_query_candidates", "so_scan_test", "so_align_pairs", "so_align_pairs_aln", "so_set_profile",
            "so_bucket_count", "so_ref_len", "so_search_device", "so_device_hits_copy", "so_query_work", "so_mcl", "so_mcl_free",
            "so_mcl_last_error", "so_tsv_lines", "so_tsv_scan", "so_tsv_codes", "so_format_pairs", "so_py_repr", "so_fmt_rows",
            "so_search_loaded_cigar", "so_free_cigar", "so_format_cigar", "so_write_sc_cigar", "so_align_pairs_cigar",
@@ -165,6 +165,7 @@
     L.so_masked_query.argtypes = [vp, i64, cp, i64]
     L.so_query_candidates.restype = i64
     L.so_query_candidates.argtypes = [vp, i64, vp, i64]
+    L.so_scan_test.argtypes = [vp, C.c_int, C.c_int, i64, C.c_int, vp, vp, vp]
     L.so_align_pairs.argtypes = [vp, C.c_int, i64, vp, vp, vp]
     L.so_align_pairs_aln.argtypes = [vp, C.c_int, i64, vp, vp, vp, C.POINTER(C.c_void_p), C.POINTER(i64)]
     L.so_mcl.argtypes = [C.c_int, i64, vp, vp, vp, C.c_double, C.c_int32, C.c_int32, C.c_double, C.c_double, C.c_double, C.POINTER(SoMclResult)]
diff --git a/swiftortho_amd/csrc/host.h b/swiftortho_amd/csrc/host.h
--- a/swiftortho_amd/csrc/host.h
+++ b/swiftortho_amd/csrc/host.h
@@ -235,6 +235,10 @@
     unsigned long long* h_qhits = nullptr;
     size_t h_qhits_cap = 0;
     unsigned long long* h_small = nullptr;
+    u32* hw_dev = nullptr;
+    ScanChain scan;
+    bool scan_fallback_told = false;
+    struct { const u32* in = nullptr; u32* out = nullptr; size_t n = 0; bool inclusive = false; int slot = -1; u32 epoch = 0; } scan_last;
     std::map<std::string, double> tm;
     std::map<std::string, double> lt;
     std::shared_ptr<void> batch;
@@ -603,6 +607,18 @@
 u32 d2h_u32(so_ctx* c, const u32* p);
 void stash_u32(so_ctx* c, const u32* p, int slot);
 void d2h_pair(so_ctx* c, const u32* second, u32& a, u32& b);
+enum { HW_SCAN_ERR = SM_WORDS, HW_WORDS = SM_WORDS + 16 };
+u32* host_words(so_ctx* c);
+u32* host_word_dev(so_ctx* c, int k);
+ScanChain* scan_chain(so_ctx* c);
+const u32* ctx_scan(so_ctx* c, const u32* in, u32* out, size_t n, bool inclusive, int slot = -1);
+const u32* ctx_effscan(so_ctx* c, const u8* mark, const u32* scnt, size_t n, u32* hoff, u32* cidx);
+void fetch_word(so_ctx* c, const u32* dev, int slot, int n = 1);
+const u32* read_slots(so_ctx* c, int lo, int n);
+inline u32 scan_total(so_ctx* c, const u32* in, u32* out, size_t n, bool inclusive) {
+    ctx_scan(c, in, out, n, inclusive, SM_STASH0);
+    return read_slots(c, SM_STASH0, 1)[SM_STASH0];
+}
 void ensure_sort_tmp(so_ctx* c, size_t bytes);
 const unsigned long long* chunk_qhits(so_ctx* c, Batch& b, int ci);
 void chunk_qhits_deferred(so_ctx* c, Batch& b, int ci);
diff --git a/swiftortho_amd/csrc/host_abi.hip b/swiftortho_amd/csrc/host_abi.hip
--- a/swiftortho_amd/csrc/host_abi.hip
+++ b/swiftortho_amd/csrc/host_abi.hip
@@ -177,6 +177,7 @@
     if (c->pinned) (void)hipHostFree(c->pinned);
     if (c->pinned_aln) (void)hipHostFree(c->pinned_aln);
     if (c->h_small) (void)hipHostFree(c->h_small);
+    scan_chain_release(c->scan);
     if (c->h_qhits) (void)hipHostFree(c->h_qhits);
     if (c->ev0) (void)hipEventDestroy(c->ev0);
     if (c->ev1) (void)hipEventDestroy(c->ev1);
@@ -609,6 +610,37 @@
     return n;
 }
 
+int so_scan_test(so_ctx* c, int kind, int inclusive, int64_t n, int offset, const void* in, void* out, uint32_t* total) {
+    return guarded(c, [&] {
+        if (n < 0 || offset < 0 || offset > 3 || kind < 0 || kind > 2) throw SoError("so_scan_test: bad arguments");
+        const size_t N = (size_t)n;
+        DevBuf<u32> d_in, d_out;
+        DevBuf<u8> d_mark;
+        d_in.ensure(N + 8), d_out.ensure(2 * N + 16);
+        u32 *pi = d_in.p + offset, *po = d_out.p + offset;
+        if (N) HIP_CHECK(hipMemcpyAsync(pi, in, N * sizeof(u32), hipMemcpyHostToDevice, c->st));
+        if (kind == 1) {
+            d_mark.ensure(N + 8);
+            u8* pm = d_mark.p + offset;
+            u32* po2 = po + N + 4;
+            if (N) HIP_CHECK(hipMemcpyAsync(pm, (const u32*)in + N, N, hipMemcpyHostToDevice, c->st));
+            c->d_scan_tmp.ensure(effscan_temp_elems(N) + 8);
+            ctx_effscan(c, pm, pi, N, po, po2);
+            const u32* v = read_slots(c, 0, 0);
+            total[0] = v[SM_STASH0], total[1] = v[SM_STASH1];
+            if (N) {
+                HIP_CHECK(hipMemcpy(out, po, N * sizeof(u32), hipMemcpyDeviceToHost));
+                HIP_CHECK(hipMemcpy((u32*)out + N, po2, N * sizeof(u32), hipMemcpyDeviceToHost));
+            }
+            return;
+        }
+        c->d_scan_tmp.ensure(scan_u32_temp_elems(N) + 8);
+        u32* dst = kind == 2 ? pi : po;
+        total[0] = scan_total(c, pi, dst, N, inclusive != 0);
+        if (N) HIP_CHECK(hipMemcpy(out, dst, N * sizeof(u32), hipMemcpyDeviceToHost));
+    });
+}
+
 int so_align_pairs(so_ctx* c, int kernel, int64_t n, const int64_t* task6, const uint32_t* order, int32_t* out) {
     return guarded(c, [&] { align_pairs(c, kernel, n, task6, order, out); });
 }
diff --git a/swiftortho_amd/csrc/host_index.hip b/swiftortho_amd/csrc/host_index.hip
--- a/swiftortho_amd/csrc/host_index.hip
+++ b/swiftortho_amd/csrc/host_index.hip
@@ -124,7 +124,7 @@
             c->ix_flags.ensure((size_t)E + 4), c->ix_ridx.ensure((size_t)E + 4);
             c->d_scan_tmp.ensure(scan_u32_temp_elems((size_t)E + 1) + 8);
             launch_run_heads(c->ix_bkt2.p, E, c->ix_flags.p, c->st);
-            const u32 U = d2h_u32(c, scan_u32(c->ix_flags.p, c->ix_ridx.p, E, false, c->d_scan_tmp.p, c->st));
+            const u32 U = scan_total(c, c->ix_flags.p, c->ix_ridx.p, E, false);
             ch->U = U;
             ch->ub.ensure((size_t)U + 4), ch->ubeg.ensure((size_t)U + 4), ch->ucnt.ensure((size_t)U + 4);
             launch_run_list(c->ix_bkt2.p, c->ix_flags.p, c->ix_ridx.p, E, U, ch->ub.p, ch->ubeg.p, ch->ucnt.p, c->st);
diff --git a/swiftortho_amd/csrc/host_phase2.hip b/swiftortho_amd/csrc/host_phase2.hip
--- a/swiftortho_amd/csrc/host_phase2.hip
+++ b/swiftortho_amd/csrc/host_phase2.hip
@@ -70,7 +70,7 @@
     c->d_scan_tmp.ensure(scan_u32_temp_elems((size_t)n + 1) + 8);
     if ((u64)n * 129u >= (1ull << 30)) throw SoError("alignments: more than 8 M reported rows in one batch; search a smaller query range per call");
     launch_aln_units(tasks, list, n, s, a.units.p, c->st);
-    const size_t units = d2h_u32(c, scan_u32(a.units.p, a.rofs.p, (size_t)n + 1, false, c->d_scan_tmp.p, c->st));
+    const size_t units = scan_total(c, a.units.p, a.rofs.p, (size_t)n + 1, false);
     a.slot_words = units * aln_unit_words();
     a.code.ensure(a.slot_words + 64);
     launch_aln_scatter(list, n, a.rofs.p, a.aofs.p, c->st);
@@ -78,7 +78,7 @@
 static size_t aln_compact(so_ctx* c, AlnChain& a, const u32* list, u32 n, const AlnRes* res) {
     a.words.ensure((size_t)n + 4), a.cofs.ensure((size_t)n + 4);
     launch_aln_words(list, n, res, a.words.p, c->st);
-    const size_t words = d2h_u32(c, scan_u32(a.words.p, a.cofs.p, (size_t)n + 1, false, c->d_scan_tmp.p, c->st));
+    const size_t words = scan_total(c, a.words.p, a.cofs.p, (size_t)n + 1, false);
     a.comp.ensure(words + 64);
     launch_aln_compact(list, n, a.aofs.p, a.code.p, a.cofs.p, a.comp.p, c->st);
     return words;
@@ -87,7 +87,7 @@
     if (a.slot_words * 16ull >= (1ull << 32)) throw SoError("CIGARs: the reported rows of one batch hold 2^32 columns or more; search a smaller query range per call");
     a.runs.ensure((size_t)n + 4), a.oofs.ensure((size_t)n + 4);
     launch_cigar_count(list, n, a.aofs.p, a.code.p, res, a.runs.p, c->st);
-    const size_t n_ops = d2h_u32(c, scan_u32(a.runs.p, a.oofs.p, (size_t)n + 1, false, c->d_scan_tmp.p, c->st));
+    const size_t n_ops = scan_total(c, a.runs.p, a.oofs.p, (size_t)n + 1, false);
     a.ops.ensure(n_ops + 64);
     launch_cigar_emit(list, n, a.aofs.p, a.code.p, res, a.oofs.p, a.ops.p, c->st);
     return n_ops;
@@ -122,14 +122,14 @@
     HIP_CHECK(hipMemsetAsync(b.qtot.p, 0, ((size_t)nq + 4) * sizeof(u32), c->st));
     for (int ci = 0; ci < nchunks; ++ci) launch_add_u32(b.qtot.p, b.ccnt.p + (size_t)ci * nq, nq, c->st);
     c->d_scan_tmp.ensure(scan_u32_temp_elems((size_t)nq + 1) + 8);
-    scan_u32(b.qtot.p, b.qcoff.p, (size_t)nq + 1, false, c->d_scan_tmp.p, c->st);
+    ctx_scan(c, b.qtot.p, b.qcoff.p, (size_t)nq + 1, false);
     b.fin_rec.ensure(4 * (size_t)Ntot + 16);
     HIP_CHECK(hipMemsetAsync(b.prior.p, 0, ((size_t)nq + 4) * sizeof(u32), c->st));
     for (int ci = 0; ci < nchunks; ++ci) {
         const u32 lo = ci == 0 ? 0u : b.chunk_base[ci - 1], hi = b.chunk_base[ci];
         const u32* cc = b.ccnt.p + (size_t)ci * nq;
         if (hi > lo) {
-            scan_u32(cc, b.cqoff.p, nq, false, c->d_scan_tmp.p, c->st);
+            ctx_scan(c, cc, b.cqoff.p, nq, false);
             launch_gather_cands(b.cand_q.p + lo, b.cand_rec.p + 4 * (size_t)lo, hi - lo, b.cqoff.p, b.prior.p, b.qcoff.p, b.fin_rec.p,
                                 c->st);
         }
@@ -183,11 +183,13 @@
         HIP_CHECK(hipEventRecord(c->ev_ug_done, c->st_side));
         HIP_CHECK(hipStreamWaitEvent(c->st, c->ev_ug_done, 0));
     }
-    const u32* dNRk = scan_u32(b.ntask.p, b.roffc.p, (size_t)nq + 1, false, c->d_scan_tmp.p, c->st);
-    stash_u32(c, dNRk, SM_STASH0);
-    const u32* dNT = scan_u32(b.ntile.p, b.toff.p, (size_t)nq + 1, false, c->d_scan_tmp.p, c->st);
+    ctx_scan(c, b.ntask.p, b.roffc.p, (size_t)nq + 1, false, SM_STASH0);
+    ctx_scan(c, b.ntile.p, b.toff.p, (size_t)nq + 1, false, SM_STASH1);
     u32 NRK;
-    d2h_pair(c, dNT, NRK, p.NT);
+    {
+        const u32* v = read_slots(c, SM_STASH0, 2);
+        NRK = v[SM_STASH0], p.NT = v[SM_STASH1];
+    }
     const u32 NT = p.NT;
     p.sc.lap("phase2.csort");
     b.tasks.ensure((size_t)NT + 4), b.ares.ensure((size_t)NT + 4), b.bits.ensure((size_t)NT + 4), b.sel.ensure((size_t)NT + 4);
@@ -241,7 +243,7 @@
     b.tr_units.ensure((size_t)n + 4), b.tr_ofs.ensure((size_t)n + 4);
     c->d_scan_tmp.ensure(scan_u32_temp_elems((size_t)n + 1) + 8);
     launch_trace_units(b.tasks.p, list, n, p.seqs, b.tr_units.p, c->st);
-    return (size_t)d2h_u32(c, scan_u32(b.tr_units.p, b.tr_ofs.p, (size_t)n + 1, false, c->d_scan_tmp.p, c->st)) * p.TU;
+    return (size_t)scan_total(c, b.tr_units.p, b.tr_ofs.p, (size_t)n + 1, false) * p.TU;
 }
 
 static void align_rounds(so_ctx* c, Batch& b, P2& p) {
@@ -268,11 +270,10 @@
             launch_round_counts_spec(b.ntask.p, b.ntile.p, b.roffc.p, b.rk_slot.p, b.qcoff.p, b.st_state.p, nq, c->max_miss, minr, b.tasks.p, b.toff.p,
                                      b.dev.d_off.p, c->ref.d_off.p, c->d_bittab.p, so_ctx::BITTAB_N, c->ref.N, c->expect * spec_slack, b.rcnt.p, b.tcnt.p, b.spcnt.p,
                                      c->d_small.p + SM_ANY_RANK, c->st);
-            stash_u32(c, scan_u32(b.tcnt.p, b.roff.p, (size_t)nq + 1, false, c->d_scan_tmp.p, c->st), SM_STASH0);
-            stash_u32(c, scan_u32(b.spcnt.p, b.spoff.p, (size_t)nq + 1, false, c->d_scan_tmp.p, c->st), SM_STASH1);
-            u32* v = (u32*)small_host(c);
-            HIP_CHECK(hipMemcpyAsync(v, c->d_small.p, (SM_ANY_RANK + 1) * sizeof(u32), hipMemcpyDeviceToHost, c->st));
-            HIP_CHECK(hipStreamSynchronize(c->st));
+            ctx_scan(c, b.tcnt.p, b.roff.p, (size_t)nq + 1, false, SM_STASH0);
+            ctx_scan(c, b.spcnt.p, b.spoff.p, (size_t)nq + 1, false, SM_STASH1);
+            fetch_word(c, c->d_small.p + SM_ANY_RANK, SM_ANY_RANK);
+            const u32* v = read_slots(c, SM_STASH0, 2);
             NR = v[SM_STASH0], NS = v[SM_STASH1], RR = v[SM_ANY_RANK];
             if (NS > spec_cap) spec_round = false;
         }
@@ -280,10 +281,10 @@
             NS = 0;
             launch_round_counts(b.ntask.p, b.ntile.p, b.roffc.p, b.rk_slot.p, b.qcoff.p, b.st_state.p, nq, c->max_miss, minr, b.rcnt.p,
                                 b.tcnt.p, c->st);
-            const u32* dNR = scan_u32(b.tcnt.p, b.roff.p, (size_t)nq + 1, false, c->d_scan_tmp.p, c->st);
-            stash_u32(c, dNR, SM_STASH0);
-            const u32* dRR = scan_u32(b.rcnt.p, b.order_tmp.p, (size_t)nq + 1, false, c->d_scan_tmp.p, c->st);
-            d2h_pair(c, dRR, NR, RR);
+            ctx_scan(c, b.tcnt.p, b.roff.p, (size_t)nq + 1, false, SM_STASH0);
+            ctx_scan(c, b.rcnt.p, b.order_tmp.p, (size_t)nq + 1, false, SM_STASH1);
+            const u32* v = read_slots(c, SM_STASH0, 2);
+            NR = v[SM_STASH0], RR = v[SM_STASH1];
         }
         if (RR == 0) break;
         if (spec_round) {
@@ -348,20 +349,18 @@
     HIP_CHECK(hipMemsetAsync(b.nout.p, 0xFF, (size_t)nq * sizeof(u32), c->st));
     HIP_CHECK(hipMemsetAsync(b.nout.p + nq, 0, 4 * sizeof(u32), c->st));
     launch_final_select(b.toff.p, nq, c->v, b.sel.p, b.st_state.p, b.bits.p, b.nout.p, c->st);
-    const u32* dNO = scan_u32(b.nout.p, b.ooff.p, (size_t)nq + 1, false, c->d_scan_tmp.p, c->st);
+    ctx_scan(c, b.nout.p, b.ooff.p, (size_t)nq + 1, false, SM_STASH0);
     const int emit_parts = std::min<int>(EMIT_PARTS_MAX, std::max(1, (p.nspec && (b.permuted || p.pk_mixed)) ? 2 : (int)tune().emit_parts));
     const u32 emit_min_rows = (u32)std::max(1ll, tune().emit_min_rows);
     const u32 qstep = p.qstep = (nq + emit_parts - 1) / emit_parts;
     c->d_small.ensure(SM_WORDS);
-    launch_stride_gather(b.ooff.p, qstep, (nq + qstep - 1) / qstep, c->d_small.p + SM_PART_ROW, c->st);
-    stash_u32(c, dNO, SM_STASH0);
-    u32* v = (u32*)small_host(c);
-    HIP_CHECK(hipMemcpyAsync(v, c->d_small.p, (SM_PART_ROW + EMIT_PARTS_MAX) * sizeof(u32), hipMemcpyDeviceToHost, c->st));
+    u32* part_dst = host_word_dev(c, SM_PART_ROW);
+    launch_stride_gather(b.ooff.p, qstep, (nq + qstep - 1) / qstep, part_dst ? part_dst : c->d_small.p + SM_PART_ROW, c->st);
     if (b.permuted && !c->dev_out) {
         p.h_ooff.resize((size_t)nq + 1);
         HIP_CHECK(hipMemcpyAsync(p.h_ooff.data(), b.ooff.p, ((size_t)nq + 1) * sizeof(u32), hipMemcpyDeviceToHost, c->st));
     }
-    HIP_CHECK(hipStreamSynchronize(c->st));
+    const u32* v = read_slots(c, SM_STASH0, SM_PART_ROW + EMIT_PARTS_MAX);
     const u32 NO = p.NO = v[SM_STASH0];
     for (int q = 0; q <= emit_parts; ++q) p.part_row[q] = (u64)q * qstep < nq ? v[SM_PART_ROW + q] : NO;
     p.parts = (c->dev_out || NO < emit_min_rows) ? 1 : emit_parts;
@@ -378,7 +377,7 @@
     b.flags.ensure((size_t)NO + 4), b.gidx.ensure((size_t)NO + 4), b.sel_b.ensure((size_t)NO + 4), b.sel_a.ensure((size_t)NO + 4);
     c->d_scan_tmp.ensure(scan_u32_temp_elems((size_t)NO + 1) + 8);
     launch_trace_flags(slist, NO, b.tpos.p, b.flags.p, c->st);
-    const u32* dNB = scan_u32(b.flags.p, b.gidx.p, NO, false, c->d_scan_tmp.p, c->st);
+    const u32* dNB = ctx_scan(c, b.flags.p, b.gidx.p, NO, false);
     launch_trace_split(slist, NO, b.flags.p, b.gidx.p, b.sel_b.p, b.sel_a.p, c->st);
     u32* v = (u32*)small_host(c);
     HIP_CHECK(hipMemcpyAsync(v + parts, dNB, sizeof(u32), hipMemcpyDeviceToHost, c->st));
@@ -531,7 +530,7 @@
         b.d_ocnt.ensure((size_t)nq + 4), b.d_ostart.ensure((size_t)nq + 4);
         launch_scatter_u32(b.nout.p, b.d_qid.p, nq, b.d_ocnt.p, c->st);
         HIP_CHECK(hipMemsetAsync(b.d_ocnt.p + nq, 0, sizeof(u32), c->st));
-        scan_u32(b.d_ocnt.p, b.d_ostart.p, (size_t)nq + 1, false, c->d_scan_tmp.p, c->st);
+        ctx_scan(c, b.d_ocnt.p, b.d_ostart.p, (size_t)nq + 1, false);
         d_qid = b.d_qid.p, d_ostart = b.d_ostart.p;
     }
     launch_make_hits(b.outrec.p, NO, b.q_lo, d_qid, b.ooff.p, d_ostart, c->qry.d_off.p, c->ref.d_off.p, c->ref.N, c->d_p2tab.p, P2TAB_N,
@@ -769,7 +768,7 @@
         d_units.ensure((size_t)n + 4), d_tofs.ensure((size_t)n + 4);
         c->d_scan_tmp.ensure(scan_u32_temp_elems((size_t)n + 1) + 8);
         launch_trace_units(d_tasks.p, d_list.p, (u32)n, seqs, d_units.p, c->st);
-        const size_t tw = (size_t)d2h_u32(c, scan_u32(d_units.p, d_tofs.p, (size_t)n + 1, false, c->d_scan_tmp.p, c->st)) * TU;
+        const size_t tw = (size_t)scan_total(c, d_units.p, d_tofs.p, (size_t)n + 1, false) * TU;
         d_trace.ensure(tw + 64);
         if (aln || cig) aln_slots(c, chain, d_tasks.p, d_list.p, (u32)n, (u32)n, seqs);
         launch_align_walk(d_tasks.p, d_list.p, (u32)n, seqs, d_trace.p, TU, d_tofs.p, d_res.p, c->st, kernel == 3 ? (u32)n : 0u, aln || cig ? chain.code.p : nullptr,
diff --git a/swiftortho_amd/csrc/host_seed.hip b/swiftortho_amd/csrc/host_seed.hip
--- a/swiftortho_amd/csrc/host_seed.hip
+++ b/swiftortho_amd/csrc/host_seed.hip
@@ -158,8 +158,76 @@
 
 
 void* small_host(so_ctx* c) {
-    if (!c->h_small) HIP_CHECK(hipHostMalloc((void**)&c->h_small, 1024, hipHostMallocDefault));
+    if (!c->h_small) {
+        HIP_CHECK(hipHostMalloc((void**)&c->h_small, 1024 + HW_WORDS * sizeof(u32), hipHostMallocDefault));
+        memset(c->h_small, 0, 1024 + HW_WORDS * sizeof(u32));
+        HIP_CHECK(hipHostGetDevicePointer((void**)&c->hw_dev, (char*)c->h_small + 1024, 0));
+    }
     return c->h_small;
+}
+
+u32* host_words(so_ctx* c) { return (u32*)((char*)small_host(c) + 1024); }
+u32* host_word_dev(so_ctx* c, int k) {
+    if (!tune().host_words) return nullptr;
+    small_host(c);
+    return c->hw_dev + k;
+}
+ScanChain* scan_chain(so_ctx* c) {
+    if (!tune().scan_chain) return nullptr;
+    small_host(c);
+    c->scan.err = c->hw_dev + HW_SCAN_ERR;
+    return &c->scan;
+}
+
+const u32* ctx_scan(so_ctx* c, const u32* in, u32* out, size_t n, bool inclusive, int slot) {
+    ScanChain* ch = scan_chain(c);
+    u32* hw = slot >= 0 ? host_word_dev(c, slot) : nullptr;
+    const u32 e0 = c->scan.epoch;
+    const u32* d = scan_u32(in, out, n, inclusive, c->d_scan_tmp.p, c->st, ch, hw);
+    if (c->scan.epoch != e0) c->scan_last = {in, out, n, inclusive, slot, c->scan.epoch};
+    if (slot >= 0 && !hw) stash_u32(c, d, slot);
+    return d;
+}
+const u32* ctx_effscan(so_ctx* c, const u8* mark, const u32* scnt, size_t n, u32* hoff, u32* cidx) {
+    u32* hw = host_word_dev(c, SM_STASH0);
+    static_assert(SM_STASH1 == SM_STASH0 + 1, "effscan's two totals");
+    const u32* d = effscan(mark, scnt, n, hoff, cidx, c->d_scan_tmp.p, c->st, scan_chain(c), hw);
+    if (!hw) fetch_word(c, d, SM_STASH0, 2);
+    return d;
+}
+void fetch_word(so_ctx* c, const u32* dev, int slot, int n) {
+    HIP_CHECK(hipMemcpyAsync(host_words(c) + slot, dev, (size_t)n * sizeof(u32), hipMemcpyDeviceToHost, c->st));
+}
+
+static void scan_ran_out(so_ctx* c, bool pretend) {
+    u32* hw = host_words(c);
+    const auto& L = c->scan_last;
+    const u32 e = pretend ? L.epoch : hw[HW_SCAN_ERR];
+    hw[HW_SCAN_ERR] = 0;
+    if (!c->scan_fallback_told) {
+        c->scan_fallback_told = true;
+        if (!pretend) fprintf(stderr, "[sohit] chained scan %u: look-back ran out of polls, scan redone by the three-launch path\n", e);
+    }
+    if (e != L.epoch || L.slot < 0 || L.in == L.out) {
+        if (pretend) return;
+        throw SoError("chained scan: look-back ran out of polls in a scan that cannot be redone (SOHIT_SCAN_CHAIN=0 avoids the path)");
+    }
+    u32* hwd = host_word_dev(c, L.slot);
+    const u32* d = scan_u32(L.in, L.out, L.n, L.inclusive, c->d_scan_tmp.p, c->st, nullptr, hwd);
+    if (!hwd) fetch_word(c, d, L.slot);
+    HIP_CHECK(hipStreamSynchronize(c->st));
+}
+
+const u32* read_slots(so_ctx* c, int lo, int n) {
+    u32* hw = host_words(c);
+    if (n > 0 && !tune().host_words) {
+        c->d_small.ensure(SM_WORDS);
+        HIP_CHECK(hipMemcpyAsync(hw + lo, c->d_small.p + lo, (size_t)n * sizeof(u32), hipMemcpyDeviceToHost, c->st));
+    }
+    HIP_CHECK(hipStreamSynchronize(c->st));
+    if (hw[HW_SCAN_ERR] != 0) scan_ran_out(c, false);
+    else if (tune().scan_chain == 2 && c->scan_last.slot >= lo && c->scan_last.slot < lo + n && c->scan_last.epoch == c->scan.epoch) scan_ran_out(c, true);
+    return hw;
 }
 
 u32 d2h_u32(so_ctx* c, const u32* p) {
@@ -359,18 +427,16 @@
     u32 H, K;
     if (AS == 1) {
         c->d_scan_tmp.ensure(effscan_temp_elems(Tp) + 8);
-        const u32* dHK = effscan(b.mark.p + p_lo, b.scnt.p + t_lo, Tp, b.hoff.p + t_lo, b.cidx.p + t_lo, c->d_scan_tmp.p, c->st);
-        u32* v = (u32*)small_host(c);
-        HIP_CHECK(hipMemcpyAsync(v, dHK, 2 * sizeof(u32), hipMemcpyDeviceToHost, c->st));
-        HIP_CHECK(hipStreamSynchronize(c->st));
-        H = v[0], K = v[1];
+        ctx_effscan(c, b.mark.p + p_lo, b.scnt.p + t_lo, Tp, b.hoff.p + t_lo, b.cidx.p + t_lo);
+        const u32* v = read_slots(c, 0, 0);
+        H = v[SM_STASH0], K = v[SM_STASH1];
     } else {
         b.eff.ensure((size_t)AS * b.dev.Ppad + 4), b.nz.ensure((size_t)AS * b.dev.Ppad + 4);
         launch_effcnt(b.mark.p, b.scnt.p, AS, p_lo, p_hi, b.eff.p, b.nz.p, c->st);
-        const u32* dH = scan_u32(b.eff.p + t_lo, b.hoff.p + t_lo, Tp, false, c->d_scan_tmp.p, c->st);
-        stash_u32(c, dH, SM_STASH0);
-        const u32* dK = scan_u32(b.nz.p + t_lo, b.cidx.p + t_lo, Tp, false, c->d_scan_tmp.p, c->st);
-        d2h_pair(c, dK, H, K);
+        ctx_scan(c, b.eff.p + t_lo, b.hoff.p + t_lo, Tp, false, SM_STASH0);
+        ctx_scan(c, b.nz.p + t_lo, b.cidx.p + t_lo, Tp, false, SM_STASH1);
+        const u32* v = read_slots(c, SM_STASH0, 2);
+        H = v[SM_STASH0], K = v[SM_STASH1];
     }
     sc.lap("seed.bounds_cap_scan");
     c->cnt.seed_hits += H;
@@ -473,7 +539,7 @@
         b.bt0.ensure((size_t)nqp + 4);
         launch_bkt_ntiles(qseg, nqp, b.bt0.p, c->st);
         c->d_scan_tmp.ensure(scan_u32_temp_elems((size_t)nqp + 1) + 8);
-        const u32 NT = d2h_u32(c, scan_u32(b.bt0.p, b.bt0.p, (size_t)nqp + 1, false, c->d_scan_tmp.p, c->st));
+        const u32 NT = scan_total(c, b.bt0.p, b.bt0.p, (size_t)nqp + 1, false);
         if ((u64)L.R * NT >= 0xFFFFFFF0ull) return false;
         b.btd.ensure(4 * (size_t)NT + 8);
         launch_bkt_tiledesc(qseg, b.bt0.p, nqp, NT, b.cs_hoff.p, K, b.btd.p, c->st);
@@ -501,10 +567,10 @@
         b.bpart.ensure(npart + 4);
         c->d_scan_tmp.ensure(scan_u32_temp_elems(npart + 1) + 8);
         launch_bkt_colsum(b.bmat.p, NT, L.R, b.bpart.p, c->st);
-        const u32* dHv = scan_u32(b.bpart.p, b.bpart.p, npart, false, c->d_scan_tmp.p, c->st);
-        stash_u32(c, dHv, SM_SEED_TOTAL);
+        const u32* dHv = ctx_scan(c, b.bpart.p, b.bpart.p, npart, false, SM_SEED_TOTAL);
+        if (tune().host_words) stash_u32(c, dHv, SM_SEED_TOTAL);
         launch_bkt_colscan(b.bmat.p, NT, L.R, b.bpart.p, c->st);
-        const u32 Hv = d2h_u32(c, c->d_small.p + SM_SEED_TOTAL);
+        const u32 Hv = read_slots(c, SM_SEED_TOTAL, 1)[SM_SEED_TOTAL];
         sc.lap("seed.bucket_count");
         b.hits32.ensure((size_t)H + 2);
         {
@@ -658,13 +724,13 @@
             c->d_scan_tmp.ensure(scan_u32_temp_elems((size_t)bnb + 2) + 8);
             HIP_CHECK(hipMemsetAsync(b.bcnt.p, 0, ((size_t)bnb + 2) * sizeof(u32), c->st));
             launch_rec_count(b.p_qs.p, NP, klr.bs, bL, b.bcnt.p, b.pidx.p, c->st);
-            scan_u32(b.bcnt.p, b.bcnt.p, (size_t)bnb + 1, false, c->d_scan_tmp.p, c->st);
+            ctx_scan(c, b.bcnt.p, b.bcnt.p, (size_t)bnb + 1, false);
             launch_rec_scatter(b.p_qs.p, b.p_sd.p, b.p_ft.p, b.pidx.p, NP, klr, bL, ft_bits_entry, bsp, c->ref.d_off.p + ch.seq_lo, b.bcnt.p, b.q_qs.p,
                                b.q_sd.p, b.q_ft.p, c->st);
             HIP_CHECK(hipMemsetAsync(b.bccnt.p + bnb, 0, 2 * sizeof(u32), c->st));
             launch_bkt_best(false, b.q_qs.p, b.q_sd.p, b.q_ft.p, b.bcnt.p, bnb, bL, klr.bs, (u32)ch.seq_lo, b.bccnt.p, nullptr, nullptr, nullptr, bsp, 0,
                             c->st);
-            NS = d2h_u32(c, scan_u32(b.bccnt.p, b.bccnt.p, (size_t)bnb + 1, false, c->d_scan_tmp.p, c->st));
+            NS = scan_total(c, b.bccnt.p, b.bccnt.p, (size_t)bnb + 1, false);
             if (tune().debug)
                 fprintf(stderr, "[sohit] seed pass: queries %u..%u hits %u seeds %u pass records %u candidates %u (bucketed best)\n", qa, qb, H, K, NP, NS);
             b.c_ft.ensure((size_t)NS + 2), b.c_q.ensure((size_t)NS + 2), b.c_rec.ensure(4 * (size_t)NS + 8);
@@ -689,17 +755,18 @@
             c->d_scan_tmp.ensure(scan_u32_temp_elems((size_t)nqp + 2) + 8);
             HIP_CHECK(hipMemsetAsync(b.bcnt.p, 0, ((size_t)nqp + 2) * sizeof(u32), c->st));
             launch_rec_count(q_qs, NP, klr.bs, Lq, b.bcnt.p, b.pidx.p, c->st);
-            scan_u32(b.bcnt.p, b.bcnt.p, (size_t)nqp + 1, false, c->d_scan_tmp.p, c->st);
+            ctx_scan(c, b.bcnt.p, b.bcnt.p, (size_t)nqp + 1, false);
             launch_qrec_scatter(q_qs, q_sd, q_ft, b.pidx.p, NP, klr.bs, qa, b.bcnt.p, b.pidx2.p , b.order.p , b.p_qs2.p ,
                                 b.tmp64.p , c->st);
             HIP_CHECK(hipMemsetAsync(b.bflag.p, 0, sizeof(u32), c->st));
             launch_q_best(b.bcnt.p, qa, nqp, b.order.p, b.p_qs2.p, b.tmp64.p, (u32)ch.seq_lo, bsp, b.c_rec.p, b.order2.p, qcnt, b.bflag.p, c->st);
             HIP_CHECK(hipMemcpyAsync(b.bccnt.p, qcnt + qa, (size_t)nqp * sizeof(u32), hipMemcpyDeviceToDevice, c->st));
             HIP_CHECK(hipMemsetAsync(b.bccnt.p + nqp, 0, 2 * sizeof(u32), c->st));
-            const u32* dT = scan_u32(b.bccnt.p, b.bccnt.p, (size_t)nqp + 1, false, c->d_scan_tmp.p, c->st);
-            stash_u32(c, dT, SM_STASH0);
-            u32 flag = 0;
-            d2h_pair(c, b.bflag.p, NS, flag);
+            ctx_scan(c, b.bccnt.p, b.bccnt.p, (size_t)nqp + 1, false, SM_STASH0);
+            fetch_word(c, b.bflag.p, SM_STASH1);
+            const u32* v = read_slots(c, SM_STASH0, 1);
+            NS = v[SM_STASH0];
+            const u32 flag = v[SM_STASH1];
             if (!flag) {
                 if (tune().debug) fprintf(stderr, "[sohit] seed pass: queries %u..%u hits %u seeds %u pass records %u candidates %u (per query)\n", qa, qb, H, K, NP, NS);
                 if (NS) {
@@ -725,10 +792,14 @@
         b.flags.ensure((size_t)NP + 4), b.gidx.ensure((size_t)NP + 4);
         c->d_small.ensure(SM_WORDS);
         launch_seg_flags(b.p_qs2.p, NP, b.flags.p, c->d_small.p + SM_STASH0, c->st);
-        const u32* dS = scan_u32(b.flags.p, b.gidx.p, NP, false, c->d_scan_tmp.p, c->st);
+        const u32* dS = ctx_scan(c, b.flags.p, b.gidx.p, NP, false, SM_STASH1);
         b.qseg.ensure((size_t)b.nq + 4);
         launch_qseg(b.p_qs2.p, NP, b.gidx.p, dS, klr.bs, qa, qb, b.qseg.p, c->d_small.p + SM_STASH0, c->st);
-        d2h_pair(c, dS, maxseg, NS);
+        fetch_word(c, c->d_small.p + SM_STASH0, SM_STASH0);
+        {
+            const u32* v = read_slots(c, SM_STASH1, 1);
+            maxseg = v[SM_STASH0], NS = v[SM_STASH1];
+        }
         b.shead.ensure((size_t)NS + 2);
         if (tune().debug) fprintf(stderr, "[sohit] seed pass: queries %u..%u hits %u seeds %u pass records %u candidates %u\n", qa, qb, H, K, NP, NS);
         launch_group_list(b.flags.p, b.gidx.p, NP, b.shead.p, c->st);
diff --git a/swiftortho_amd/csrc/k_util.hip b/swiftortho_amd/csrc/k_util.hip
--- a/swiftortho_amd/csrc/k_util.hip
+++ b/swiftortho_amd/csrc/k_util.hip
@@ -1,5 +1,6 @@
 #include "common.h"
 #include "kernels.h"
+#include <type_traits>
 
 #define SCAN_THREADS 256
 #define SCAN_ITERS 8
@@ -58,7 +59,7 @@
     if (threadIdx.x == 0) blocksums[blockIdx.x] = tot;
 }
 
-__global__ __launch_bounds__(SCAN_THREADS) void k_scan_blocksums(u32* __restrict__ blocksums, size_t nb) {
+__global__ __launch_bounds__(SCAN_THREADS) void k_scan_blocksums(u32* __restrict__ blocksums, size_t nb, u32* __restrict__ total2) {
     __shared__ u32 lds4[4];
     u32 carry = 0;
     for (size_t b0 = 0; b0 < nb; b0 += SCAN_THREADS) {
@@ -69,7 +70,10 @@
         if (i < nb) blocksums[i] = carry + ex;
         carry += tot;
     }
-    if (threadIdx.x == 0) blocksums[nb] = carry;
+    if (threadIdx.x == 0) {
+        blocksums[nb] = carry;
+        if (total2) *total2 = carry;
+    }
 }
 
 __global__ __launch_bounds__(SCAN_THREADS) void k_scan_apply(const u32* __restrict__ in, u32* __restrict__ out, size_t n,
@@ -161,7 +165,7 @@
     if (threadIdx.x == 0) blocksums[blockIdx.x] = tot;
 }
 
-__global__ __launch_bounds__(SCAN_THREADS) void k_scan_blocksums64(u64* __restrict__ blocksums, size_t nb) {
+__global__ __launch_bounds__(SCAN_THREADS) void k_scan_blocksums64(u64* __restrict__ blocksums, size_t nb, u32* __restrict__ total2) {
     __shared__ u64 lds4[4];
     u64 carry = 0;
     for (size_t b0 = 0; b0 < nb; b0 += SCAN_THREADS) {
@@ -172,7 +176,10 @@
         if (i < nb) blocksums[i] = carry + ex;
         carry += tot;
     }
-    if (threadIdx.x == 0) blocksums[nb] = carry;
+    if (threadIdx.x == 0) {
+        blocksums[nb] = carry;
+        if (total2) total2[0] = (u32)carry, total2[1] = (u32)(carry >> 32);
+    }
 }
 
 __global__ __launch_bounds__(SCAN_THREADS) void k_effscan_apply(const u8* __restrict__ mark, const u32* __restrict__ scnt, size_t n,
@@ -200,25 +207,10 @@
     }
 }
 
-size_t effscan_temp_elems(size_t n) { return 2 * ((n + SCAN_TILE - 1) / SCAN_TILE + 2) + 2; }
-
-const u32* effscan(const u8* mark, const u32* scnt, size_t n, u32* hoff, u32* cidx, u32* temp, hipStream_t st) {
-    const size_t nb = (n + SCAN_TILE - 1) / SCAN_TILE;
-    u64* t64 = reinterpret_cast<u64*>(temp);
-    if (nb == 0) {
-        HIP_CHECK(hipMemsetAsync(t64, 0, sizeof(u64), st));
-        return temp;
-    }
-    hipLaunchKernelGGL(k_effscan_reduce, dim3((unsigned)nb), dim3(SCAN_THREADS), 0, st, mark, scnt, n, t64);
-    hipLaunchKernelGGL(k_scan_blocksums64, dim3(1), dim3(SCAN_THREADS), 0, st, t64, nb);
-    hipLaunchKernelGGL(k_effscan_apply, dim3((unsigned)nb), dim3(SCAN_THREADS), 0, st, mark, scnt, n, t64, hoff, cidx);
-    return reinterpret_cast<const u32*>(t64 + nb);
-}
-
 #define SS_THREADS 1024
 #define SS_ITEMS 16
 __global__ __launch_bounds__(SS_THREADS) void k_scan_small(const u32* __restrict__ in, u32* __restrict__ out, size_t n, u32* __restrict__ total,
-                                                           int inclusive) {
+                                                           int inclusive, u32* __restrict__ total2) {
     __shared__ u32 s_w[SS_THREADS / 64];
     const int lane = threadIdx.x & 63, w = threadIdx.x >> 6;
     u32 carry = 0;
@@ -266,24 +258,258 @@
         }
         carry += tot;
     }
-    if (threadIdx.x == 0) *total = carry;
-}
+    if (threadIdx.x == 0) {
+        *total = carry;
+        if (total2) *total2 = carry;
+    }
+}
+#define SCAN_SPIN_MAX (1u << 22)
+#define SCAN_TICKET0 0xFFFFFF00u
+typedef __attribute__((address_space(1))) u64 gu64;
+
+template <int W>
+__device__ __forceinline__ void chain_publish(u64* slot, u32 epoch, u64 v) {
+    __hip_atomic_store((gu64*)slot, ((u64)epoch << 32) | (u32)v, __ATOMIC_RELAXED, __HIP_MEMORY_SCOPE_AGENT);
+    if (W == 2) __hip_atomic_store((gu64*)slot + 1, ((u64)epoch << 32) | (u32)(v >> 32), __ATOMIC_RELAXED, __HIP_MEMORY_SCOPE_AGENT);
+}
+template <int W>
+__device__ __forceinline__ bool chain_read(const u64* slot, u32 epoch, u64& v) {
+    const u64 a = __hip_atomic_load((const gu64*)slot, __ATOMIC_RELAXED, __HIP_MEMORY_SCOPE_AGENT);
+    if ((u32)(a >> 32) != epoch) return false;
+    v = (u32)a;
+    if (W == 2) {
+        const u64 b = __hip_atomic_load((const gu64*)slot + 1, __ATOMIC_RELAXED, __HIP_MEMORY_SCOPE_AGENT);
+        if ((u32)(b >> 32) != epoch) return false;
+        v |= b << 32;
+    }
+    return true;
+}
+template <int W>
+__device__ __forceinline__ bool chain_lookback(const u64* status, u32 tile, u32 epoch, u32 spin_max, u64& excl_out) {
+    const int lane = threadIdx.x & 63;
+    u64 excl = 0;
+    i64 j = (i64)tile - 1;
+    u32 polls = 0;
+    for (;;) {
+        const i64 idx = j - lane;
+        u64 v = 0;
+        bool has_prefix = false, ready = true;
+        if (idx >= 0) {
+            const u64* s = status + 4 * (size_t)idx;
+            has_prefix = chain_read<W>(s + 2, epoch, v);
+            ready = has_prefix || chain_read<W>(s, epoch, v);
+        }
+        const unsigned long long mp = __ballot(has_prefix), mn = __ballot(!ready);
+        const int fp = mp ? __ffsll(mp) - 1 : 64, fn = mn ? __ffsll(mn) - 1 : 64;
+        if (fn < fp) {
+            if (++polls > spin_max) return false;
+            __builtin_amdgcn_s_sleep(1);
+            continue;
+        }
+        u64 x = lane <= fp ? v : 0;
+#pragma unroll
+        for (int o = 32; o; o >>= 1) x += __shfl_xor((unsigned long long)x, o);
+        excl += x;
+        if (fp < 64) break;
+        j -= 64;
+    }
+    excl_out = excl;
+    return true;
+}
+
+struct ChainArgs {
+    u32* ticket;
+    u64* status;
+    u32 base, epoch, spin_max, nb;
+    u32* total;
+    u32* total2;
+    u32* err;
+};
+
+__device__ __forceinline__ u32 wave_incl_scan(u32 v, int lane) { return wave_incl_scan_u32(v, lane); }
+__device__ __forceinline__ u64 wave_incl_scan(u64 v, int lane) { return wave_incl_scan_u64(v, lane); }
+
+template <bool EFF>
+__global__ __launch_bounds__(SCAN_THREADS) void k_scan_chain(const u32* in, const u8* mark, u32* out, u32* out2, size_t n, int inclusive, ChainArgs a) {
+    typedef typename std::conditional<EFF, u64, u32>::type V;
+    constexpr int W = EFF ? 2 : 1;
+    __shared__ V s_w[SCAN_ITERS * (SCAN_THREADS / 64)];
+    __shared__ u64 s_excl;
+    __shared__ u32 s_tile;
+    __shared__ int s_ok;
+    const int lane = threadIdx.x & 63, w = threadIdx.x >> 6;
+    if (threadIdx.x == 0) s_tile = atomicAdd(a.ticket, 1u) - a.base;
+    __syncthreads();
+    const u32 tile = s_tile;
+    if (tile >= a.nb) {
+        if (threadIdx.x == 0) *a.err = a.epoch;
+        return;
+    }
+    const size_t base = (size_t)tile * SCAN_TILE;
+    uint4 c[SCAN_ITERS];
+    V ex[SCAN_ITERS];
+#pragma unroll
+    for (int it = 0; it < SCAN_ITERS; ++it) {
+        const size_t i = base + (size_t)it * SCAN_THREADS * 4 + (size_t)threadIdx.x * 4;
+        V s;
+        if (EFF) {
+            c[it] = eff4(mark, in, i, n);
+            s = (V)pair4(c[it]);
+        } else {
+            c[it] = make_uint4(0, 0, 0, 0);
+            if (i + 3 < n) {
+                c[it] = ld4(in + i);
+            } else {
+                if (i < n) c[it].x = in[i];
+                if (i + 1 < n) c[it].y = in[i + 1];
+                if (i + 2 < n) c[it].z = in[i + 2];
+            }
+            s = (V)(c[it].x + c[it].y + c[it].z + c[it].w);
+        }
+        const V inc = wave_incl_scan(s, lane);
+        if (lane == 63) s_w[it * (SCAN_THREADS / 64) + w] = inc;
+        ex[it] = inc - s;
+    }
+    __syncthreads();
+    V run = 0;
+#pragma unroll
+    for (int it = 0; it < SCAN_ITERS; ++it)
+#pragma unroll
+        for (int k = 0; k < SCAN_THREADS / 64; ++k) {
+            if (k == w) ex[it] += run;
+            run += s_w[it * (SCAN_THREADS / 64) + k];
+        }
+    if (threadIdx.x < 64) {
+        u64* slot = a.status + 4 * (size_t)tile;
+        u64 excl = 0;
+        bool ok = true;
+        if (tile == 0) {
+            if (lane == 0) chain_publish<W>(slot + 2, a.epoch, (u64)run);
+        } else {
+            if (lane == 0) chain_publish<W>(slot, a.epoch, (u64)run);
+            ok = chain_lookback<W>(a.status, tile, a.epoch, a.spin_max, excl);
+            if (ok && lane == 0) chain_publish<W>(slot + 2, a.epoch, excl + (u64)run);
+        }
+        if (lane == 0) {
+            s_excl = excl, s_ok = ok;
+            if (!ok) {
+                *a.err = a.epoch;
+            } else if (tile == a.nb - 1) {
+                const u64 t = excl + (u64)run;
+                a.total[0] = (u32)t;
+                if (EFF) a.total[1] = (u32)(t >> 32);
+                if (a.total2) {
+                    a.total2[0] = (u32)t;
+                    if (EFF) a.total2[1] = (u32)(t >> 32);
+                }
+            }
+        }
+    }
+    __syncthreads();
+    if (!s_ok) return;
+    const V carry = (V)s_excl;
+#pragma unroll
+    for (int it = 0; it < SCAN_ITERS; ++it) {
+        const size_t i = base + (size_t)it * SCAN_THREADS * 4 + (size_t)threadIdx.x * 4;
+        const V e = carry + ex[it];
+        const uint4 v = c[it];
+        if (EFF) {
+            const u32 h0 = (u32)e, h1 = h0 + v.x, h2 = h1 + v.y, h3 = h2 + v.z;
+            const u32 k0 = (u32)((u64)e >> 32), k1 = k0 + (v.x != 0), k2 = k1 + (v.y != 0), k3 = k2 + (v.z != 0);
+            if (i + 3 < n) {
+                st4(out + i, make_uint4(h0, h1, h2, h3));
+                st4(out2 + i, make_uint4(k0, k1, k2, k3));
+            } else {
+                if (i < n) out[i] = h0, out2[i] = k0;
+                if (i + 1 < n) out[i + 1] = h1, out2[i + 1] = k1;
+                if (i + 2 < n) out[i + 2] = h2, out2[i + 2] = k2;
+            }
+        } else {
+            u32 o0, o1, o2, o3;
+            if (inclusive) o0 = (u32)e + v.x, o1 = o0 + v.y, o2 = o1 + v.z, o3 = o2 + v.w;
+            else o0 = (u32)e, o1 = o0 + v.x, o2 = o1 + v.y, o3 = o2 + v.z;
+            if (i + 3 < n) {
+                st4(out + i, make_uint4(o0, o1, o2, o3));
+            } else {
+                if (i < n) out[i] = o0;
+                if (i + 1 < n) out[i + 1] = o1;
+                if (i + 2 < n) out[i + 2] = o2;
+            }
+        }
+    }
+}
+
+void scan_chain_release(ScanChain& ch) {
+    if (ch.ticket) (void)hipFree(ch.ticket);
+    if (ch.status) (void)hipFree(ch.status);
+    ch.ticket = nullptr, ch.status = nullptr, ch.tiles = 0;
+}
+
+static ChainArgs chain_next(ScanChain& ch, size_t nb, u32* total, u32* total2, hipStream_t st) {
+    if (!ch.ticket) {
+        const u32 t0 = SCAN_TICKET0;
+        HIP_CHECK(hipMalloc((void**)&ch.ticket, 256));
+        HIP_CHECK(hipMemcpy(ch.ticket, &t0, sizeof t0, hipMemcpyHostToDevice));
+        ch.base = t0, ch.epoch = 0;
+    }
+    if (nb > ch.tiles) {
+        HIP_CHECK(hipStreamSynchronize(st));
+        if (ch.status) (void)hipFree(ch.status);
+        ch.status = nullptr, ch.tiles = 0;
+        const size_t t = nb + nb / 2 + 256;
+        HIP_CHECK(hipMalloc((void**)&ch.status, t * 4 * sizeof(u64)));
+        HIP_CHECK(hipMemsetAsync(ch.status, 0, t * 4 * sizeof(u64), st));
+        ch.tiles = t;
+    }
+    if (++ch.epoch == 0) {
+        HIP_CHECK(hipMemsetAsync(ch.status, 0, ch.tiles * 4 * sizeof(u64), st));
+        ch.epoch = 1;
+    }
+    ChainArgs a;
+    a.ticket = ch.ticket, a.status = ch.status, a.base = ch.base, a.epoch = ch.epoch, a.spin_max = SCAN_SPIN_MAX, a.nb = (u32)nb;
+    a.total = total, a.total2 = total2, a.err = ch.err;
+    ch.base += (u32)nb;
+    return a;
+}
+
+size_t effscan_temp_elems(size_t n) { return 2 * ((n + SCAN_TILE - 1) / SCAN_TILE + 2) + 2; }
+
+const u32* effscan(const u8* mark, const u32* scnt, size_t n, u32* hoff, u32* cidx, u32* temp, hipStream_t st, ScanChain* ch, u32* total2) {
+    const size_t nb = (n + SCAN_TILE - 1) / SCAN_TILE;
+    u64* t64 = reinterpret_cast<u64*>(temp);
+    if (nb == 0) {
+        HIP_CHECK(hipMemsetAsync(t64, 0, sizeof(u64), st));
+        if (total2) fill_u32(total2, 2, 0u, st);
+        return temp;
+    }
+    if (ch && ch->err && !ch->use_three) {
+        hipLaunchKernelGGL(k_scan_chain<true>, dim3((unsigned)nb), dim3(SCAN_THREADS), 0, st, scnt, mark, hoff, cidx, n, 0,
+                           chain_next(*ch, nb, reinterpret_cast<u32*>(t64 + nb), total2, st));
+        return reinterpret_cast<const u32*>(t64 + nb);
+    }
+    hipLaunchKernelGGL(k_effscan_reduce, dim3((unsigned)nb), dim3(SCAN_THREADS), 0, st, mark, scnt, n, t64);
+    hipLaunchKernelGGL(k_scan_blocksums64, dim3(1), dim3(SCAN_THREADS), 0, st, t64, nb, total2);
+    hipLaunchKernelGGL(k_effscan_apply, dim3((unsigned)nb), dim3(SCAN_THREADS), 0, st, mark, scnt, n, t64, hoff, cidx);
+    return reinterpret_cast<const u32*>(t64 + nb);
+}
+
 #define SCAN_SMALL_TILES 4
 
 size_t scan_u32_temp_elems(size_t n) { return (n + SCAN_TILE - 1) / SCAN_TILE + 2; }
 
-const u32* scan_u32(const u32* in, u32* out, size_t n, bool inclusive, u32* temp, hipStream_t st) {
+const u32* scan_u32(const u32* in, u32* out, size_t n, bool inclusive, u32* temp, hipStream_t st, ScanChain* ch, u32* total2) {
     size_t nb = (n + SCAN_TILE - 1) / SCAN_TILE;
-    if (nb == 0) {
-        HIP_CHECK(hipMemsetAsync(temp, 0, sizeof(u32), st));
-        return temp;
-    }
     if (nb <= SCAN_SMALL_TILES) {
-        hipLaunchKernelGGL(k_scan_small, dim3(1), dim3(SS_THREADS), 0, st, in, out, n, temp + nb, inclusive ? 1 : 0);
+        hipLaunchKernelGGL(k_scan_small, dim3(1), dim3(SS_THREADS), 0, st, in, out, n, temp + nb, inclusive ? 1 : 0, total2);
         return temp + nb;
     }
+    if (ch && ch->err && !ch->use_three) {
+        hipLaunchKernelGGL(k_scan_chain<false>, dim3((unsigned)nb), dim3(SCAN_THREADS), 0, st, in, (const u8*)nullptr, out, (u32*)nullptr, n,
+                           inclusive ? 1 : 0, chain_next(*ch, nb, temp + nb, total2, st));
+        return temp + nb;
+    }
     hipLaunchKernelGGL(k_scan_reduce, dim3((unsigned)nb), dim3(SCAN_THREADS), 0, st, in, n, temp);
-    hipLaunchKernelGGL(k_scan_blocksums, dim3(1), dim3(SCAN_THREADS), 0, st, temp, nb);
+    hipLaunchKernelGGL(k_scan_blocksums, dim3(1), dim3(SCAN_THREADS), 0, st, temp, nb, total2);
     hipLaunchKernelGGL(k_scan_apply, dim3((unsigned)nb), dim3(SCAN_THREADS), 0, st, in, out, n, temp, inclusive ? 1 : 0);
     return temp + nb;
 }
diff --git a/swiftortho_amd/csrc/kernels.h b/swiftortho_amd/csrc/kernels.h
--- a/swiftortho_amd/csrc/kernels.h
+++ b/swiftortho_amd/csrc/kernels.h
@@ -5,8 +5,20 @@
 
 size_t scan_u32_temp_elems(size_t n);
 size_t effscan_temp_elems(size_t n);
-const u32* effscan(const u8* mark, const u32* scnt, size_t n, u32* hoff, u32* cidx, u32* temp, hipStream_t st);
-const u32* scan_u32(const u32* in, u32* out, size_t n, bool inclusive, u32* temp, hipStream_t st);
+struct ScanChain {
+    u32* ticket = nullptr;
+    u64* status = nullptr;
+    size_t tiles = 0;
+    u32 base = 0;
+    u32 epoch = 0;
+    u32* err = nullptr;
+    bool use_three = false;
+};
+void scan_chain_release(ScanChain& ch);
+const u32* effscan(const u8* mark, const u32* scnt, size_t n, u32* hoff, u32* cidx, u32* temp, hipStream_t st, ScanChain* ch = nullptr,
+                   u32* total2 = nullptr);
+const u32* scan_u32(const u32* in, u32* out, size_t n, bool inclusive, u32* temp, hipStream_t st, ScanChain* ch = nullptr,
+                    u32* total2 = nullptr);
 void fill_u32(u32* p, size_t n, u32 v, hipStream_t st);
 
 size_t sort_keys_u64_temp_bytes(size_t n, int bits);
diff --git a/swiftortho_amd/csrc/tune.h b/swiftortho_amd/csrc/tune.h
--- a/swiftortho_amd/csrc/tune.h
+++ b/swiftortho_amd/csrc/tune.h
@@ -38,6 +38,9 @@
     X(I, emit_parts, "SOHIT_EMIT_PARTS", 4, "... and otherwise")                                                                                               \
     X(I, emit_min_rows, "SOHIT_EMIT_MIN_ROWS", 1 << 18, "rows below which the emission is one part")                                                           \
     X(P, test_oom_phase2, "SOHIT_TEST_OOM_PHASE2", 0, "tests: phase 2 of the first batch fails once with an out-of-memory error")                              \
+                                                                                                                  \
+    X(B, host_words, "SOHIT_HOST_WORDS", 1, "totals and counts the host waits for are stored to pinned host words by the kernel that computes them (0: parked in a device word and copied)") \
+    X(I, scan_chain, "SOHIT_SCAN_CHAIN", 1, "device-wide scans above 32 k values in one launch, tiles chained by look-back (0: reduce / block sums / apply; 2, tests: chained, and every total the host reads is computed again by the three launches as if a look-back had run out)") \
                                                                                                                                  \
     X(I, batch, "SOHIT_BATCH", 0, "queries per device batch (0: 131072, lowered when the candidate estimate asks)")                                            \
     X(I, max_hits, "SOHIT_MAX_HITS", 0, "seed hits per pass (0: 2^30)")                                                                                        \
```

New measurement: 670.8 M query-aa/s. Within noise of the previous version (-0.2%).
